# settylab/Mellon

Measured on AMD Instinct MI355X. Metric: cells/sec fit_predict, higher is better.
Workload: dtype f64

## Files before the change

### include/mellon_hip.h

```cpp
#ifndef MELLON_HIP_H
#define MELLON_HIP_H

#include <stdint.h>

#ifdef __cplusplus
extern "C" {
#endif

typedef struct mln_ctx mln_ctx;
typedef struct mln_fit mln_fit;

typedef enum {
  MLN_OK = 0,
  MLN_ERR_NOT_PD = 1,
  MLN_ERR_SHAPE = 2,
  MLN_ERR_HIP = 3,
  MLN_ERR_RCCL = 4,
  MLN_ERR_ARG = 5,
  MLN_ERR_UNSUPPORTED = 6,
  MLN_ERR_NOCONV = 7
} mln_status;

typedef enum {
  MLN_K_MATERN32 = 1,
// ... 35 lines not shown
int mln_ctx_create(int device, mln_ctx** out);
void mln_ctx_destroy(mln_ctx* ctx);
const char* mln_last_error(mln_ctx* ctx);
int mln_device_info(mln_ctx* ctx, char* name, int name_cap, int* n_cu, int64_t* mem_bytes);
int mln_device_count(int* count_out);
int mln_synchronize(mln_ctx* ctx);

int mln_malloc(mln_ctx* ctx, int64_t bytes, void** dev_ptr);
int mln_free(mln_ctx* ctx, void* dev_ptr);
int mln_memcpy(mln_ctx* ctx, void* dst, const void* src, int64_t bytes);
int mln_host_register(mln_ctx* ctx, const void* host_ptr, int64_t bytes);
int mln_host_unregister(mln_ctx* ctx, const void* host_ptr);
int mln_release_cached_memory(void);
int mln_diag_alloc_stats(int64_t* out);

#define MLN_UNIQUE_ID_BYTES 128
int mln_comm_unique_id(void* id_out );
int mln_comm_init(mln_ctx* ctx, const void* id, int n_ranks, int rank);
int mln_comm_allreduce_sum(mln_ctx* ctx, double* buf, int64_t count);
typedef struct mln_loopback mln_loopback;
int mln_loopback_create(int n_ranks , mln_loopback** out);
void mln_loopback_destroy(mln_loopback* group);
int mln_comm_init_loopback(mln_ctx* ctx, mln_loopback* group, int rank);
typedef int (*mln_host_collective_fn)(void* user, int op, double* buf, double* buf2, int64_t count);
int mln_comm_init_host(mln_ctx* ctx, int n_ranks, int rank, mln_host_collective_fn fn, void* user);
void mln_loopback_abort(mln_loopback* group);
int mln_comm_info(mln_ctx* ctx, int32_t* info, double* stats, int32_t flags);

int mln_kernel_matrix(mln_ctx* ctx, const mln_kernel_desc* cov, const double* x, int64_t n,
                      const double* y, int64_t m, int32_t d, double* out);

int mln_kernel_gram(mln_ctx* ctx, const mln_kernel_desc* cov, const double* x, int64_t n_local, int32_t d,
                    const double* xu, int64_t m, double* out );
int mln_nn_distances(mln_ctx* ctx, const double* x, int64_t n, const double* y, int64_t m, int32_t d,
                     int64_t self_offset, double* out );
int mln_knn(mln_ctx* ctx, const double* x, int64_t n, const double* y, int64_t m, int32_t d, int32_t k,
            int32_t exclude, int64_t self_offset, double* dist , int64_t* idx );
int mln_local_dimensionality(mln_ctx* ctx, const double* x, int64_t n, int32_t d, const int64_t* nbr, int64_t q,
                             int32_t k, double* out );

int mln_kmeans(mln_ctx* ctx, const double* x, int64_t n, int32_t d, int64_t m, int64_t seed,
               int32_t max_iter, double tol, double* centers, int32_t* n_iter_out, double* inertia_out);
int mln_kmeans_sklearn(mln_ctx* ctx, const double* x, int64_t n, int32_t d, int64_t m, int64_t first_id,
                       const double* uniforms, int32_t n_local_trials, int32_t max_iter, double tol, double* centers,
                       int64_t* indices_out, int32_t* n_iter_out, double* inertia_out);

int mln_chol_lower(mln_ctx* ctx, double* A, int64_t m, double add_diag);

int mln_trsm_lower(mln_ctx* ctx, const double* Lf, int64_t m, int32_t trans, double* B, int64_t p);

#define MLN_FIT_IMPLICIT 1
int mln_fit_prepare(mln_ctx* ctx, const mln_kernel_desc* cov, const double* x, int64_t n_local,
                    int32_t d, const double* xu, int64_t m, double jitter, const double* Lp_in,
                    int32_t flags, mln_fit** out);
int mln_fit_from_L(mln_ctx* ctx, const double* L, int64_t n_local, int64_t m, const double* Lp,
                   mln_fit** out);
#define MLN_FIT_FULL 2
#define MLN_FIT_DEFER_LP 4
int mln_fit_prepare_from_K(mln_ctx* ctx, const double* Kuu, int64_t n_local, int64_t m, double jitter,
                           const double* Lp_in, int32_t flags, mln_fit** out);
int mln_fit_set_K_rows(mln_fit* fit, int64_t row0, int64_t n_rows, const double* K_rows);
int mln_fit_finish_K(mln_fit* fit);
int mln_gemm(mln_ctx* ctx, int32_t ta, int32_t tb, int64_t M, int64_t N, int64_t K, double alpha, const double* A,
             int64_t lda, const double* B, int64_t ldb, double beta, double* C, int64_t ldc);
int mln_ewise(mln_ctx* ctx, int32_t op, const double* a, const double* b, double scalar, double* out, int64_t count);

void mln_fit_destroy(mln_fit* fit);
int mln_fit_get_Lp(mln_fit* fit, double* out );
int mln_fit_get_L(mln_fit* fit, int64_t row0, int64_t n_rows, double* out );
int mln_fit_rank(mln_fit* fit, int64_t* m_out);

int mln_kernel_grad(mln_ctx* ctx, const mln_kernel_desc* cov, const double* x, int64_t n, const double* y,
                    int64_t m, int32_t d, double* out );
int mln_predict_gradient(mln_ctx* ctx, const mln_kernel_desc* cov, const double* xnew, int64_t n_new,
                         int32_t d, const double* centers, int64_t m, const double* W ,
                         double* out );
int mln_predict_hessian(mln_ctx* ctx, const mln_kernel_desc* cov, const double* xnew, int64_t n_new, int32_t d,
                        const double* centers, int64_t m, const double* W , double* out);


int mln_eigh(mln_ctx* ctx, const double* A, int64_t m, double* w, double* V, int32_t* n_sweeps);
int mln_fit_gram_eigh(mln_fit* fit, double* w , int32_t* n_sweeps);
int mln_fit_gram_rank(mln_fit* fit, double tol, int64_t* rank_out, double* sigma_max_out);
int mln_fit_project(mln_fit* fit, int64_t p, mln_fit** out);

int mln_ridge_init(mln_fit* fit, const double* target, double* z0 );

int mln_precond_build(mln_fit* fit, int64_t row_stride );
int mln_fit_set_row_offset(mln_fit* fit, int64_t global_row0);
int mln_precond_apply(mln_fit* fit, int32_t mode, const double* in, double* out);
int mln_objective_precond(mln_fit* fit, const double* u, double* loss, double* grad_u ,
                          double* z_out );

int mln_fit_set_likelihood(mln_fit* fit, const double* V, const double* Vdr, double mu);

int mln_objective(mln_fit* fit, const double* z, double* loss, double* grad ,
                  double* hess_diag );

int mln_objective_batch(mln_fit* fit, const double* Z, int32_t S, double* loss , double* grad );

typedef struct {
  int32_t maxiter;
  int32_t maxcor;
  int32_t maxls;
  double ftol;
  double gtol;
} mln_solver_opts;
int mln_map_solve(mln_fit* fit, const double* z0, const mln_solver_opts* opts ,
                  double* z_out , double* loss_out, int32_t* n_eval_out, int32_t* n_iter_out,
                  int32_t* status_out);

int mln_fit_set_dim_likelihood(mln_fit* fit, const double* ell, int32_t k, double mu_dim, double mu_dens);
int mln_dim_objective(mln_fit* fit, const double* z, double* loss, double* grad ,
                      double* hess_diag );

int mln_dim_objective_batch(mln_fit* fit, const double* Z, int32_t S, double* loss , double* grad );

int mln_transform(mln_fit* fit, const double* z, double mu, double* f_out );

int mln_weights_cholesky(mln_fit* fit, const double* z, double* w );
int mln_weights_full(mln_fit* fit, const double* y, int64_t p, double mu, double* w );

int mln_sparse_solve(mln_ctx* ctx, const mln_kernel_desc* cov, const double* x, int64_t n_local,
                     int32_t d, const double* xu, int64_t m, const double* y, int64_t p, double mu,
                     double sigma, double jitter, double* W );
int mln_sparse_solve_factors(mln_ctx* ctx, const mln_kernel_desc* cov, const double* x, int64_t n_local,
                             int32_t d, const double* xu, int64_t m, const double* y, int64_t p, double mu,
                             double sigma, double jitter, double* W, double* Lp_out, double* Cs_out);

enum { MLN_SIGMA_SCALAR = 0, MLN_SIGMA_PER_OUTPUT = 1, MLN_SIGMA_PER_CELL = 2 };
int mln_sparse_solve_noise(mln_ctx* ctx, const mln_kernel_desc* cov, const double* x, int64_t n_local,
                           int32_t d, const double* xu, int64_t m, const double* y, int64_t p, double mu,
                           const double* sigma, int32_t sigma_kind, double jitter, double* W );

int mln_full_conditional_noise(mln_ctx* ctx, const mln_kernel_desc* cov, const double* x, int64_t n, int32_t d,
                               const double* y, int64_t p, double mu, const double* sigma , double jitter,
                               double* W, double* leverage, double* corrected_r2, double* variance_W);

int mln_landmark_leverage(mln_ctx* ctx, const mln_kernel_desc* cov, const double* x, int64_t n_local, int32_t d,
                          const double* xu, int64_t m, const double* Lk, const double* sigma, int64_t p,
                          double jitter, double* out );

int mln_predict_mean(mln_ctx* ctx, const mln_kernel_desc* cov, const double* xnew, int64_t n_new,
                     int32_t d, const double* centers, int64_t m, const double* W, int64_t p,
                     double mu, double* out);

int mln_diag_peak(mln_ctx* ctx, int32_t what, int64_t bytes, double* result);
int mln_diag_dgemm(mln_ctx* ctx, int32_t ta, int32_t tb, int64_t M, int64_t N, int64_t K,
                   int32_t lower_only, int32_t split_k, int32_t reps, double* ms_out);
int mln_diag_dgemm_compare(mln_ctx* ctx, int32_t ta, int32_t tb, int64_t M, int64_t N, int64_t K, int32_t lower_only,
                           int32_t kmode, double beta, int32_t any_size, double* out);
int mln_diag_gram_i8(mln_ctx* ctx, const double* A, int64_t rows, int64_t m, double* out, int32_t reps, double* ms_out);
int mln_diag_overlap(mln_ctx* ctx, int64_t n, int64_t m, int32_t d, int64_t gram_rows, double* out );

int mln_predict_covariance(mln_ctx* ctx, const mln_kernel_desc* cov, const double* xnew, int64_t n_new,
                           int32_t d, const double* centers, int64_t m, const double* Lf, int32_t diag,
                           double* out);
int mln_predict_mean_covariance(mln_ctx* ctx, const mln_kernel_desc* cov, const double* xnew, int64_t n_new,
                                int32_t d, const double* centers, int64_t m, const double* W, int64_t q,
                                int32_t diag, double* out);

#define MLN_N_STAGE_TIMES 22
int mln_stage_times(mln_fit* fit, double* out );

#ifdef __cplusplus
}
#endif
#endif
```

### mellon_amd/_lib.py

```python
import ctypes as C
import os
import threading

import numpy as np

_HERE = os.path.dirname(os.path.abspath(__file__))
LIB_PATH = os.path.join(_HERE, "libmellon_hip.so")

MLN_OK, MLN_ERR_NOT_PD, MLN_ERR_SHAPE, MLN_ERR_HIP, MLN_ERR_RCCL, MLN_ERR_ARG, MLN_ERR_UNSUPPORTED = range(7)
MLN_UNIQUE_ID_BYTES = 128
MLN_N_STAGE_TIMES = 22

K_MATERN32, K_MATERN52, K_EXPQUAD, K_EXPONENTIAL, K_RATQUAD, K_LINEAR, K_DISTANCE = 1, 2, 3, 4, 5, 6, 7
OP_LEAF, OP_CONST, OP_ADD, OP_MUL, OP_POW = 0, 1, 2, 3, 4


HOST_COLLECTIVE_FN = C.CFUNCTYPE(C.c_int, C.c_void_p, C.c_int, C.c_void_p, C.c_void_p, C.c_int64)


class MellonHipError(RuntimeError):
    """HIP / RCCL / argument failure inside libmellon_hip.so."""


class Leaf(C.Structure):
    _fields_ = [("kind", C.c_int32), ("ndims", C.c_int32), ("ls", C.c_double), ("alpha", C.c_double),
                ("dims", C.POINTER(C.c_int32))]


class Tok(C.Structure):
    _fields_ = [("op", C.c_int32), ("leaf", C.c_int32), ("value", C.c_double)]


class SolverOpts(C.Structure):
    _fields_ = [("maxiter", C.c_int32), ("maxcor", C.c_int32), ("maxls", C.c_int32), ("ftol", C.c_double),
                ("gtol", C.c_double)]


class KernelDesc(C.Structure):
    _fields_ = [("n_leaves", C.c_int32), ("n_toks", C.c_int32), ("leaves", C.POINTER(Leaf)),
                ("toks", C.POINTER(Tok))]


_vp, _i64, _i32, _dbl, _dp = C.c_void_p, C.c_int64, C.c_int32, C.c_double, C.c_void_p
_KD = C.POINTER(KernelDesc)
SYMBOLS = [
    ("mln_ctx_create", C.c_int, [C.c_int, C.POINTER(_vp)]),
    ("mln_ctx_destroy", None, [_vp]),
    ("mln_last_error", C.c_char_p, [_vp]),
    ("mln_device_info", C.c_int, [_vp, C.c_char_p, C.c_int, C.POINTER(C.c_int), C.POINTER(_i64)]),
    ("mln_device_count", C.c_int, [C.POINTER(C.c_int)]),
    ("mln_synchronize", C.c_int, [_vp]),
    ("mln_malloc", C.c_int, [_vp, _i64, C.POINTER(_vp)]),
    ("mln_free", C.c_int, [_vp, _vp]),
    ("mln_memcpy", C.c_int, [_vp, _vp, _vp, _i64]),
    ("mln_host_register", C.c_int, [_vp, _vp, _i64]),
    ("mln_host_unregister", C.c_int, [_vp, _vp]),
    ("mln_release_cached_memory", C.c_int, []),
    ("mln_diag_alloc_stats", C.c_int, [_vp]),
    ("mln_comm_unique_id", C.c_int, [_vp]),
    ("mln_comm_init", C.c_int, [_vp, _vp, C.c_int, C.c_int]),
    ("mln_comm_allreduce_sum", C.c_int, [_vp, _dp, _i64]),
    ("mln_loopback_create", C.c_int, [C.c_int, C.POINTER(_vp)]),
    ("mln_loopback_destroy", None, [_vp]),
    ("mln_comm_init_loopback", C.c_int, [_vp, _vp, C.c_int]),
    ("mln_comm_init_host", C.c_int, [_vp, C.c_int, C.c_int, _vp, _vp]),
    ("mln_loopback_abort", None, [_vp]),
    ("mln_comm_info", C.c_int, [_vp, C.POINTER(_i32), _dp, _i32]),
    ("mln_kernel_matrix", C.c_int, [_vp, _KD, _dp, _i64, _dp, _i64, _i32, _dp]),
    ("mln_kernel_grad", C.c_int, [_vp, _KD, _dp, _i64, _dp, _i64, _i32, _dp]),
    ("mln_predict_gradient", C.c_int, [_vp, _KD, _dp, _i64, _i32, _dp, _i64, _dp, _dp]),
    ("mln_predict_hessian", C.c_int, [_vp, _KD, _dp, _i64, _i32, _dp, _i64, _dp, _dp]),
    ("mln_kernel_gram", C.c_int, [_vp, _KD, _dp, _i64, _i32, _dp, _i64, _dp]),
    ("mln_nn_distances", C.c_int, [_vp, _dp, _i64, _dp, _i64, _i32, _i64, _dp]),
    ("mln_knn", C.c_int, [_vp, _dp, _i64, _dp, _i64, _i32, _i32, _i32, _i64, _dp, _vp]),
    ("mln_local_dimensionality", C.c_int, [_vp, _dp, _i64, _i32, _vp, _i64, _i32, _dp]),
    ("mln_kmeans", C.c_int, [_vp, _dp, _i64, _i32, _i64, _i64, _i32, _dbl, _dp, C.POINTER(_i32), C.POINTER(_dbl)]),
    ("mln_kmeans_sklearn", C.c_int, [_vp, _dp, _i64, _i32, _i64, _i64, _dp, _i32, _i32, _dbl, _dp, _vp, C.POINTER(_i32),
                                     C.POINTER(_dbl)]),
    ("mln_chol_lower", C.c_int, [_vp, _dp, _i64, _dbl]),
    ("mln_trsm_lower", C.c_int, [_vp, _dp, _i64, _i32, _dp, _i64]),
    ("mln_fit_prepare", C.c_int, [_vp, _KD, _dp, _i64, _i32, _dp, _i64, _dbl, _dp, _i32, C.POINTER(_vp)]),
    ("mln_fit_from_L", C.c_int, [_vp, _dp, _i64, _i64, _dp, C.POINTER(_vp)]),
    ("mln_fit_prepare_from_K", C.c_int, [_vp, _dp, _i64, _i64, _dbl, _dp, _i32, C.POINTER(_vp)]),
    ("mln_fit_set_K_rows", C.c_int, [_vp, _i64, _i64, _dp]),
    ("mln_fit_finish_K", C.c_int, [_vp]),
    ("mln_gemm", C.c_int, [_vp, _i32, _i32, _i64, _i64, _i64, _dbl, _dp, _i64, _dp, _i64, _dbl, _dp, _i64]),
    ("mln_ewise", C.c_int, [_vp, _i32, _dp, _dp, _dbl, _dp, _i64]),
    ("mln_fit_destroy", None, [_vp]),
    ("mln_fit_get_Lp", C.c_int, [_vp, _dp]),
    ("mln_fit_get_L", C.c_int, [_vp, _i64, _i64, _dp]),
    ("mln_fit_rank", C.c_int, [_vp, C.POINTER(_i64)]),
    ("mln_eigh", C.c_int, [_vp, _dp, _i64, _dp, _dp, C.POINTER(_i32)]),
    ("mln_fit_gram_eigh", C.c_int, [_vp, _dp, C.POINTER(_i32)]),
    ("mln_fit_gram_rank", C.c_int, [_vp, _dbl, C.POINTER(_i64), C.POINTER(_dbl)]),
    ("mln_fit_project", C.c_int, [_vp, _i64, C.POINTER(_vp)]),
    ("mln_ridge_init", C.c_int, [_vp, _dp, _dp]),
    ("mln_precond_build", C.c_int, [_vp, _i64]),
    ("mln_fit_set_row_offset", C.c_int, [_vp, _i64]),
    ("mln_precond_apply", C.c_int, [_vp, _i32, _dp, _dp]),
    ("mln_objective_precond", C.c_int, [_vp, _dp, C.POINTER(_dbl), _dp, _dp]),
    ("mln_map_solve", C.c_int, [_vp, _dp, C.POINTER(SolverOpts), _dp, C.POINTER(_dbl), C.POINTER(_i32),
                                C.POINTER(_i32), C.POINTER(_i32)]),
    ("mln_fit_set_likelihood", C.c_int, [_vp, _dp, _dp, _dbl]),
    ("mln_objective", C.c_int, [_vp, _dp, C.POINTER(_dbl), _dp, _dp]),
    ("mln_objective_batch", C.c_int, [_vp, _dp, _i32, _dp, _dp]),
    ("mln_fit_set_dim_likelihood", C.c_int, [_vp, _dp, _i32, _dbl, _dbl]),
    ("mln_dim_objective", C.c_int, [_vp, _dp, C.POINTER(_dbl), _dp, _dp]),
    ("mln_dim_objective_batch", C.c_int, [_vp, _dp, _i32, _dp, _dp]),
    ("mln_transform", C.c_int, [_vp, _dp, _dbl, _dp]),
    ("mln_weights_cholesky", C.c_int, [_vp, _dp, _dp]),
    ("mln_weights_full", C.c_int, [_vp, _dp, _i64, _dbl, _dp]),
    ("mln_sparse_solve", C.c_int, [_vp, _KD, _dp, _i64, _i32, _dp, _i64, _dp, _i64, _dbl, _dbl, _dbl, _dp]),
    ("mln_sparse_solve_factors", C.c_int, [_vp, _KD, _dp, _i64, _i32, _dp, _i64, _dp, _i64, _dbl, _dbl, _dbl, _dp,
                                           _dp, _dp]),
    ("mln_sparse_solve_noise", C.c_int, [_vp, _KD, _dp, _i64, _i32, _dp, _i64, _dp, _i64, _dbl, _dp, _i32, _dbl, _dp]),
    ("mln_full_conditional_noise", C.c_int, [_vp, _KD, _dp, _i64, _i32, _dp, _i64, _dbl, _dp, _dbl, _dp, _dp, _dp, _dp]),
    ("mln_landmark_leverage", C.c_int, [_vp, _KD, _dp, _i64, _i32, _dp, _i64, _dp, _dp, _i64, _dbl, _dp]),
    ("mln_predict_mean", C.c_int, [_vp, _KD, _dp, _i64, _i32, _dp, _i64, _dp, _i64, _dbl, _dp]),
    ("mln_predict_covariance", C.c_int, [_vp, _KD, _dp, _i64, _i32, _dp, _i64, _dp, _i32, _dp]),
    ("mln_predict_mean_covariance", C.c_int, [_vp, _KD, _dp, _i64, _i32, _dp, _i64, _dp, _i64, _i32, _dp]),
    ("mln_stage_times", C.c_int, [_vp, _dp]),
    ("mln_diag_peak", C.c_int, [_vp, _i32, _i64, C.POINTER(_dbl)]),
    ("mln_diag_overlap", C.c_int, [_vp, _i64, _i64, _i32, _i64, _dp]),
    ("mln_diag_gram_i8", C.c_int, [_vp, _vp, _i64, _i64, _vp, _i32, C.POINTER(_dbl)]),
    ("mln_diag_dgemm", C.c_int, [_vp, _i32, _i32, _i64, _i64, _i64, _i32, _i32, _i32, C.POINTER(_dbl)]),
    ("mln_diag_dgemm_compare", C.c_int, [_vp, _i32, _i32, _i64, _i64, _i64, _i32, _i32, _dbl, _i32, C.POINTER(_dbl)]),
]

_lib = None
_lib_lock = threading.Lock()


def load_library():
    global _lib
    with _lib_lock:
        if _lib is not None:
            return _lib
        if not os.path.exists(LIB_PATH):
            raise MellonHipError(
                f"{LIB_PATH} is missing: build it with `python -c \"import __graft_entry__ as g; g.build()\"` "
                "(hipcc --offload-arch=gfx950).  mellon_amd has no CPU fallback.")
        lib = C.CDLL(LIB_PATH, mode=C.RTLD_GLOBAL)
        for name, res, args in SYMBOLS:
            fn = getattr(lib, name)
            fn.restype = res
            fn.argtypes = args
        _lib = lib
        return lib


def device_count():
    n = C.c_int(0)
    load_library().mln_device_count(C.byref(n))
    return int(n.value)


class BlockEvaluatedCov:
    rows_per_block = 8192

    def block(self, x, y):
        raise NotImplementedError


def _needs_program(desc, what):
    if isinstance(desc, BlockEvaluatedCov):
        raise NotImplementedError(
            f"{what} needs a covariance that lowers to one device program (built-in kernels combined with + * ** within "
            "the program limits); user-defined Python kernels and larger trees support k(), fit and the predictive mean.")


class DeviceArray:

    def __init__(self, ctx, shape):
        self.ctx = ctx
        self.shape = tuple(int(s) for s in shape)
        self.size = int(np.prod(self.shape)) if self.shape else 1
        ptr = C.c_void_p()
        ctx._check(ctx.lib.mln_malloc(ctx.handle, self.size * 8, C.byref(ptr)))
        self.ptr = ptr.value

    @property
    def nbytes(self):
        return self.size * 8

    @property
    def ndim(self):
        return len(self.shape)

    def to_host(self):
        out = np.empty(self.shape, dtype=np.float64)
        self.ctx._check(self.ctx.lib.mln_memcpy(self.ctx.handle, out.ctypes.data, self.ptr, self.nbytes))
        return out

    def free(self):
        if self.ptr is not None and self.ctx.handle is not None:
            self.ctx.lib.mln_free(self.ctx.handle, self.ptr)
        self.ptr = None

    def __del__(self):
        try:
            self.free()
        except Exception:
            pass


def _f64(a):
    return np.ascontiguousarray(a, dtype=np.float64)


def _ptr(a):
    if a is None:
        return None
    if isinstance(a, DeviceArray):
        return a.ptr
    return a.ctypes.data


class Context:

    def __init__(self, device=None):
        self.lib = load_library()
        if device is None:
            device = int(os.environ.get("LOCAL_RANK", "0")) if "MELLON_AMD_DEVICE" not in os.environ \
                else int(os.environ["MELLON_AMD_DEVICE"])
        h = C.c_void_p()
        rc = self.lib.mln_ctx_create(int(device), C.byref(h))
        self.handle = None
        if rc != MLN_OK:
            msg = self.lib.mln_last_error(None).decode()
            raise MellonHipError(f"mln_ctx_create(device={device}) failed: {msg}")
        self.handle = h.value
        self.device = int(device)
        self.n_ranks, self.rank = 1, 0

    def close(self):
        if self.handle is not None:
            self.lib.mln_ctx_destroy(self.handle)
            self.handle = None

    def __del__(self):
        try:
            self.close()
        except Exception:
            pass

    def _check(self, rc, jitter=None):
        if rc == MLN_OK:
            return
        msg = self.lib.mln_last_error(self.handle).decode()
        if rc == MLN_ERR_NOT_PD:
            raise ValueError(
                f"Covariance not positively definite with jitter={jitter}. "
                "Consider increasing the jitter for numerical stabilization.")
        if rc == MLN_ERR_SHAPE:
            raise ValueError(f"libmellon_hip: {msg}")
        if rc == MLN_ERR_UNSUPPORTED:
            raise NotImplementedError(f"libmellon_hip: {msg}")
        cause = None
        staged = getattr(self, "_host_collective", None)
        if staged is not None and getattr(staged[1], "failure", None) is not None:
            cause, staged[1].failure = staged[1].failure, None
        raise MellonHipError(f"libmellon_hip error {rc}: {msg}" + (f" ({type(cause).__name__}: {cause})" if cause else "")) from cause

    def device_info(self):
        name = C.create_string_buffer(64)
        cu, mem = C.c_int(), C.c_int64()
        self._check(self.lib.mln_device_info(self.handle, name, 64, C.byref(cu), C.byref(mem)))
        return {"arch": name.value.decode(), "n_cu": cu.value, "mem_bytes": mem.value}

    def synchronize(self):
        self._check(self.lib.mln_synchronize(self.handle))

    def to_device(self, a):
        a = _f64(a)
        d = DeviceArray(self, a.shape)
        self._check(self.lib.mln_memcpy(self.handle, d.ptr, a.ctypes.data, a.nbytes))
# ... 622 lines not shown

    def gram_rank(self, tol):
        r, smax = _i64(0), C.c_double()
        self._check(self.lib.mln_fit_gram_rank(self.handle, float(tol), C.byref(r), C.byref(smax)))
        return int(r.value), smax.value

    def project(self, p):
        new = Fit.__new__(Fit)
        new.ctx, new.lib, new.handle = self.ctx, self.lib, None
        h = C.c_void_p()
        self._check(self.lib.mln_fit_project(self.handle, int(p), C.byref(h)))
        new.handle = h.value
        new.n, new.d, new.m, new.jitter = self.n, None, int(p), None
        new.implicit = False
        new._has_lp = False
        return new

    def __init__(self, ctx, desc, x, landmarks, jitter, Lp=None, implicit=False):
        self.ctx, self.lib, self.handle = ctx, ctx.lib, None
        self.implicit = bool(implicit) and landmarks is not None
        x = x if isinstance(x, DeviceArray) else _as2d(x)
        n, d = x.shape
        xu = None if landmarks is None else (landmarks if isinstance(landmarks, DeviceArray) else _as2d(landmarks))
        m = n if xu is None else xu.shape[0]
        Lp_ = None if Lp is None else _f64(Lp)
        if Lp_ is not None and Lp_.shape != (m, m):
            raise ValueError(f"Lp has shape {Lp_.shape}, expected {(m, m)}")
        h = C.c_void_p()
        flags = (1 | (4 if Lp_ is None else 0)) if self.implicit else 0
        ctx._check(self.lib.mln_fit_prepare(ctx.handle, desc.ref, _ptr(x), n, d, _ptr(xu), m, float(jitter),
                                            _ptr(Lp_), flags, C.byref(h)), jitter=jitter)
        self.handle = h.value
        self.n, self.d, self.m, self.jitter = n, d, m, jitter
        self._has_lp = True

    def _check(self, rc, jitter=None):
        if rc == MLN_ERR_NOT_PD and self.lib.mln_last_error(self.ctx.handle).startswith(b"cov(xu, xu)"):
            jitter = self.jitter
        self.ctx._check(rc, jitter=jitter)

    def close(self):
        if self.handle is not None and self.ctx.handle is not None:
            self.lib.mln_fit_destroy(self.handle)
        self.handle = None

    def __del__(self):
        try:
            self.close()
        except Exception:
            pass

    def Lp(self):
        out = np.empty((self.m, self.m), dtype=np.float64)
        self._check(self.lib.mln_fit_get_Lp(self.handle, out.ctypes.data))
        return out

    def L(self, row0=0, n_rows=None):
        n_rows = self.n - row0 if n_rows is None else n_rows
        out = np.empty((n_rows, self.m), dtype=np.float64)
        self._check(self.lib.mln_fit_get_L(self.handle, row0, n_rows, out.ctypes.data))
        return out

    def ridge_init(self, target):
        target = target if isinstance(target, DeviceArray) else _f64(target)
        z0 = np.empty(self.m, dtype=np.float64)
        self._check(self.lib.mln_ridge_init(self.handle, _ptr(target), z0.ctypes.data), jitter="ridge")
        return z0

    def set_likelihood(self, V, Vdr, mu):
        V = V if isinstance(V, DeviceArray) else _f64(V)
        Vdr = Vdr if isinstance(Vdr, DeviceArray) else _f64(Vdr)
        self._check(self.lib.mln_fit_set_likelihood(self.handle, _ptr(V), _ptr(Vdr), float(mu)))

    def objective(self, z, with_hess=False):
        z = _f64(z)
        loss = C.c_double()
        grad = np.empty(self.m, dtype=np.float64)
        hess = np.empty(self.m, dtype=np.float64) if with_hess else None
        self._check(self.lib.mln_objective(self.handle, z.ctypes.data, C.byref(loss), grad.ctypes.data,
                                               _ptr(hess)))
        return (loss.value, grad, hess) if with_hess else (loss.value, grad)

    def objective_batch(self, Z):
        Z = _f64(Z)
        if Z.ndim != 2 or Z.shape[1] != self.m or Z.shape[0] < 1:
            raise ValueError(f"Z has shape {Z.shape}, expected (S >= 1, {self.m})")
        loss = np.empty(Z.shape[0], dtype=np.float64)
        grad = np.empty(Z.shape, dtype=np.float64)
        self._check(self.lib.mln_objective_batch(self.handle, Z.ctypes.data, int(Z.shape[0]), loss.ctypes.data,
                                                 grad.ctypes.data))
        return loss, grad

    def set_dim_likelihood(self, ell, mu_dim, mu_dens):
        ell = _f64(ell)
        if ell.ndim != 2 or ell.shape[0] != self.n:
            raise ValueError(f"ell has shape {ell.shape}, expected ({self.n}, k)")
        self._check(self.lib.mln_fit_set_dim_likelihood(self.handle, ell.ctypes.data, int(ell.shape[1]), float(mu_dim),
                                                        float(mu_dens)))

    def dim_objective(self, z, with_hess=False):
        z = _f64(z)
        if z.shape != (2, self.m):
            raise ValueError(f"z has shape {z.shape}, expected {(2, self.m)}")
        loss = C.c_double()
        grad = np.empty((2, self.m), dtype=np.float64)
        hess = np.empty((2, self.m), dtype=np.float64) if with_hess else None
        self._check(self.lib.mln_dim_objective(self.handle, z.ctypes.data, C.byref(loss), grad.ctypes.data, _ptr(hess)))
        return (loss.value, grad, hess) if with_hess else (loss.value, grad)

    def dim_objective_batch(self, Z):
        Z = _f64(Z)
        if Z.ndim not in (2, 3) or Z.shape[0] < 1 or Z.shape[1:] not in ((2, self.m), (2 * self.m,)):
            raise ValueError(f"Z has shape {Z.shape}, expected (S >= 1, 2, {self.m}) or (S >= 1, {2 * self.m})")
        loss = np.empty(Z.shape[0], dtype=np.float64)
        grad = np.empty(Z.shape, dtype=np.float64)
        self._check(self.lib.mln_dim_objective_batch(self.handle, Z.ctypes.data, int(Z.shape[0]), loss.ctypes.data,
                                                     grad.ctypes.data))
        return loss, grad

    def precond_build(self, row_stride=1, row_offset=0, force=False):
        built = getattr(self, "_precond_stride", None)
        if built is not None and (not force or built == int(row_stride)):
            return
        self._check(self.lib.mln_fit_set_row_offset(self.handle, int(row_offset)))
        self._check(self.lib.mln_precond_build(self.handle, int(row_stride)), jitter="ridge")
        self._precond_stride = max(1, int(row_stride))

    def precond_apply(self, mode, v):
        v = _f64(v)
        out = np.empty(self.m, dtype=np.float64)
        self._check(self.lib.mln_precond_apply(self.handle, int(mode), v.ctypes.data, out.ctypes.data),
                        jitter="ridge")
        return out

    def objective_precond(self, u):
        u = _f64(u)
        loss = C.c_double()
        grad = np.empty(self.m, dtype=np.float64)
        z = np.empty(self.m, dtype=np.float64)
        self._check(self.lib.mln_objective_precond(self.handle, u.ctypes.data, C.byref(loss), grad.ctypes.data,
                                                       z.ctypes.data), jitter="ridge")
        return loss.value, grad, z

    def map_solve(self, z0, maxiter=5000, maxcor=10, maxls=30, ftol=1e-13, gtol=1e-7):
        z0 = _f64(z0)
        opts = SolverOpts(int(maxiter), int(maxcor), int(maxls), float(ftol), float(gtol))
        z = np.empty(self.m, dtype=np.float64)
        loss, nev, nit, st = C.c_double(), C.c_int32(), C.c_int32(), C.c_int32()
        self._check(self.lib.mln_map_solve(self.handle, z0.ctypes.data, C.byref(opts), z.ctypes.data,
                                               C.byref(loss), C.byref(nev), C.byref(nit), C.byref(st)),
                        jitter="ridge")
        return z, loss.value, nev.value, nit.value, st.value

    def transform(self, z, mu, out=None):
        z = _f64(z)
        ret = np.empty(self.n, dtype=np.float64) if out is None else out
        self._check(self.lib.mln_transform(self.handle, z.ctypes.data, float(mu), _ptr(ret)))
        return ret

    def weights_cholesky(self, z):
        z = _f64(z)
        w = np.empty(self.m, dtype=np.float64)
        self._check(self.lib.mln_weights_cholesky(self.handle, z.ctypes.data, w.ctypes.data))
        return w

    def weights_full(self, y, mu):
        y2 = _f64(y)
        p = 1 if y2.ndim == 1 else y2.shape[1]
        w = np.empty_like(y2)
        self._check(self.lib.mln_weights_full(self.handle, y2.ctypes.data, p, float(mu), w.ctypes.data))
        return w

    def stage_times(self):
        out = np.zeros(MLN_N_STAGE_TIMES, dtype=np.float64)
        self._check(self.lib.mln_stage_times(self.handle, out.ctypes.data))
        keys = ["kernel_matrix_s", "cholesky_s", "trsm_s", "ridge_gram_s", "ridge_solve_s",
                "objective_kernel_s", "objective_launches", "objective_bytes_per_launch",
                "objective32_kernel_s", "objective32_launches", "copy32_format", "emulation_excluded_s",
                "objective_sub_kernel_s", "objective_sub_launches", "objective_sub_stride", "precond_rebuild_s",
                "precond_rebuilds", "objective_pass_equivalents", "precond_rebuilds_declined", "precond_reverts",
                "start_halvings", "rank_path"]
        return dict(zip(keys, out.tolist()))


def release_cached_memory():
    load_library().mln_release_cached_memory()


def alloc_stats():
    out = (C.c_int64 * 5)()
    rc = load_library().mln_diag_alloc_stats(out)
    if rc != 0:
        raise MellonHipError(f"mln_diag_alloc_stats failed ({rc})")
    keys = ["live_blocks", "live_bytes", "live_pinned_blocks", "cached_bytes", "driver_allocs"]
    return dict(zip(keys, [int(v) for v in out]))


_default_ctx = None


def default_context():
    global _default_ctx
    from . import distributed
    comm = distributed.thread_state()
    if comm is not None and comm.ctx is not None:
        return comm.ctx
    if _default_ctx is None or _default_ctx.handle is None:
        _default_ctx = Context()
    return _default_ctx
```

### mellon_amd/csrc/api_internal.h

```cpp
#pragma once
#include <chrono>
#include <cmath>
#include <cstdio>
#include <cstdlib>
#include <algorithm>
#include <atomic>
#include <cstring>
#include <memory>
#include <mutex>
#include <string>
#include <thread>
#include <vector>

#include "linalg.h"
#include "mln_internal.h"
#include "objective.h"
#include "precond_rebuild.h"
#include "solver.h"

void fit_events_borrow(mln_ctx* ctx, std::vector<hipEvent_t>* evs);
void fit_events_return(mln_ctx* ctx, std::vector<hipEvent_t>* evs);

bool is_device_ptr(const void* p);
double now_s();

struct DevIn {
  mln_ctx* ctx;
  const double* dev = nullptr;
  DevBuf<double> owned;
  int init(mln_ctx* c, const double* p, size_t count) {
    ctx = c;
    if (count == 0 || !p) { dev = p; return MLN_OK; }
    if (is_device_ptr(p)) { dev = p; return MLN_OK; }
    MLN_TRY(owned.alloc(ctx, count, "device copy of an input"));
    MLN_HIP(ctx, hipMemcpyAsync(owned, p, count * sizeof(double), hipMemcpyHostToDevice, ctx->stream));
    dev = owned;
    return MLN_OK;
  }
  ~DevIn() {
    if (owned) (void)hipStreamSynchronize(ctx->stream);
  }
};

struct DevOut {
  mln_ctx* ctx;
  double* dev = nullptr;
  DevBuf<double> owned;
  double* host = nullptr;
  size_t count = 0;
  int init(mln_ctx* c, double* p, size_t n, bool copy_in = false) {
    ctx = c; count = n;
    if (n == 0) { dev = p; return MLN_OK; }
    if (is_device_ptr(p)) { dev = p; return MLN_OK; }
    host = p;
    MLN_TRY(owned.alloc(ctx, n, "device copy of an output"));
    if (copy_in) MLN_HIP(ctx, hipMemcpyAsync(owned, p, n * sizeof(double), hipMemcpyHostToDevice, ctx->stream));
    dev = owned;
    return MLN_OK;
  }
  int commit() {
    if (owned && count) {
      MLN_HIP(ctx, hipMemcpyAsync(host, owned, count * sizeof(double), hipMemcpyDeviceToHost, ctx->stream));
    }
    MLN_HIP(ctx, hipStreamSynchronize(ctx->stream));
    return MLN_OK;
  }
  ~DevOut() {
    if (owned) (void)hipStreamSynchronize(ctx->stream);
  }
};

struct Precond { DevBuf<double> C, Cinv, P, Q1, Q2; };

struct mln_fit {
  mln_ctx* ctx = nullptr;
  DevCov cov;
  int d = 0;
  int64_t n = 0, m = 0, ldl = 0, ldp = 0;
  bool full = false;
  DevBuf<double> L_own;
  double* L = nullptr;
  DevBuf<double> Lp;
  TriInv tri;
  DevBuf<double> V, Vdr;
  double mu = 0.0;
  int n_wg = 0;
  DevBuf<double> part_grad, part_hess, part_loss;
  DevBuf<double> d_z, d_out;
  PinnedBuf<double> h_z, h_out;
  hipEvent_t ev0 = nullptr, ev1 = nullptr;
  double times[MLN_N_STAGE_TIMES] = {0};
  Precond pc, pc_saved;
  DevBuf<double> d_u, d_gu, d_tmp;
  int n_wg_cap = 0;
  bool kspace = false;
  DevBuf<double> Kj;
  bool lp_pending = false, lp_failed = false, tri_pending = false;
  double jitter = 0.0;
  DevBuf<double> d_w;
  std::vector<double> z_cached;
  DevBuf<double> d_w_cached;
  DevBuf<double> d_zw, d_zr;
  DevBuf<double> eigU;
  DevBuf<float> L32;
  double emu_excluded = 0.0;
  bool cov_bounded01 = false;
  int l32_fixed = 0;
  int evals32 = 0;
  double times32 = 0.0;
  int64_t ld2 = 0;
  DevBuf<int> d_over;
  int64_t row0 = 0;
  SolverBuffers sv{};
  DevBuf<double> sv_block;
  PinnedBuf<SolverState> h_state;
  int sv_maxcor = 0;
  std::vector<hipEvent_t> evs;
  DevBuf<double> f_keep[2];
  int f_final = -1;
  int64_t precond_stride = 0;
  bool from_K = false, k_finished = false;
  int64_t k_rows_done = 0;
  int n_revert = 0, n_rebuild_skipped = 0, n_start_halvings = 0, rank_path = 0;
  double build_seconds = 0.0;
  double times_sub = 0.0, times_rebuild = 0.0, sub_pass_equiv = 0.0;
  int evals_sub = 0, n_rebuild = 0;
  DevBuf<double> dim_ell;
  int dim_k = 0;
  double mu_dim = 0.0, mu_dens = 0.0;
  DevBuf<double> dim_part, dim_z, dim_out;
  ~mln_fit();
};

int dev_allreduce(mln_ctx* ctx, double* dev, int64_t count);
int dev_bcast0(mln_ctx* ctx, double* dev, int64_t count);
int reject_distance_leaf(mln_ctx* ctx, const DevCov& dc);
int64_t pad16(int64_t m);
void fit_sample_rows(const mln_fit* f, int64_t s, int64_t* first, int64_t* rows);
int fit_alloc_workspace(mln_fit* f);
int fit_prepare_impl(mln_ctx* ctx, const mln_kernel_desc* cov, const double* x, int64_t n, int32_t d,
                            const double* xu, int64_t m, double jitter, const double* Lp_in, int32_t flags,
                            mln_fit* f);
ObjArgs obj_args(mln_fit* f);
void obj_account(mln_fit* f, bool f32 = false);
int fit_w_from_z(mln_fit* f, const double* z_dev, double* w_dev, const double* z_host = nullptr);
int fit_cache_pair_from_u(mln_fit* f, const double* u_dev);
int fit_enqueue_eval(mln_fit* f, const double* u_dev, double* gn_dev, bool use32, const int* gate,
                            hipEvent_t* ev, const std::vector<int64_t>* sub_strides = nullptr);
int fit_objective_u(mln_fit* f, const double* u, double* loss, double* grad_u, double* z_out,
                           bool use32 = false);
int fit_solver_alloc(mln_fit* f, int maxcor);
int gram_of(mln_ctx* ctx, const double* A, int64_t lda, int64_t rows, int64_t m, double alpha, double* G,
                   int64_t ldg, bool quantised = false);
int emulated_ranks(const mln_ctx* ctx);
int fit_ensure_kj(mln_fit* f);
int fit_ensure_lp(mln_fit* f, bool need_tri = true);
int fit_lp_finish(mln_fit* f, int rc_chol, double t0);
int fit_gram(mln_fit* f, double* G, int64_t ldg, int64_t row_stride, bool whiten = true);
int fit_gemvT(mln_fit* f, const double* t_dev, double* rhs_dev);
int fit_factor_precond(mln_fit* f);
int fit_build_precond(mln_fit* f, int64_t row_stride);
int fit_rebuild_precond(mln_fit* f, const double* f_dev, double rows_per_m, int* outcome, double cap = 1e300);
int fit_precond_revert(mln_fit* f);
int fit_small_gemv(mln_fit* f, const double* M, int trans, const double* w, double* y);
int launch_scale_rows_cols(mln_ctx* ctx, double* A, int64_t ld, int64_t rows, int64_t cols, const double* row,
                                  const double* col);
int sparse_solve_impl(mln_ctx* ctx, const mln_kernel_desc* cov, const double* x, int64_t n_local,
                             int32_t d, const double* xu, int64_t m, const double* y, int64_t p, double mu,
                             const double* sigmas, int32_t kind, double jitter, double* W, double* Lp_out,
                             double* Cs_out);
unsigned grid_1d(int64_t count);
```

### mellon_amd/csrc/api_solve.hip

```cpp
#include "api_internal.h"
#include "mln_options.h"


void obj_account(mln_fit* f, bool f32) {
  float ms = 0.f;
  const bool ok = hipEventElapsedTime(&ms, f->ev0, f->ev1) == hipSuccess;
  if (f32) {
    if (ok) f->times32 += 1e-3 * ms;
    f->evals32 += 1;
    return;
  }
  if (ok) f->times[5] += 1e-3 * ms;
  f->times[6] += 1.0;
  f->times[7] = (double)f->n * (double)f->ldl * 8.0;
}

int fit_w_from_z(mln_fit* f, const double* z_dev, double* w_dev, const double* z_host) {
  mln_ctx* ctx = f->ctx;
  if (z_host && f->z_cached.size() == (size_t)f->m &&
      std::memcmp(z_host, f->z_cached.data(), sizeof(double) * f->m) == 0) {
    MLN_HIP(ctx, hipMemcpyAsync(w_dev, f->d_w_cached, sizeof(double) * f->m, hipMemcpyDeviceToDevice, ctx->stream));
    return MLN_OK;
  }
  MLN_TRY(fit_ensure_lp(f));
  MLN_HIP(ctx, hipMemcpyAsync(w_dev, z_dev, sizeof(double) * f->m, hipMemcpyDeviceToDevice, ctx->stream));
  return triinv_solve_left_T(ctx, f->tri, w_dev, 1, 1);
}

int fit_cache_pair_from_u(mln_fit* f, const double* u_dev) {
  mln_ctx* ctx = f->ctx;
  f->z_cached.assign((size_t)f->m, 0.0);
  MLN_HIP(ctx, hipMemcpyAsync(f->z_cached.data(), f->d_z, sizeof(double) * f->m, hipMemcpyDeviceToHost, ctx->stream));
  if (f->kspace) MLN_TRY(fit_small_gemv(f, f->pc.P, 0, u_dev, f->d_w_cached));
  MLN_HIP(ctx, hipStreamSynchronize(ctx->stream));
  return MLN_OK;
}

extern "C" int mln_objective(mln_fit* f, const double* z, double* loss, double* grad, double* hess_diag) {
  if (!f || !z || !loss || !grad) return MLN_ERR_ARG;
  mln_ctx* ctx = f->ctx;
  if (!f->V) { mln_set_error(ctx, "mln_fit_set_likelihood has not been called"); return MLN_ERR_ARG; }
  if (hess_diag && f->kspace) {
    mln_set_error(ctx, "the Hessian diagonal needs the explicit factor L: prepare the fit without MLN_FIT_IMPLICIT");
    return MLN_ERR_UNSUPPORTED;
  }
  MLN_HIP(ctx, hipSetDevice(ctx->device));
  MLN_TRY(fit_ensure_lp(f));
  const int64_t m = f->m;
  MLN_HIP(ctx, hipMemcpyAsync(f->d_z, z, sizeof(double) * m, hipMemcpyDefault, ctx->stream));
  MLN_HIP(ctx, hipMemcpyAsync(f->h_z, f->d_z, sizeof(double) * m, hipMemcpyDeviceToHost, ctx->stream));
  ObjArgs a = obj_args(f);
  if (f->kspace) {
    MLN_TRY(fit_w_from_z(f, f->d_z, f->d_w));
    a.z = f->d_w;
  }
  if (hess_diag) a.part_hess = f->part_hess;
  const int64_t nout = 1 + m + (hess_diag ? m : 0);
  MLN_HIP(ctx, hipEventRecord(f->ev0, ctx->stream));
  MLN_TRY(launch_objective(ctx, a));
  MLN_HIP(ctx, hipEventRecord(f->ev1, ctx->stream));
  MLN_TRY(launch_reduce_obj(ctx, a, f->d_out));
  MLN_TRY(dev_allreduce(ctx, f->d_out, nout));
  if (f->kspace) MLN_TRY(triinv_solve_left(ctx, f->tri, f->d_out + 1, 1, 1));
  MLN_HIP(ctx, hipMemcpyAsync(f->h_out, f->d_out, sizeof(double) * nout, hipMemcpyDeviceToHost, ctx->stream));
  MLN_HIP(ctx, hipStreamSynchronize(ctx->stream));
  obj_account(f);
  double zz = 0.0;
  for (int64_t j = 0; j < m; ++j) zz += f->h_z[j] * f->h_z[j];
  *loss = f->h_out[0] + 0.5 * zz + 0.5 * (double)m * std::log(2.0 * M_PI);
  std::vector<double> tmp;
  double* gh = grad;
  if (is_device_ptr(grad)) { tmp.resize(m); gh = tmp.data(); }
  for (int64_t j = 0; j < m; ++j) gh[j] = f->h_out[1 + j] + f->h_z[j];
  if (gh != grad) MLN_HIP(ctx, hipMemcpy(grad, gh, sizeof(double) * m, hipMemcpyHostToDevice));
  if (hess_diag) {
    std::vector<double> th;
    double* hh = hess_diag;
    if (is_device_ptr(hess_diag)) { th.resize(m); hh = th.data(); }
    for (int64_t j = 0; j < m; ++j) hh[j] = f->h_out[1 + m + j] + 1.0;
    if (hh != hess_diag) MLN_HIP(ctx, hipMemcpy(hess_diag, hh, sizeof(double) * m, hipMemcpyHostToDevice));
  }
  return MLN_OK;
}

extern "C" int mln_transform(mln_fit* f, const double* z, double mu, double* f_out) {
  if (!f || !z || (f->n > 0 && !f_out)) return MLN_ERR_ARG;
  mln_ctx* ctx = f->ctx;
  MLN_HIP(ctx, hipSetDevice(ctx->device));
  if (f->n == 0) return MLN_OK;
  MLN_HIP(ctx, hipMemcpyAsync(f->d_z, z, sizeof(double) * f->m, hipMemcpyDefault, ctx->stream));
  if (f->f_final >= 0 && mu == f->mu && !is_device_ptr(z) && f->z_cached.size() == (size_t)f->m &&
      std::memcmp(z, f->z_cached.data(), sizeof(double) * f->m) == 0) {
    MLN_HIP(ctx, hipMemcpyAsync(f_out, f->f_keep[f->f_final], sizeof(double) * (size_t)f->n, hipMemcpyDefault, ctx->stream));
    MLN_HIP(ctx, hipStreamSynchronize(ctx->stream));
    return MLN_OK;
  }
  DevOut o;
  MLN_TRY(o.init(ctx, f_out, (size_t)f->n));
  ObjArgs a = obj_args(f);
  if (f->kspace) {
    MLN_TRY(fit_w_from_z(f, f->d_z, f->d_w, is_device_ptr(z) ? nullptr : z));
    a.z = f->d_w;
  }
  a.f_out = o.dev;
  a.mu = mu;
  MLN_TRY(launch_objective(ctx, a));
  return o.commit();
}

int fit_enqueue_eval(mln_fit* f, const double* u_dev, double* gn_dev, bool use32, const int* gate,
                            hipEvent_t* ev, const std::vector<int64_t>* sub_strides) {
  mln_ctx* ctx = f->ctx;
  const int64_t m = f->m, ld = f->ldl, ld2 = f->ld2;
  if (f->kspace) {
    GemvTri g1{f->pc.P, ld, m, u_dev, f->d_w, nullptr, 1, m, m, 0, 0, gate};
    MLN_TRY(launch_gemv_tri(ctx, g1));
    GemvTri gk{f->Kj, f->ldp, m, f->d_w, f->d_zr, nullptr, 2, m, m, 0, 0, gate};
    MLN_TRY(launch_gemv_tri(ctx, gk));
  } else {
    GemvTri g1{f->pc.Q1, ld, m, u_dev, f->d_zr, nullptr, 1, m, m, 0, 0, gate};
    MLN_TRY(launch_gemv_tri(ctx, g1));
  }
  ObjArgs a = obj_args(f);
  a.z = f->kspace ? f->d_w : f->d_zr;
  a.gate = gate;
  if (gate && f->f_keep[0] && objective_can_keep_f(f->n, f->n_wg)) { a.f_keep[0] = f->f_keep[0]; a.f_keep[1] = f->f_keep[1]; a.f_slot = &f->sv.st->f_slot; }
  if (gate) { a.cap = &f->sv.st->cap; a.over_flag = f->d_over; }
  if (ev) MLN_HIP(ctx, hipEventRecord(ev[0], ctx->stream));
  if (f->L32 && (gate || use32)) {
    ObjArgs a32 = a;
    a32.L32 = f->L32;
    a32.l32_fixed = f->l32_fixed;
    a32.gate_want = MLN_GATE_F32;
    if (gate) a32.cap = &f->sv.st->cap;
    MLN_TRY(launch_objective(ctx, a32));
  }
  if (ev) MLN_HIP(ctx, hipEventRecord(ev[1], ctx->stream));
  if (gate || !use32 || !f->L32) {
    a.gate_want = MLN_GATE_F64;
    MLN_TRY(launch_objective(ctx, a));
  }
  if (gate && sub_strides) {
    for (size_t lv = 0; lv < sub_strides->size(); ++lv) {
      const int64_t sub_stride = (*sub_strides)[lv];
      ObjArgs as = a;
      int64_t first = 0, rows = 0;
      fit_sample_rows(f, sub_stride, &first, &rows);
      as.n = rows; as.row_first = first; as.row_stride = sub_stride; as.out_scale = (double)sub_stride;
      as.f_keep[0] = as.f_keep[1] = nullptr; as.f_slot = nullptr;
      as.gate_want = MLN_GATE_SUB;
      as.gate2 = &f->sv.st->sub_level; as.gate2_want = (int)lv;
      MLN_TRY(launch_objective(ctx, as));
    }
  }
  if (ev) MLN_HIP(ctx, hipEventRecord(ev[2], ctx->stream));
  MLN_TRY(launch_reduce_obj2(ctx, a, f->d_zr + ld2 + m, f->d_zr + ld2));
  MLN_TRY(dev_allreduce(ctx, f->d_zr + ld2, m + 2));
  if (f->kspace) {
    GemvTri g2{f->pc.Cinv, ld, m, f->d_zr, gn_dev, nullptr, 0, m, m, 0, 0, gate};
    g2.xadd = f->d_zr + ld2;
    MLN_TRY(launch_gemv_tri(ctx, g2));
  } else {
    GemvTri g2{f->pc.Q2, 2 * ld, m, f->d_zr, gn_dev, nullptr, 0, m, m, ld, ld2, gate};
    MLN_TRY(launch_gemv_tri(ctx, g2));
  }
  return MLN_OK;
}

int fit_objective_u(mln_fit* f, const double* u, double* loss, double* grad_u, double* z_out,
                           bool use32) {
  mln_ctx* ctx = f->ctx;
  const int64_t m = f->m;
  MLN_HIP(ctx, hipMemcpyAsync(f->d_u, u, sizeof(double) * m, hipMemcpyDefault, ctx->stream));
  hipEvent_t ev[3] = {f->ev0, use32 ? f->ev1 : f->ev0, f->ev1};
  MLN_TRY(fit_enqueue_eval(f, f->d_u, f->d_gu, use32, nullptr, ev));
  MLN_HIP(ctx, hipMemcpyAsync(f->h_out, f->d_zr + f->ld2 + m, sizeof(double), hipMemcpyDeviceToHost, ctx->stream));
  MLN_HIP(ctx, hipMemcpyAsync(f->h_out + 1, f->d_gu, sizeof(double) * m, hipMemcpyDeviceToHost, ctx->stream));
  MLN_HIP(ctx, hipMemcpyAsync(f->h_z, f->kspace ? f->d_w : f->d_zr, sizeof(double) * m, hipMemcpyDeviceToHost, ctx->stream));
  if (f->kspace) MLN_HIP(ctx, hipMemcpyAsync(f->h_out + 1 + m, f->d_zr, sizeof(double) * m, hipMemcpyDeviceToHost, ctx->stream));
  MLN_HIP(ctx, hipStreamSynchronize(ctx->stream));
  obj_account(f, use32);
  double zz = 0.0;
  for (int64_t j = 0; j < m; ++j) zz += f->h_z[j] * (f->kspace ? f->h_out[1 + m + j] : f->h_z[j]);
  *loss = f->h_out[0] + 0.5 * zz + 0.5 * (double)m * std::log(2.0 * M_PI);
  std::memcpy(grad_u, f->h_out + 1, sizeof(double) * m);
  if (z_out && f->kspace) {
    MLN_TRY(fit_ensure_lp(f, false));
    MLN_TRY(fit_small_gemv(f, f->Lp, 1, f->d_w, f->d_z));
    MLN_HIP(ctx, hipMemcpyAsync(z_out, f->d_z, sizeof(double) * m, hipMemcpyDeviceToHost, ctx->stream));
    MLN_HIP(ctx, hipStreamSynchronize(ctx->stream));
  } else if (z_out) {
    std::memcpy(z_out, f->h_z, sizeof(double) * m);
  }
  return MLN_OK;
}

extern "C" int mln_objective_precond(mln_fit* f, const double* u, double* loss, double* grad_u, double* z_out) {
  if (!f || !u || !loss || !grad_u) return MLN_ERR_ARG;
  mln_ctx* ctx = f->ctx;
  if (!f->V) { mln_set_error(ctx, "mln_fit_set_likelihood has not been called"); return MLN_ERR_ARG; }
  MLN_HIP(ctx, hipSetDevice(ctx->device));
  MLN_TRY(fit_build_precond(f, 1));
  return fit_objective_u(f, u, loss, grad_u, z_out);
}

int fit_solver_alloc(mln_fit* f, int maxcor) {
  mln_ctx* ctx = f->ctx;
  if (f->sv_block && f->sv_maxcor >= maxcor) return MLN_OK;
  if (f->sv_block) { MLN_HIP(ctx, hipStreamSynchronize(ctx->stream)); f->sv_block.reset(); }
  const size_t ld = (size_t)f->ldl;
  const size_t n_dbl = 6 * ld + 2 * (size_t)maxcor * ld + 2 * 64 + 4 * 512 + (sizeof(SolverState) + 63) / 64 * 8;
  MLN_TRY(f->sv_block.alloc_zeroed(ctx, n_dbl, "sv_block"));
  double* p = f->sv_block;
  SolverBuffers& b = f->sv;
  b.u = p; p += ld; b.g = p; p += ld; b.un = p; p += ld; b.gn = p; p += ld; b.d = p; p += ld;
  b.S = p; p += (size_t)maxcor * ld; b.Y = p; p += (size_t)maxcor * ld;
  b.rho = p; p += 64; b.yy = p; p += 64;
  b.c = p; p += ld;
  b.trace = p; p += 4 * 512;
  b.st = (SolverState*)p;
  b.ld = (int64_t)ld;
  b.z = f->kspace ? f->d_w : f->d_zr;
  b.z2 = f->kspace ? f->d_zr : nullptr;
  b.lik = f->d_zr + f->ld2 + f->m;
  b.over = f->d_zr + f->ld2 + f->m + 1;
  f->sv_maxcor = maxcor;
  if (!f->h_state) MLN_TRY(f->h_state.alloc(ctx, 1, "h_state"));
  return MLN_OK;
}

extern "C" int mln_map_solve(mln_fit* f, const double* z0, const mln_solver_opts* opts_in, double* z_out,
                             double* loss_out, int32_t* n_eval_out, int32_t* n_iter_out, int32_t* status_out) {
  if (!f || !z0 || !z_out) return MLN_ERR_ARG;
  mln_ctx* ctx = f->ctx;
  if (!f->V) { mln_set_error(ctx, "mln_fit_set_likelihood has not been called"); return MLN_ERR_ARG; }
  MLN_HIP(ctx, hipSetDevice(ctx->device));
  if (f->m > 8192) {
    mln_set_error(ctx, "mln_map_solve: the device-resident solver holds at most 8192 landmarks; drive mln_objective_precond "
                       "from the host instead (the Python binding does: inference.minimize_lbfgsb)");
    return MLN_ERR_UNSUPPORTED;
  }
  MLN_TRY(fit_build_precond(f, 1));
  fit_events_borrow(ctx, &f->evs);
  mln_solver_opts o = {5000, 10, 30, 1e-13, 1e-7};
  if (opts_in) o = *opts_in;
  if (o.maxcor < 1) o.maxcor = 1;
  if (o.maxcor > 64) o.maxcor = 64;
  if (o.maxls < 1) o.maxls = 1;
  const int64_t m = f->m;
  MLN_TRY(fit_solver_alloc(f, o.maxcor));
  for (int b = 0; b < 2; ++b)
    if (!f->f_keep[b]) MLN_TRY(f->f_keep[b].alloc(ctx, (size_t)(f->n > 0 ? f->n : 1), "f_keep"));
  f->f_final = -1;
  MLN_HIP(ctx, hipMemcpyAsync(f->d_u, z0, sizeof(double) * m, hipMemcpyDefault, ctx->stream));
  if (f->kspace) {
    MLN_TRY(fit_w_from_z(f, f->d_u, f->d_w, is_device_ptr(z0) ? nullptr : z0));
    MLN_TRY(fit_small_gemv(f, f->pc.C, 1, f->d_w, f->d_gu));
  } else {
    MLN_TRY(fit_small_gemv(f, f->pc.C, 1, f->d_u, f->d_gu));
  }
  MLN_TRY(dev_bcast0(ctx, f->d_gu, m));
  const int trace_lvl = std::getenv("MELLON_AMD_TRACE") ? std::atoi(std::getenv("MELLON_AMD_TRACE")) : 0;
  const bool phase32 = f->kspace && f->L32 != nullptr;
  SolverState init{};
  init.gate = phase32 ? MLN_GATE_F32 : MLN_GATE_F64;
  init.mode = MLN_SOLVE_FIRST;
  init.status = 1;
  init.maxiter = o.maxiter; init.maxcor = o.maxcor; init.maxls = o.maxls;
  init.m = (int)m;
  init.ftol = o.ftol; init.gtol = o.gtol;
  init.ftol32 = f->l32_fixed ? 1e-9 : 3e-6;
  init.use_corr = (phase32 && f->l32_fixed) ? 1 : 0;
  if (const char* ev = mln_experiment("MELLON_AMD_CORRECTED")) init.use_corr = init.use_corr && std::atoi(ev) != 0;
  init.prior_const = 0.5 * (double)m * std::log(2.0 * M_PI);
  init.t0 = 1.0;
  init.boost = 0.15;
  if (const char* ev = mln_experiment("MELLON_AMD_LS_BOOST")) init.boost = std::atof(ev);
  init.cap = 9.0;
  init.cap_step = 4.0;
  if (const char* ev = mln_experiment("MELLON_AMD_EXP_CAP"))
    init.cap = (std::strcmp(ev, "off") == 0 || std::atof(ev) <= 0.0) ? __builtin_inf() : std::atof(ev);
  if (phase32 && !mln_experiment("MELLON_AMD_EXP_CAP")) init.cap = __builtin_inf();
  init.cap0 = init.cap;
  init.boost_fall = 0.15;
  std::vector<int64_t> sub_strides;
  if (f->precond_stride >= 11) sub_strides.push_back(std::max<int64_t>(2, 3 * f->precond_stride / 16));
  if (const char* ev = mln_experiment("MELLON_AMD_SUBSAMPLE")) { if (std::atoi(ev) == 0) sub_strides.clear(); }
  const std::vector<int64_t>* subs = sub_strides.empty() ? nullptr : &sub_strides;
  init.gate_full = init.gate;
  init.sub_tol = 1e-3;
  init.sub_max_evals = 1 << 30;
  init.n_sub_levels = (int)sub_strides.size();
  init.sub_level = 0;
  if (subs) init.gate = MLN_GATE_SUB;
  const double pass_s = (double)f->n * (double)f->ldl * 8.0 / 6.5e12 + 1.4e-4;
  const double md = (double)f->m;
  const double gram_rows = (double)f->n / (double)(f->precond_stride > 0 ? f->precond_stride : 1);
  const double build_model_s = 2.2e-4 * std::ceil(md / 128.0) + gram_rows * md * md * 2.0 / 1.0e15;
  double want_rebuild = (f->build_seconds > 0.0 && 13.0 * pass_s > build_model_s) ? 1.0 : 0.0;
  if (const char* ev = mln_experiment("MELLON_AMD_REBUILD")) want_rebuild = std::atoi(ev) != 0 ? 1.0 : 0.0;
  if (phase32 && !(f->l32_fixed)) want_rebuild = 0.0;
  const bool keeps_f = f->f_keep[0] && f->f_keep[1] && objective_can_keep_f(f->n, f->n_wg);
  {
    double vote[2] = {ctx->rank == 0 ? want_rebuild : 0.0, keeps_f ? 0.0 : 1.0};
    MLN_HIP(ctx, hipMemcpyAsync(f->d_tmp, vote, sizeof(vote), hipMemcpyHostToDevice, ctx->stream));
    MLN_TRY(dev_allreduce(ctx, f->d_tmp, 2));
    MLN_HIP(ctx, hipMemcpyAsync(vote, f->d_tmp, sizeof(vote), hipMemcpyDeviceToHost, ctx->stream));
    MLN_HIP(ctx, hipStreamSynchronize(ctx->stream));
    want_rebuild = (vote[0] != 0.0 && vote[1] == 0.0) ? 1.0 : 0.0;
  }
  int max_rebuilds = 1000;
  if (const char* ev = mln_experiment("MELLON_AMD_MAX_REBUILDS")) max_rebuilds = std::max(1, std::atoi(ev));
  init.rebuild_armed = want_rebuild != 0.0 ? (phase32 ? 1 : max_rebuilds) : 0;
  init.it_resume = -1;
  init.over_many = std::max(8.0, 1e-4 * (double)f->n * (double)(ctx->n_ranks > 1 ? ctx->n_ranks : 1));
  init.over_cnt_acc = 0.0;
  init.switch_t0 = 0.35;
  init.gap_tol = 0.2 * o.ftol;
  init.dec_prev = 0.0; init.dec_prev2 = 0.0;
  init.rebuild_tol = 1e-3;
  init.start_cap = 1e30;
  init.n_shrink = 0;
  init.revert_after = 0; init.it_at_resume = -1; init.pause_reason = 0;
  int revert_after = 60;
  if (const char* ev = mln_experiment("MELLON_AMD_REVERT_AFTER")) revert_after = std::atoi(ev);
  double rebuild_rows_per_m = 6.0;
  MLN_TRY(launch_solver_init(ctx, f->sv, init, f->d_gu));
  const int* gate = &f->sv.st->gate;
  static const bool timing = !(std::getenv("MELLON_AMD_TIMING") && std::atoi(std::getenv("MELLON_AMD_TIMING")) == 0);
  int n_enq = 0, rebuilds_this_solve = 0, failed_rebuilds = 0;
  auto events_for = [&](int i) -> hipEvent_t* {
    if (!timing || i >= 512) return nullptr;
    while ((int)f->evs.size() < 3 * (i + 1)) {
      hipEvent_t e;
      if (hipEventCreate(&e) != hipSuccess) return nullptr;
      f->evs.push_back(e);
    }
    return &f->evs[3 * i];
  };
  MLN_TRY(fit_enqueue_eval(f, f->sv.un, f->sv.gn, false, gate, events_for(n_enq), subs));
  ++n_enq;
  std::vector<std::pair<int, int>> slot_shift;
  const std::vector<int64_t>* subs_live = subs;
  int batch = 8;
  const int64_t hard_cap = (int64_t)o.maxiter * o.maxls + 16;
  for (;;) {
    for (int b = 0; b < batch; ++b) {
      MLN_TRY(launch_solver_step(ctx, f->sv, (int)m));
      MLN_TRY(fit_enqueue_eval(f, f->sv.un, f->sv.gn, false, gate, events_for(n_enq), subs_live));
      ++n_enq;
    }
    MLN_TRY(dev_bcast0(ctx, (double*)f->sv.st, (int64_t)(sizeof(SolverState) / sizeof(double))));
    MLN_HIP(ctx, hipMemcpyAsync(f->h_state, f->sv.st, sizeof(SolverState), hipMemcpyDeviceToHost, ctx->stream));
    MLN_HIP(ctx, hipStreamSynchronize(ctx->stream));
    if (f->h_state->gate == MLN_GATE_DONE) break;
    if (subs_live && f->h_state->n_eval_sub > 0 && f->h_state->gate != MLN_GATE_SUB) subs_live = nullptr;
    if (f->h_state->gate == MLN_GATE_PAUSE) {
      const double tr0 = now_s(), ex_r0 = f->emu_excluded;
      const SolverState ps = *f->h_state;
      const bool revert = ps.pause_reason == 2 && f->pc_saved.C;
      if (!revert && (ps.pause_reason == 2 || !ps.f_valid)) {
        MLN_TRY(launch_solver_resume(ctx, f->sv, ps.gate_after_pause, 0));
      } else {
        DevBuf<double> zt;
        MLN_TRY(zt.alloc_zeroed(ctx, 3 * (size_t)f->ldl, "zt"));
        double *gz = zt + f->ldl, *cz = gz + f->ldl;
        int rc = f->kspace ? fit_small_gemv(f, f->pc.P, 0, f->sv.u, zt) : fit_small_gemv(f, f->pc.Cinv, 1, f->sv.u, zt);
        if (rc == MLN_OK) rc = fit_small_gemv(f, f->pc.C, 0, f->sv.g, gz);
        if (rc == MLN_OK && ps.corr) rc = fit_small_gemv(f, f->pc.C, 0, f->sv.c, cz);
        int outcome = 0;
        if (rc == MLN_OK) rc = revert ? fit_precond_revert(f) : fit_rebuild_precond(f, f->f_keep[ps.f_slot], rebuild_rows_per_m * (rebuilds_this_solve > 0 ? 2.0 : 1.0), &outcome, ps.cap);
        if (rc == MLN_OK && outcome == 0) {
          rc = fit_small_gemv(f, f->pc.C, 1, zt, f->sv.u);
          if (rc == MLN_OK) rc = f->kspace ? fit_small_gemv(f, f->pc.P, 1, gz, f->sv.g) : fit_small_gemv(f, f->pc.Cinv, 0, gz, f->sv.g);
          if (rc == MLN_OK && ps.corr) rc = f->kspace ? fit_small_gemv(f, f->pc.P, 1, cz, f->sv.c) : fit_small_gemv(f, f->pc.Cinv, 0, cz, f->sv.c);
        }
        (void)hipStreamSynchronize(ctx->stream);
        zt.reset();
        MLN_TRY(rc);
        if (outcome == 0) {
          if (revert && ps.corr && (ps.gate_after_pause & 3) == MLN_GATE_F32)
            MLN_TRY(launch_solver_resume_plain32(ctx, f->sv, MLN_GATE_F32, (int)m, 1));
          else
            MLN_TRY(launch_solver_resume(ctx, f->sv, ps.gate_after_pause, 1, (revert || ps.rebuild_armed > 0) ? 0 : revert_after));
          if (revert) f->n_revert += 1; else { f->n_rebuild += 1; rebuilds_this_solve += 1; }
        } else {
          failed_rebuilds += 1;
          if (ps.corr && (ps.gate_after_pause & 3) == MLN_GATE_F32) MLN_TRY(launch_solver_resume_plain32(ctx, f->sv, MLN_GATE_F32, (int)m));
          else MLN_TRY(launch_solver_resume(ctx, f->sv, ps.gate_after_pause, 0, 0, failed_rebuilds >= 2 ? 0 : -1));
          f->n_rebuild_skipped += 1;
        }
        if (trace_lvl) fprintf(stderr, "[trace] map_solve pause at evaluation %d: %s\n", ps.n_eval,
                               revert ? "second preconditioner failed its trial: first one restored"
                                      : (outcome == 0 ? "preconditioner rebuilt" : (outcome == 1 ? "rebuild declined (weight range)" : "rebuild lost positive definiteness: kept the first")));
      }
      MLN_HIP(ctx, hipStreamSynchronize(ctx->stream));
      f->times_rebuild += now_s() - tr0 - (f->emu_excluded - ex_r0);
      slot_shift.push_back({ps.n_eval, n_enq - ps.n_eval});
      continue;
    }
    if (n_enq > hard_cap) { mln_set_error(ctx, "map_solve: the device solver did not terminate"); return MLN_ERR_NOCONV; }
    if (batch < 16 && f->h_state->gate == MLN_GATE_F64) batch = std::min(batch, 6);
  }
  const SolverState st = *f->h_state;
  if (f->pc_saved.C) (void)hipStreamSynchronize(ctx->stream);
  f->pc_saved = Precond();
  f->n_start_halvings = st.n_shrink;
  std::vector<double> tr;
  const int n_done = st.n_eval < 512 ? st.n_eval : 512;
  if (n_done > 0) {
    tr.resize((size_t)4 * n_done);
    MLN_HIP(ctx, hipMemcpy(tr.data(), f->sv.trace, sizeof(double) * 4 * n_done, hipMemcpyDeviceToHost));
    for (int i = 0; i < n_done && timing; ++i) {
      const int gcode = (int)tr[4 * i + 3] & 15, lvl = (int)tr[4 * i + 3] >> 4;
      const bool was32 = (gcode & 3) == MLN_GATE_F32, was_sub = gcode == MLN_GATE_SUB;
      int slot = i;
      for (const auto& sh : slot_shift) if (i >= sh.first) slot = i + sh.second;
      if (3 * (slot + 1) > (int)f->evs.size()) continue;
      float ms = 0.f;
      if (hipEventElapsedTime(&ms, f->evs[3 * slot + (was32 ? 0 : 1)], f->evs[3 * slot + (was32 ? 1 : 2)]) != hipSuccess) continue;
      if (was_sub) {
        f->times_sub += 1e-3 * ms; f->evals_sub += 1;
        f->sub_pass_equiv += 1.0 / (double)((lvl >= 0 && lvl < (int)sub_strides.size()) ? sub_strides[lvl] : 1);
      }
      else if (was32) { f->times32 += 1e-3 * ms; f->evals32 += 1; }
      else { f->times[5] += 1e-3 * ms; f->times[6] += 1.0; f->times[7] = (double)f->n * (double)f->ldl * 8.0; }
    }
    if (trace_lvl >= 2)
      for (int i = 0; i < n_done; ++i)
        fprintf(stderr, "[eval %d] %s mode=%d t=%.3g f=%.15g\n", i, ((int)tr[4 * i + 3] & 15) == MLN_GATE_F32 ? "f32" : (((int)tr[4 * i + 3] & 15) == MLN_GATE_F32C ? "f32c" : (((int)tr[4 * i + 3] & 15) == MLN_GATE_SUB ? (((int)tr[4 * i + 3] >> 4) ? "sub1" : "sub0") : "f64")),
                (int)tr[4 * i + 2], tr[4 * i + 1], tr[4 * i]);
  }
  {
    if (f->kspace) {
      GemvTri g1{f->pc.P, f->ldl, m, f->sv.u, f->d_w_cached, nullptr, 1, m, m, 0, 0, nullptr};
      MLN_TRY(launch_gemv_tri(ctx, g1));
      MLN_TRY(fit_ensure_lp(f, false));
      MLN_TRY(fit_small_gemv(f, f->Lp, 1, f->d_w_cached, f->d_z));
    } else {
      GemvTri g1{f->pc.Q1, f->ldl, m, f->sv.u, f->d_z, nullptr, 1, m, m, 0, 0, nullptr};
      MLN_TRY(launch_gemv_tri(ctx, g1));
    }
    f->z_cached.assign((size_t)m, 0.0);
    MLN_HIP(ctx, hipMemcpyAsync(f->z_cached.data(), f->d_z, sizeof(double) * m, hipMemcpyDeviceToHost, ctx->stream));
    MLN_HIP(ctx, hipMemcpyAsync(z_out, f->d_z, sizeof(double) * m, hipMemcpyDefault, ctx->stream));
    MLN_HIP(ctx, hipStreamSynchronize(ctx->stream));
  }
  if (st.f_valid && objective_can_keep_f(f->n, f->n_wg)) f->f_final = st.f_slot;
  if (trace_lvl)
    fprintf(stderr, "[trace] map_solve: %d evaluations (%d on the 32-bit copy, %d on the row subsample of stride %lld), %d iterations, "
            "%d rebuild(s), %d enqueued, status %d\n", st.n_eval, st.n_eval32, st.n_eval_sub, (long long)(subs ? sub_strides[0] : 0), st.it,
            f->n_rebuild, n_enq, st.status);
  if (loss_out) *loss_out = st.fx;
  if (n_eval_out) *n_eval_out = st.n_eval;
  if (n_iter_out) *n_iter_out = st.it;
  if (status_out) *status_out = st.status | ((st.status != 0 && st.over_acc && st.cap < 1e300) ? 4 : 0);
  return MLN_OK;
}

extern "C" int mln_weights_cholesky(mln_fit* f, const double* z, double* w) {
  if (!f || !z || !w) return MLN_ERR_ARG;
  mln_ctx* ctx = f->ctx;
  MLN_HIP(ctx, hipSetDevice(ctx->device));
  if (!f->Lp) { mln_set_error(ctx, "this fit handle holds no Lp"); return MLN_ERR_ARG; }
  DevOut o;
  MLN_TRY(o.init(ctx, w, (size_t)f->m));
  if (f->kspace && !is_device_ptr(z) && f->z_cached.size() == (size_t)f->m &&
      std::memcmp(z, f->z_cached.data(), sizeof(double) * f->m) == 0) {
    MLN_HIP(ctx, hipMemcpyAsync(o.dev, f->d_w_cached, sizeof(double) * f->m, hipMemcpyDeviceToDevice, ctx->stream));
    return o.commit();
  }
  MLN_TRY(fit_ensure_lp(f));
  MLN_HIP(ctx, hipMemcpyAsync(o.dev, z, sizeof(double) * f->m, hipMemcpyDefault, ctx->stream));
  MLN_TRY(triinv_solve_left_T(ctx, f->tri, o.dev, 1, 1));
  return o.commit();
}

extern "C" int mln_weights_full(mln_fit* f, const double* y, int64_t p, double mu, double* w) {
  if (!f || !y || !w || p < 1) return MLN_ERR_ARG;
  mln_ctx* ctx = f->ctx;
  MLN_HIP(ctx, hipSetDevice(ctx->device));
  if (!f->Lp) { mln_set_error(ctx, "this fit handle holds no Lp"); return MLN_ERR_ARG; }
  MLN_TRY(fit_ensure_lp(f));
  const int64_t cnt = f->m * p;
  DevOut o;
  MLN_TRY(o.init(ctx, w, (size_t)cnt));
  MLN_HIP(ctx, hipMemcpyAsync(o.dev, y, sizeof(double) * cnt, hipMemcpyDefault, ctx->stream));
  if (mu != 0.0) {
    DevBuf<double> ones;
    MLN_TRY(ones.alloc(ctx, cnt, "ones"));
    std::vector<double> h((size_t)cnt, 1.0);
    MLN_HIP(ctx, hipMemcpyAsync(ones, h.data(), sizeof(double) * cnt, hipMemcpyHostToDevice, ctx->stream));
    int rc = launch_axpby(ctx, cnt, -mu, ones, 1.0, o.dev);
    (void)hipStreamSynchronize(ctx->stream);
    ones.reset();
    if (rc != MLN_OK) return rc;
  }
  MLN_TRY(triinv_solve_left(ctx, f->tri, o.dev, p, p));
  MLN_TRY(triinv_solve_left_T(ctx, f->tri, o.dev, p, p));
  return o.commit();
}

extern "C" int mln_stage_times(mln_fit* f, double* out) {
  if (!f || !out) return MLN_ERR_ARG;
  for (int i = 0; i < 8; ++i) out[i] = f->times[i];
  out[8] = f->times32;
  out[9] = (double)f->evals32;
  out[10] = f->L32 ? (f->l32_fixed ? 2.0 : 1.0) : 0.0;
  out[11] = f->emu_excluded;
  out[12] = f->times_sub;
  out[13] = (double)f->evals_sub;
  out[14] = (double)(f->precond_stride > 0 ? f->precond_stride : 1);
  out[15] = f->times_rebuild;
  out[16] = (double)f->n_rebuild;
  out[17] = f->times[6] + 0.5 * (double)f->evals32 + f->sub_pass_equiv;
  out[18] = (double)f->n_rebuild_skipped;
  out[19] = (double)f->n_revert;
  out[20] = (double)f->n_start_halvings;
  out[21] = (double)f->rank_path;
  return MLN_OK;
}
```

### mellon_amd/csrc/objective.h

```cpp
#pragma once
#include "mln_core.h"

struct ObjArgs {
  const double* L; int64_t ldl; int64_t n; int64_t m;
  const double* z; const double* V; const double* Vdr; double mu;
  double* part_grad;
  double* part_hess;
  double* part_loss;
  const double* weights;
  double* f_out;
  int n_wg; int64_t m_pad;
  const float* L32;
  int l32_fixed;
  double* f_keep[2];
  const int* f_slot;
  const double* cap;
  int* over_flag;
  const int* gate;
  int gate_want;
  int64_t row_stride;
  int64_t row_first;
  double out_scale;
  const int* gate2;
  int gate2_want;
  int64_t seg_cols;
  int64_t seg_left;
  int f_accum;
};
enum { MLN_GATE_F64 = 0, MLN_GATE_F32 = 1, MLN_GATE_DONE = 2, MLN_GATE_SUB = 3, MLN_GATE_F32C = 5, MLN_GATE_PAUSE = 6 };
int objective_max_m();
int objective_max_m_one_pass();
bool objective_can_keep_f(int64_t n, int n_wg);
int launch_to_f32(mln_ctx* ctx, const double* src, float* dst, int64_t count);
int launch_objective(mln_ctx* ctx, const ObjArgs& a);
int launch_reduce_obj(mln_ctx* ctx, const ObjArgs& a, double* out_loss_grad );
int launch_reduce_obj2(mln_ctx* ctx, const ObjArgs& a, double* out_loss, double* out_grad);
int launch_gemv_rows(mln_ctx* ctx, const double* M, int64_t ld, int64_t rows, int64_t cols, const double* x,
                     double* y);
int launch_gemv_rows_tri(mln_ctx* ctx, const double* M, int64_t ld, int64_t rows, const double* x, double* y,
                         int upper, int64_t blk, int64_t ncol, int64_t seg);
struct GemvTri {
  const double* M; int64_t ld; int64_t rows;
  const double* x; double* y; double* y2;
  int upper;
  int64_t blk, ncol, mseg, xseg;
  const int* gate;
  const double* xadd;
};
int launch_gemv_tri(mln_ctx* ctx, const GemvTri& g);
```

### mellon_amd/csrc/objective.hip

```cpp
#include <cstdlib>

#include "mln_internal.h"
#include "objective.h"
#include "mln_options.h"

namespace {

constexpr int WG = 512;
constexpr int MLN_FSTAGE = 6144;
enum { MODE_OBJ = 0, MODE_OBJ_HESS = 1, MODE_GEMVT = 2, MODE_FONLY = 3 };

typedef double d2 __attribute__((ext_vector_type(2)));

__device__ __forceinline__ void lds_store_f64(double* base, int idx, double v) {
  const unsigned addr = (unsigned)(uintptr_t)(__attribute__((address_space(3))) double*)base + 8u * (unsigned)idx;
  asm volatile("ds_write_b64 %0, %1" : : "v"(addr), "v"(v));
}

struct RowMap { int64_t r0, rs; __device__ __forceinline__ int64_t operator()(int64_t i) const { return r0 + i * rs; } };
__device__ __forceinline__ RowMap row_map(const ObjArgs& a) { return RowMap{a.row_first, a.row_stride > 0 ? a.row_stride : 1}; }

template <int CPT, int R>
__device__ __forceinline__ void load_rows(const d2* __restrict__ L2, int64_t ld2, int64_t row, int64_t row_end,
                                          unsigned tid, d2 (&v)[R][CPT], const RowMap rm, unsigned lim) {
#pragma unroll
  for (int r = 0; r < R; ++r) {
    const bool rok = (row + r) < row_end;
    const d2* rowp = L2 + rm(rok ? (row + r) : row) * ld2;
#pragma unroll
    for (int c = 0; c < CPT; ++c) {
      unsigned off = (unsigned)c * WG + tid;
      off = (off < lim) ? off : lim - 1u;
      v[r][c] = __builtin_nontemporal_load(rowp + off);
    }
  }
}


template <int R>
__device__ __forceinline__ void load_lik(const ObjArgs& a, int64_t row, double (&pv)[2][R]) {
  const RowMap rm = row_map(a);
#pragma unroll
  for (int r = 0; r < R; ++r) {
    const int64_t i = rm((row + r < a.n) ? (row + r) : (a.n - 1));
    pv[0][r] = a.V[i];
    pv[1][r] = a.Vdr[i];
  }
}

template <int R>
__device__ __forceinline__ void load_lik_vec(const ObjArgs& a, int64_t row, int tid, double (&pv)[2][R]) {
  const RowMap rm = row_map(a);
  const int lane = tid & 63;
  const int64_t want = row + (lane < R ? lane : R - 1);
  const int64_t i = rm((want < a.n) ? want : (a.n - 1));
  pv[0][0] = a.V[i];
  pv[1][0] = a.Vdr[i];
}

__device__ __forceinline__ double read_lane_f64(double v, int lane) {
  const int lo = __builtin_amdgcn_readlane(__double2loint(v), lane);
  const int hi = __builtin_amdgcn_readlane(__double2hiint(v), lane);
  return __hiloint2double(hi, lo);
}

template <int R>
__device__ __forceinline__ double transposed_wave_sum(double (&v)[R], int lane) {
  constexpr int K = (R == 16) ? 4 : (R == 8) ? 3 : (R == 4) ? 2 : (R == 2) ? 1 : 0;
  static_assert((1 << K) == R, "R must be a power of two <= 16");
#pragma unroll
  for (int st = 0; st < K; ++st) {
    const int half = R >> (st + 1), mask = 32 >> st;
    const bool upper = (lane & mask) != 0;
#pragma unroll
    for (int i = 0; i < half; ++i) {
      const double send = upper ? v[i] : v[i + half];
      const double keep = upper ? v[i + half] : v[i];
      v[i] = keep + __shfl_xor(send, mask, 64);
    }
  }
  double s = v[0];
#pragma unroll
  for (int mask = 32 >> K; mask > 0; mask >>= 1) s += __shfl_xor(s, mask, 64);
  return s;
}

template <int CPT, int R, int MODE, bool KEEP, bool VEC = false>
__device__ __forceinline__ void process_rows(const ObjArgs& a, int64_t row, int64_t row_end, int tid, int par,
                                             const d2 (&v)[R][CPT], const d2 (&z)[CPT], d2 (&g)[CPT],
                                             d2 (&h)[CPT], double& loss, double (*red)[8][R], double* fstage,
                                             int64_t fbase, const double (&pv)[2][R], const double capv, int& any_over) {
  double coef[R], aexp[R];
  const RowMap rm = row_map(a);
  if constexpr (MODE == MODE_GEMVT) {
#pragma unroll
    for (int r = 0; r < R; ++r) coef[r] = (row + r < row_end) ? a.weights[rm(row + r)] : 0.0;
  } else if constexpr (VEC && (MODE == MODE_OBJ || MODE == MODE_OBJ_HESS)) {
    double dot[R];
#pragma unroll
    for (int r = 0; r < R; ++r) {
      double s = 0.0;
#pragma unroll
      for (int c = 0; c < CPT; ++c) {
        s = fma(v[r][c].x, z[c].x, s);
        s = fma(v[r][c].y, z[c].y, s);
      }
      dot[r] = s;
    }
    const int wave = tid >> 6, lane = tid & 63;
    constexpr int GRP = 64 / R;
    const double tot = transposed_wave_sum<R>(dot, lane);
    if ((lane & (GRP - 1)) == 0) red[par][wave][lane / GRP] = tot;
    __syncthreads();
    const int rl = lane < R ? lane : R - 1;
    double sr = 0.0;
#pragma unroll
    for (int w = 0; w < 8; ++w) sr += red[par][w][rl];
    const bool rok = lane < R && (row + rl) < row_end;
    const double f = sr + a.mu;
    const double Vi = pv[0][0];
    const double tt = f + Vi;
    const bool over = tt > capv;
    const double ex = rok ? exp(over ? capv : tt) : 0.0;
    const double dc = over ? (tt - capv) : 0.0;
    const double e = ex * fma(dc, fma(0.5, dc, 1.0), 1.0);
    const double cf = rok ? (over ? fma(ex, dc, ex - 1.0) : ex - 1.0) : 0.0;
    if (wave == 0 && rok) loss -= (f + pv[1][0]) - e;
    any_over += (wave == 0 && rok && over) ? 1 : 0;
    if (KEEP) lds_store_f64(fstage, (wave == 0 && rok) ? (int)(row + rl - fbase) : (MLN_FSTAGE + tid), f);
#pragma unroll
    for (int r = 0; r < R; ++r) {
      coef[r] = read_lane_f64(cf, r);
      aexp[r] = (MODE == MODE_OBJ_HESS) ? read_lane_f64(ex, r) : 0.0;
    }
  } else {
    double dot[R];
#pragma unroll
    for (int r = 0; r < R; ++r) {
      double s = 0.0;
#pragma unroll
      for (int c = 0; c < CPT; ++c) {
        s = fma(v[r][c].x, z[c].x, s);
        s = fma(v[r][c].y, z[c].y, s);
      }
#pragma unroll
      for (int off = 32; off > 0; off >>= 1) s += __shfl_xor(s, off, 64);
      dot[r] = s;
    }
    const int wave = tid >> 6;
    if ((tid & 63) == 0) {
#pragma unroll
      for (int r = 0; r < R; ++r) red[par][wave][r] = dot[r];
    }
    __syncthreads();
#pragma unroll
    for (int r = 0; r < R; ++r) {
      double s = 0.0;
#pragma unroll
      for (int w = 0; w < 8; ++w) s += red[par][w][r];
      const bool rok = (row + r) < row_end;
      const double f = s + a.mu;
      if (MODE == MODE_FONLY) {
        if (rok && tid == 0) a.f_out[row + r] = a.f_accum ? (s + a.f_out[row + r]) : f;
        coef[r] = 0.0;
        aexp[r] = 0.0;
      } else {
        const double Vi = KEEP ? pv[0][r] : (rok ? a.V[rm(row + r)] : 0.0);
        const double tt = f + Vi;
        const bool over = tt > capv;
        const double ex = rok ? exp(over ? capv : tt) : 0.0;
        const double dc = over ? (tt - capv) : 0.0;
        const double e = ex * fma(dc, fma(0.5, dc, 1.0), 1.0);
        aexp[r] = ex;
        coef[r] = rok ? (over ? fma(ex, dc, ex - 1.0) : ex - 1.0) : 0.0;
        if (KEEP) { if (tid == 0 && rok) loss -= (f + pv[1][r]) - e; }
        else if (tid == 0 && rok) loss -= (f + a.Vdr[rm(row + r)]) - e;
        any_over += (tid == 0 && rok && over) ? 1 : 0;
        if (KEEP) lds_store_f64(fstage, (tid == 0 && rok) ? (int)(row + r - fbase) : (MLN_FSTAGE + tid), f);
      }
    }
  }
  if (MODE != MODE_FONLY) {
#pragma unroll
    for (int r = 0; r < R; ++r) {
#pragma unroll
      for (int c = 0; c < CPT; ++c) {
        g[c].x = fma(coef[r], v[r][c].x, g[c].x);
        g[c].y = fma(coef[r], v[r][c].y, g[c].y);
        if (MODE == MODE_OBJ_HESS) {
          h[c].x = fma(aexp[r] * v[r][c].x, v[r][c].x, h[c].x);
          h[c].y = fma(aexp[r] * v[r][c].y, v[r][c].y, h[c].y);
        }
      }
    }
  }
}

template <int CPT, int R, int MODE, bool KEEP = false, bool VEC = false>
__global__ __launch_bounds__(WG) void k_objective(ObjArgs a) {
  if (a.gate && (*a.gate & 3) != a.gate_want) return;
  if (a.gate2 && *a.gate2 != a.gate2_want) return;
  __shared__ double red[2][8][R];
  const int tid = threadIdx.x;
  const int64_t ld2 = a.ldl / 2;
  const d2* __restrict__ L2 = reinterpret_cast<const d2*>(a.L);
  const int64_t nsteps = (a.n + R - 1) / R;
  const int64_t per = (nsteps + a.n_wg - 1) / a.n_wg;
  const int64_t s_beg = (int64_t)blockIdx.x * per;
  int64_t s_end = s_beg + per;
  if (s_end > nsteps) s_end = nsteps;

  d2 z[CPT], g[CPT], h[CPT];
#pragma unroll
  for (int c = 0; c < CPT; ++c) {
    const int64_t col = 2 * ((int64_t)c * WG + tid);
    z[c] = (d2){0.0, 0.0};
    if (MODE != MODE_GEMVT) {
      if (col < a.m) z[c].x = a.z[col];
      if (col + 1 < a.m) z[c].y = a.z[col + 1];
    }
    g[c] = (d2){0.0, 0.0};
    h[c] = (d2){0.0, 0.0};
  }
  double loss = 0.0;
  int any_over = 0;
  const double capv = a.cap ? *a.cap : __builtin_inf();
  __shared__ double fstage[KEEP ? (MLN_FSTAGE + WG) : 1];
  const int64_t fbase = s_beg * R;
  d2 va[R][CPT], vb[R][CPT];
  const int64_t s_last = s_end - 1;
  double pa[2][R], pb[2][R];
  const RowMap rm = row_map(a);
  const unsigned lim = a.seg_cols > 0 ? (unsigned)(a.seg_left / 2) : (unsigned)ld2;
  auto lik = [&](int64_t r0, double (&pv)[2][R]) { if (VEC) load_lik_vec<R>(a, r0, tid, pv); else load_lik<R>(a, r0, pv); };
  constexpr bool PRE = KEEP || (VEC && (MODE == MODE_OBJ || MODE == MODE_OBJ_HESS));
  if (s_beg < s_end) { load_rows<CPT, R>(L2, ld2, s_beg * R, a.n, tid, va, rm, lim); if (PRE) lik(s_beg * R, pa); }
  for (int64_t s = s_beg; s < s_end; s += 2) {
    const int64_t s1 = (s + 1 < s_end) ? s + 1 : s_last, s2 = (s + 2 < s_end) ? s + 2 : s_last;
    load_rows<CPT, R>(L2, ld2, s1 * R, a.n, tid, vb, rm, lim);
    if (PRE) lik(s1 * R, pb);
    process_rows<CPT, R, MODE, KEEP, VEC>(a, s * R, a.n, tid, 0, va, z, g, h, loss, red, fstage, fbase, pa, capv, any_over);
    load_rows<CPT, R>(L2, ld2, s2 * R, a.n, tid, va, rm, lim);
    if (PRE) lik(s2 * R, pa);
    if (s + 1 < s_end) process_rows<CPT, R, MODE, KEEP, VEC>(a, (s + 1) * R, a.n, tid, 1, vb, z, g, h, loss, red, fstage, fbase, pb, capv, any_over);
  }
  if (any_over && a.over_flag) atomicAdd(a.over_flag, any_over);
  if (KEEP) {
    __syncthreads();
    double* fo = a.f_keep[1 - *a.f_slot];
    const int64_t r_beg = s_beg * R, r_end = (s_end * R < a.n) ? s_end * R : a.n;
    for (int64_t i = r_beg + tid; i < r_end; i += WG) fo[i] = fstage[i - r_beg];
  }
  if (MODE != MODE_FONLY) {
    double* pg = a.part_grad + (int64_t)blockIdx.x * a.m_pad;
    const int64_t store_lim = a.seg_cols > 0 ? ((a.seg_cols + 1) & ~(int64_t)1) : a.m_pad;
    const double osc = a.out_scale != 0.0 ? a.out_scale : 1.0;
#pragma unroll
    for (int c = 0; c < CPT; ++c) {
      const int64_t col = 2 * ((int64_t)c * WG + tid);
      if (col < store_lim) *reinterpret_cast<d2*>(pg + col) = (d2){g[c].x * osc, g[c].y * osc};
    }
    if (MODE == MODE_OBJ_HESS) {
      double* ph = a.part_hess + (int64_t)blockIdx.x * a.m_pad;
#pragma unroll
      for (int c = 0; c < CPT; ++c) {
        const int64_t col = 2 * ((int64_t)c * WG + tid);
        if (col < a.m_pad) *reinterpret_cast<d2*>(ph + col) = h[c];
      }
    }
    if (VEC) {
#pragma unroll
      for (int off = 32; off > 0; off >>= 1) loss += __shfl_xor(loss, off, 64);
    }
    if (tid == 0 && a.part_loss) a.part_loss[blockIdx.x] = loss * osc;
  }
}

typedef float f4 __attribute__((ext_vector_type(4)));

template <int CQ, int R, int NW>
__device__ __forceinline__ void load_rows32(const f4* __restrict__ L4, int64_t ld4, int64_t row, int64_t row_end,
                                            unsigned tid, f4 (&v)[R][CQ], const RowMap rm) {
#pragma unroll
  for (int r = 0; r < R; ++r) {
    const bool rok = (row + r) < row_end;
    const f4* rowp = L4 + rm(rok ? (row + r) : row) * ld4;
#pragma unroll
    for (int c = 0; c < CQ; ++c) {
      unsigned off = (unsigned)c * (64 * NW) + tid;
      off = (off < (unsigned)ld4) ? off : (unsigned)ld4 - 1u;
      v[r][c] = __builtin_nontemporal_load(rowp + off);
    }
  }
}

template <bool FIXED>
__device__ __forceinline__ double elem32(float v) {
  return FIXED ? (double)__float_as_uint(v) : (double)v;
}

template <int CQ, int R, bool GEMVT, bool KEEP, int NW, bool FIXED, bool VEC = false>
__device__ __forceinline__ void process_rows32(const ObjArgs& a, int64_t row, int64_t row_end, int tid, int par,
                                               const f4 (&v)[R][CQ], const double (&z)[CQ][4], double (&g)[CQ][4],
                                               double& loss, double (*red)[NW][R], double* fstage, int64_t fbase,
                                               const double (&pv)[2][R], double capv, double ecap, int& any_over) {
  double coef[R], dot[R];
  const RowMap rm = row_map(a);
  if (GEMVT) {
#pragma unroll
    for (int r = 0; r < R; ++r) coef[r] = (row + r < row_end) ? a.weights[rm(row + r)] : 0.0;
#pragma unroll
    for (int r = 0; r < R; ++r) {
#pragma unroll
      for (int c = 0; c < CQ; ++c) {
        g[c][0] = fma(coef[r], elem32<FIXED>(v[r][c].x), g[c][0]);
        g[c][1] = fma(coef[r], elem32<FIXED>(v[r][c].y), g[c][1]);
        g[c][2] = fma(coef[r], elem32<FIXED>(v[r][c].z), g[c][2]);
        g[c][3] = fma(coef[r], elem32<FIXED>(v[r][c].w), g[c][3]);
      }
    }
    return;
  }
  if constexpr (VEC) {
#pragma unroll
    for (int r = 0; r < R; ++r) {
      double s = 0.0;
#pragma unroll
      for (int c = 0; c < CQ; ++c) {
        s = fma(elem32<FIXED>(v[r][c].x), z[c][0], s);
        s = fma(elem32<FIXED>(v[r][c].y), z[c][1], s);
        s = fma(elem32<FIXED>(v[r][c].z), z[c][2], s);
        s = fma(elem32<FIXED>(v[r][c].w), z[c][3], s);
      }
      dot[r] = s;
    }
    const int wave = tid >> 6, lane = tid & 63;
    constexpr int GRP = 64 / R;
    const double tot = transposed_wave_sum<R>(dot, lane);
    if ((lane & (GRP - 1)) == 0) red[par][wave][lane / GRP] = tot;
    __syncthreads();
    const int rl = lane < R ? lane : R - 1;
    double sr = 0.0;
#pragma unroll
    for (int w = 0; w < NW; ++w) sr += red[par][w][rl];
    const bool rok = lane < R && (row + rl) < row_end;
    const double f = sr + a.mu;
    const double Vi = pv[0][0];
    const double tt = f + Vi;
    const bool over = tt > capv;
    const double ex = exp(over ? capv : tt);
    const double dc = over ? (tt - capv) : 0.0;
    const double e = rok ? ex * fma(dc, fma(0.5, dc, 1.0), 1.0) : 0.0;
    const double cf = rok ? (over ? fma(ex, dc, ex - 1.0) : ex - 1.0) : 0.0;
    if (wave == 0 && rok) loss -= (f + pv[1][0]) - e;
    any_over += (wave == 0 && rok && over) ? 1 : 0;
    if (KEEP) lds_store_f64(fstage, (wave == 0 && rok) ? (int)(row + rl - fbase) : (MLN_FSTAGE + tid), f);
#pragma unroll
    for (int r = 0; r < R; ++r) coef[r] = read_lane_f64(cf, r);
  } else {
#pragma unroll
  for (int r = 0; r < R; ++r) {
    double s = 0.0;
#pragma unroll
    for (int c = 0; c < CQ; ++c) {
      s = fma(elem32<FIXED>(v[r][c].x), z[c][0], s);
      s = fma(elem32<FIXED>(v[r][c].y), z[c][1], s);
      s = fma(elem32<FIXED>(v[r][c].z), z[c][2], s);
      s = fma(elem32<FIXED>(v[r][c].w), z[c][3], s);
    }
#pragma unroll
    for (int off = 32; off > 0; off >>= 1) s += __shfl_xor(s, off, 64);
    dot[r] = s;
  }
  const int wave = tid >> 6;
  if ((tid & 63) == 0) {
#pragma unroll
    for (int r = 0; r < R; ++r) red[par][wave][r] = dot[r];
  }
  __syncthreads();
#pragma unroll
  for (int r = 0; r < R; ++r) {
    double s = 0.0;
#pragma unroll
    for (int w = 0; w < NW; ++w) s += red[par][w][r];
    const bool rok = (row + r) < row_end;
    const double f = s + a.mu;
    const double Vi = KEEP ? pv[0][r] : (rok ? a.V[rm(row + r)] : 0.0);
    const double tt = f + Vi;
    const bool over = tt > capv;
    const double ex = exp(over ? capv : tt);
    const double dc = over ? (tt - capv) : 0.0;
    const double e = rok ? ex * fma(dc, fma(0.5, dc, 1.0), 1.0) : 0.0;
    coef[r] = rok ? (over ? fma(ex, dc, ex - 1.0) : ex - 1.0) : 0.0;
    if (KEEP) { if (tid == 0 && rok) loss -= (f + pv[1][r]) - e; }
    else if (tid == 0 && rok) loss -= (f + a.Vdr[rm(row + r)]) - e;
    any_over += (tid == 0 && rok && over) ? 1 : 0;
    if (KEEP) lds_store_f64(fstage, (tid == 0 && rok) ? (int)(row + r - fbase) : (MLN_FSTAGE + tid), f);
  }
  }
#pragma unroll
  for (int r = 0; r < R; ++r) {
#pragma unroll
    for (int c = 0; c < CQ; ++c) {
      g[c][0] = fma(coef[r], elem32<FIXED>(v[r][c].x), g[c][0]);
      g[c][1] = fma(coef[r], elem32<FIXED>(v[r][c].y), g[c][1]);
      g[c][2] = fma(coef[r], elem32<FIXED>(v[r][c].z), g[c][2]);
      g[c][3] = fma(coef[r], elem32<FIXED>(v[r][c].w), g[c][3]);
    }
  }
}

template <int CQ, int R, bool GEMVT = false, bool KEEP = false, int NW = 8, bool FIXED = false, bool VEC = false>
__global__ __launch_bounds__(64 * NW) void k_objective32(ObjArgs a) {
  if (a.gate && (*a.gate & 3) != a.gate_want) return;
  if (a.gate2 && *a.gate2 != a.gate2_want) return;
  constexpr int WG = 64 * NW;
  __shared__ double red[2][NW][R];
  const int tid = threadIdx.x;
  const int64_t ld4 = a.ldl / 4;
  const f4* __restrict__ L4 = reinterpret_cast<const f4*>(a.L32);
  const int64_t nsteps = (a.n + R - 1) / R;
  const int64_t per = (nsteps + a.n_wg - 1) / a.n_wg;
  const int64_t s_beg = (int64_t)blockIdx.x * per;
  int64_t s_end = s_beg + per;
  if (s_end > nsteps) s_end = nsteps;
  double z[CQ][4], g[CQ][4];
#pragma unroll
  for (int c = 0; c < CQ; ++c)
#pragma unroll
    for (int e = 0; e < 4; ++e) {
      const int64_t col = 4 * ((int64_t)c * WG + tid) + e;
      z[c][e] = (!GEMVT && col < a.m) ? a.z[col] * (FIXED ? 0x1p-32 : 1.0) : 0.0;
      g[c][e] = 0.0;
    }
  double loss = 0.0;
  int any_over = 0;
  const double capv = a.cap ? *a.cap : __builtin_inf();
  const double ecap = exp(capv);
  __shared__ double fstage[KEEP ? (MLN_FSTAGE + WG) : 1];
  const int64_t fbase = s_beg * R;
  f4 va[R][CQ], vb[R][CQ];
  const int64_t s_last = s_end - 1;
  double pa[2][R], pb[2][R];
  const RowMap rm = row_map(a);
  constexpr bool PRE = KEEP || (VEC && !GEMVT);
  auto lik = [&](int64_t r0, double (&pv)[2][R]) { if (VEC) load_lik_vec<R>(a, r0, tid, pv); else load_lik<R>(a, r0, pv); };
  if (s_beg < s_end) { load_rows32<CQ, R, NW>(L4, ld4, s_beg * R, a.n, tid, va, rm); if (PRE) lik(s_beg * R, pa); }
  for (int64_t s = s_beg; s < s_end; s += 2) {
    const int64_t s1 = (s + 1 < s_end) ? s + 1 : s_last, s2 = (s + 2 < s_end) ? s + 2 : s_last;
    load_rows32<CQ, R, NW>(L4, ld4, s1 * R, a.n, tid, vb, rm);
    if (PRE) lik(s1 * R, pb);
    process_rows32<CQ, R, GEMVT, KEEP, NW, FIXED, VEC>(a, s * R, a.n, tid, 0, va, z, g, loss, red, fstage, fbase, pa, capv, ecap, any_over);
    load_rows32<CQ, R, NW>(L4, ld4, s2 * R, a.n, tid, va, rm);
    if (PRE) lik(s2 * R, pa);
    if (s + 1 < s_end) process_rows32<CQ, R, GEMVT, KEEP, NW, FIXED, VEC>(a, (s + 1) * R, a.n, tid, 1, vb, z, g, loss, red, fstage, fbase, pb, capv, ecap, any_over);
  }
  if (any_over && a.over_flag) atomicAdd(a.over_flag, any_over);
  if (KEEP) {
    __syncthreads();
    double* fo = a.f_keep[1 - *a.f_slot];
    const int64_t r_beg = s_beg * R, r_end = (s_end * R < a.n) ? s_end * R : a.n;
    for (int64_t i = r_beg + tid; i < r_end; i += WG) fo[i] = fstage[i - r_beg];
  }
  double* pg = a.part_grad + (int64_t)blockIdx.x * a.m_pad;
#pragma unroll
  for (int c = 0; c < CQ; ++c) {
    const int64_t col = 4 * ((int64_t)c * WG + tid);
    if (col < a.m_pad) {
      const double sc = (FIXED ? 0x1p-32 : 1.0) * (a.out_scale != 0.0 ? a.out_scale : 1.0);
      *reinterpret_cast<d2*>(pg + col) = (d2){g[c][0] * sc, g[c][1] * sc};
      *reinterpret_cast<d2*>(pg + col + 2) = (d2){g[c][2] * sc, g[c][3] * sc};
    }
  }
  if (VEC) {
#pragma unroll
    for (int off = 32; off > 0; off >>= 1) loss += __shfl_xor(loss, off, 64);
  }
  if (tid == 0 && a.part_loss) a.part_loss[blockIdx.x] = loss * (a.out_scale != 0.0 ? a.out_scale : 1.0);
}

template <int CQ, int R, int NW, bool VEC = false>
int launch_f32_nw(mln_ctx* ctx, const ObjArgs& a) {
  const dim3 grid((unsigned)a.n_wg), block(64 * NW);
  if (a.l32_fixed) {
    if (a.weights) hipLaunchKernelGGL((k_objective32<CQ, R, true, false, NW, true>), grid, block, 0, ctx->stream, a);
    else hipLaunchKernelGGL((k_objective32<CQ, R, false, false, NW, true, VEC>), grid, block, 0, ctx->stream, a);
  } else {
    if (a.weights) hipLaunchKernelGGL((k_objective32<CQ, R, true, false, NW>), grid, block, 0, ctx->stream, a);
    else hipLaunchKernelGGL((k_objective32<CQ, R, false, false, NW, false, VEC>), grid, block, 0, ctx->stream, a);
  }
  MLN_HIP(ctx, hipGetLastError());
  return MLN_OK;
}

template <int CQ, int R, bool VEC = false>
int launch_f32(mln_ctx* ctx, const ObjArgs& a) {
  const int64_t ld4 = a.ldl / 4;
  int nw = (int)((ld4 + 64 * CQ - 1) / (64 * CQ));
  if (nw <= 6) return launch_f32_nw<CQ, R, 6, VEC>(ctx, a);
  if (nw == 7) return launch_f32_nw<CQ, R, 7, VEC>(ctx, a);
  return launch_f32_nw<CQ, R, 8, VEC>(ctx, a);
}

__global__ void k_to_f32(const double* __restrict__ src, float* __restrict__ dst, int64_t count) {
  const int64_t i = 2 * ((int64_t)blockIdx.x * blockDim.x + threadIdx.x);
  if (i + 1 < count) {
    const d2 v = __builtin_nontemporal_load(reinterpret_cast<const d2*>(src + i));
    dst[i] = (float)v.x;
    dst[i + 1] = (float)v.y;
  } else if (i < count) {
    dst[i] = (float)src[i];
  }
}

__global__ __launch_bounds__(256) void k_reduce_obj(ObjArgs a, double* __restrict__ out_loss,
                                                    double* __restrict__ out_grad, int with_hess) {
  if (a.gate && (*a.gate & 3) == MLN_GATE_DONE) return;
  __shared__ double red[2][16][16];
  const int c = threadIdx.x & 15, grp = threadIdx.x >> 4;
  const int64_t j = (int64_t)blockIdx.x * 16 + c;
  double s = 0.0, t = 0.0;
  if (j < a.m) {
    const int per = (a.n_wg + 15) / 16;
    const int w0 = grp * per, w1 = (w0 + per < a.n_wg) ? (w0 + per) : a.n_wg;
#pragma unroll 4
    for (int w = w0; w < w1; ++w) s += a.part_grad[(int64_t)w * a.m_pad + j];
    if (with_hess)
      for (int w = w0; w < w1; ++w) t += a.part_hess[(int64_t)w * a.m_pad + j];
  }
  red[0][grp][c] = s;
  red[1][grp][c] = t;
  __syncthreads();
  if (grp == 0 && j < a.m) {
    double gs = 0.0, hs = 0.0;
#pragma unroll
    for (int q = 0; q < 16; ++q) { gs += red[0][q][c]; hs += red[1][q][c]; }
    out_grad[j] = gs;
    if (with_hess) out_grad[a.m + j] = hs;
  }
  if (blockIdx.x == 0 && threadIdx.x < 64) {
    double l = 0.0;
    if (a.part_loss)
      for (int w = threadIdx.x; w < a.n_wg; w += 64) l += a.part_loss[w];
#pragma unroll
    for (int off = 32; off > 0; off >>= 1) l += __shfl_xor(l, off, 64);
    if (threadIdx.x == 0) {
      out_loss[0] = l;
      if (a.over_flag) { out_loss[1] = (double)*a.over_flag; *a.over_flag = 0; }
    }
  }
}

__global__ __launch_bounds__(256) void k_gemv_rows(const double* __restrict__ M, int64_t ld, int64_t rows,
                                                   int64_t cols, const double* __restrict__ x,
                                                   double* __restrict__ y) {
  const int lane = threadIdx.x & 63;
  const int64_t r = (int64_t)blockIdx.x * 4 + (threadIdx.x >> 6);
  if (r >= rows) return;
  const d2* __restrict__ row = reinterpret_cast<const d2*>(M + r * ld);
  const d2* __restrict__ xv = reinterpret_cast<const d2*>(x);
  const int64_t pairs = cols / 2;
  double s0 = 0.0, s1 = 0.0;
  for (int64_t p = lane; p < pairs; p += 64) {
    const d2 a = row[p], b = xv[p];
    s0 = fma(a.x, b.x, s0);
    s1 = fma(a.y, b.y, s1);
  }
  double s = s0 + s1;
  if ((cols & 1) && lane == 0) s = fma(M[r * ld + cols - 1], x[cols - 1], s);
#pragma unroll
  for (int off = 32; off > 0; off >>= 1) s += __shfl_xor(s, off, 64);
  if (lane == 0) y[r] = s;
}

__global__ __launch_bounds__(256) void k_gemv_rows_tri(GemvTri g) {
  if (g.gate && (*g.gate & 3) == MLN_GATE_DONE) return;
  const int lane = threadIdx.x & 63;
  const int64_t r = (int64_t)blockIdx.x * 4 + (threadIdx.x >> 6);
  if (r >= g.rows) return;
  const int64_t i = r % g.blk;
  const int64_t c_lo = (g.upper == 1) ? (i & ~(int64_t)1) : 0, c_hi = g.upper ? g.ncol : i + 1;
  const double* __restrict__ rowp = g.M + r * g.ld;
  double s0 = 0.0, s1 = 0.0;
  const int nseg = g.mseg ? 2 : 1;
  for (int sg = 0; sg < nseg; ++sg) {
    const double* __restrict__ rb = rowp + sg * g.mseg;
    const double* __restrict__ xb = g.x + sg * g.xseg;
    const d2* __restrict__ row = reinterpret_cast<const d2*>(rb);
    const d2* __restrict__ xv = reinterpret_cast<const d2*>(xb);
    const d2* __restrict__ xa = (g.xadd && sg == 0) ? reinterpret_cast<const d2*>(g.xadd) : nullptr;
    int64_t p = c_lo / 2 + lane;
    const int64_t p_end = c_hi / 2;
    double t0 = 0.0, t1 = 0.0, t2 = 0.0, t3 = 0.0, t4 = 0.0, t5 = 0.0;
    for (; p + 192 < p_end; p += 256) {
      const d2 a0 = row[p], a1 = row[p + 64], a2 = row[p + 128], a3 = row[p + 192];
      d2 b0 = xv[p], b1 = xv[p + 64], b2 = xv[p + 128], b3 = xv[p + 192];
      if (xa) {
        const d2 c0 = xa[p], c1 = xa[p + 64], c2 = xa[p + 128], c3 = xa[p + 192];
        b0.x += c0.x; b0.y += c0.y; b1.x += c1.x; b1.y += c1.y; b2.x += c2.x; b2.y += c2.y; b3.x += c3.x; b3.y += c3.y;
      }
      s0 = fma(a0.x, b0.x, s0); s1 = fma(a0.y, b0.y, s1);
      t0 = fma(a1.x, b1.x, t0); t1 = fma(a1.y, b1.y, t1);
      t2 = fma(a2.x, b2.x, t2); t3 = fma(a2.y, b2.y, t3);
      t4 = fma(a3.x, b3.x, t4); t5 = fma(a3.y, b3.y, t5);
    }
    for (; p < p_end; p += 64) {
      const d2 a = row[p];
      d2 b = xv[p];
      if (xa) { const d2 c = xa[p]; b.x += c.x; b.y += c.y; }
      s0 = fma(a.x, b.x, s0);
      s1 = fma(a.y, b.y, s1);
    }
    s0 += (t0 + t2) + t4;
    s1 += (t1 + t3) + t5;
    if ((c_hi & 1) && lane == 0) s0 = fma(rb[c_hi - 1], xb[c_hi - 1] + (xa ? g.xadd[c_hi - 1] : 0.0), s0);
  }
  double s = s0 + s1;
#pragma unroll
  for (int off = 32; off > 0; off >>= 1) s += __shfl_xor(s, off, 64);
  if (lane == 0) {
    if (g.y2 && r >= g.blk) g.y2[r - g.blk] = s;
    else g.y[r] = s;
  }
}

template <int CPT, int R, bool VEC = false>
int launch_mode(mln_ctx* ctx, const ObjArgs& a, int mode) {
  dim3 grid((unsigned)a.n_wg), block(WG);
  switch (mode) {
    case MODE_OBJ:
      if (a.f_slot) hipLaunchKernelGGL((k_objective<CPT, R, MODE_OBJ, true, VEC>), grid, block, 0, ctx->stream, a);
      else hipLaunchKernelGGL((k_objective<CPT, R, MODE_OBJ, false, VEC>), grid, block, 0, ctx->stream, a);
      break;
    case MODE_OBJ_HESS: hipLaunchKernelGGL((k_objective<CPT, R, MODE_OBJ_HESS, false, VEC>), grid, block, 0, ctx->stream, a); break;
    case MODE_GEMVT: hipLaunchKernelGGL((k_objective<CPT, R, MODE_GEMVT>), grid, block, 0, ctx->stream, a); break;
    default: hipLaunchKernelGGL((k_objective<CPT, R, MODE_FONLY>), grid, block, 0, ctx->stream, a); break;
  }
  MLN_HIP(ctx, hipGetLastError());
  return MLN_OK;
}

}

int launch_to_f32(mln_ctx* ctx, const double* src, float* dst, int64_t count) {
  if (count <= 0) return MLN_OK;
  const int64_t blocks = (count / 2 + 256) / 256;
  hipLaunchKernelGGL(k_to_f32, dim3((unsigned)blocks), dim3(256), 0, ctx->stream, src, dst, count);
  MLN_HIP(ctx, hipGetLastError());
  return MLN_OK;
}

int objective_max_m() { return 65535; }
static constexpr int64_t MLN_SEG = 8192;

namespace {

__global__ __launch_bounds__(256) void k_lik_rows(const double* __restrict__ f, const double* __restrict__ V,
                                                  const double* __restrict__ Vdr, int64_t n, double* __restrict__ coef,
                                                  double* __restrict__ part_loss, int n_part) {
  __shared__ double red[4];
  const int64_t per = (n + n_part - 1) / n_part;
  const int64_t r0 = (int64_t)blockIdx.x * per, r1 = (r0 + per < n) ? r0 + per : n;
  double l = 0.0;
  for (int64_t i = r0 + threadIdx.x; i < r1; i += 256) {
    const double e = exp(f[i] + V[i]);
    coef[i] = e - 1.0;
    l -= (f[i] + Vdr[i]) - e;
  }
#pragma unroll
  for (int off = 32; off > 0; off >>= 1) l += __shfl_xor(l, off, 64);
  if ((threadIdx.x & 63) == 0) red[threadIdx.x >> 6] = l;
  __syncthreads();
  if (threadIdx.x == 0) part_loss[blockIdx.x] = (red[0] + red[1]) + (red[2] + red[3]);
}

}

int launch_objective(mln_ctx* ctx, const ObjArgs& a);

static int launch_objective_wide(mln_ctx* ctx, const ObjArgs& a) {
  if (a.gate || a.part_hess || a.L32 || (a.row_stride > 1)) {
    mln_set_error(ctx, "objective: this mode is not available beyond 8192 landmarks");
    return MLN_ERR_UNSUPPORTED;
  }
  const bool gemvt = a.weights != nullptr, fonly = !gemvt && a.f_out != nullptr;
  DevBuf<double> ftmp;
  double* coef = nullptr;
  const int64_t n1 = a.n > 0 ? a.n : 1;
  if (!gemvt && !fonly) {
    MLN_TRY(ftmp.alloc(ctx, (size_t)n1 * 2, "ftmp"));
    coef = ftmp + n1;
  }
  int rc = MLN_OK;
  if (!gemvt) {
    for (int64_t c0 = 0; c0 < a.m && rc == MLN_OK; c0 += MLN_SEG) {
      ObjArgs s = a;
      s.L = a.L + c0; s.m = std::min<int64_t>(MLN_SEG, a.m - c0); s.z = a.z + c0;
      s.ldl = a.ldl; s.m_pad = a.m_pad;
      s.weights = nullptr; s.part_hess = nullptr; s.part_loss = nullptr;
      s.f_out = fonly ? a.f_out : ftmp;
      s.f_accum = c0 > 0 ? 1 : 0;
      s.f_slot = nullptr;
      s.seg_cols = s.m; s.seg_left = a.ldl - c0;
      rc = launch_objective(ctx, s);
    }
  }
  if (rc == MLN_OK && !gemvt && !fonly) {
    hipLaunchKernelGGL(k_lik_rows, dim3((unsigned)a.n_wg), dim3(256), 0, ctx->stream, ftmp, a.V, a.Vdr, a.n, coef,
                       a.part_loss, a.n_wg);
    if (hipGetLastError() != hipSuccess) rc = MLN_ERR_HIP;
  }
  if (rc == MLN_OK && !fonly) {
    for (int64_t c0 = 0; c0 < a.m && rc == MLN_OK; c0 += MLN_SEG) {
      ObjArgs s = a;
      s.L = a.L + c0; s.m = std::min<int64_t>(MLN_SEG, a.m - c0);
      s.weights = gemvt ? a.weights : coef;
      s.part_grad = a.part_grad + c0; s.part_hess = nullptr; s.part_loss = nullptr; s.f_out = nullptr; s.f_slot = nullptr;
      s.seg_cols = s.m; s.seg_left = a.ldl - c0;
      rc = launch_objective(ctx, s);
    }
  }
  if (ftmp) (void)hipStreamSynchronize(ctx->stream);
  return rc;
}

int objective_max_m_one_pass() { return (int)MLN_SEG; }
bool objective_can_keep_f(int64_t n, int n_wg) { return n_wg > 0 && (n + n_wg - 1) / n_wg + 16 <= MLN_FSTAGE; }

int launch_objective(mln_ctx* ctx, const ObjArgs& a) {
  if (a.ldl % 2 != 0) { mln_set_error(ctx, "objective: leading dimension of L must be even"); return MLN_ERR_ARG; }
  if (a.seg_cols == 0 && a.m > MLN_SEG) return launch_objective_wide(ctx, a);
  int mode = MODE_OBJ;
  if (a.weights) mode = MODE_GEMVT;
  else if (a.f_out) mode = MODE_FONLY;
  else if (a.part_hess) mode = MODE_OBJ_HESS;
  if (a.L32 && (mode == MODE_OBJ || mode == MODE_GEMVT) && a.ldl % 4 == 0) {
    const int cq = (int)((a.ldl / 4 + WG - 1) / WG);
    const bool vec32 = mode == MODE_OBJ;
    switch (cq) {
      case 1: return vec32 ? launch_f32<1, 8, true>(ctx, a) : launch_f32<1, 8>(ctx, a);
      case 2: return vec32 ? launch_f32<2, 4, true>(ctx, a) : launch_f32<2, 4>(ctx, a);
      case 3:
        return vec32 ? launch_f32<3, 2, true>(ctx, a) : launch_f32<3, 3>(ctx, a);
      default: return launch_f32<4, 2>(ctx, a);
    }
  }
  const int64_t pairs = a.seg_cols > 0 ? (a.seg_cols + 1) / 2 : a.ldl / 2;
  const int cpt = (int)((pairs + WG - 1) / WG);
  const bool vec = mode == MODE_OBJ || mode == MODE_OBJ_HESS;
  switch (cpt) {
    case 1: return vec ? launch_mode<1, 8, true>(ctx, a, mode) : launch_mode<1, 8>(ctx, a, mode);
    case 2: return vec ? launch_mode<2, 8, true>(ctx, a, mode) : launch_mode<2, 5>(ctx, a, mode);
    case 3: return vec ? launch_mode<3, 4, true>(ctx, a, mode) : launch_mode<3, 3>(ctx, a, mode);
    case 4: return launch_mode<4, 2>(ctx, a, mode);
    case 5: return launch_mode<5, 2>(ctx, a, mode);
    case 6: return launch_mode<6, 2>(ctx, a, mode);
    case 7:
    case 8: return launch_mode<8, 1>(ctx, a, mode);
    default:
      mln_set_error(ctx, "objective: m > 8192 landmarks is not supported by this build");
      return MLN_ERR_UNSUPPORTED;
  }
}

int launch_gemv_rows(mln_ctx* ctx, const double* M, int64_t ld, int64_t rows, int64_t cols, const double* x,
                     double* y) {
  if (rows <= 0) return MLN_OK;
  if ((ld & 1) || ((uintptr_t)M & 15) || ((uintptr_t)x & 15)) { mln_set_error(ctx, "gemv_rows: unaligned operands"); return MLN_ERR_ARG; }
  hipLaunchKernelGGL(k_gemv_rows, dim3((unsigned)((rows + 3) / 4)), dim3(256), 0, ctx->stream, M, ld, rows, cols, x, y);
  MLN_HIP(ctx, hipGetLastError());
  return MLN_OK;
}

int launch_gemv_tri(mln_ctx* ctx, const GemvTri& g) {
  if (g.rows <= 0) return MLN_OK;
  if ((g.ld & 1) || (g.mseg & 1) || (g.xseg & 1) || ((uintptr_t)g.M & 15) || ((uintptr_t)g.x & 15)) {
    mln_set_error(ctx, "gemv_rows_tri: unaligned operands");
    return MLN_ERR_ARG;
  }
  hipLaunchKernelGGL(k_gemv_rows_tri, dim3((unsigned)((g.rows + 3) / 4)), dim3(256), 0, ctx->stream, g);
  MLN_HIP(ctx, hipGetLastError());
  return MLN_OK;
}

int launch_gemv_rows_tri(mln_ctx* ctx, const double* M, int64_t ld, int64_t rows, const double* x, double* y,
                         int upper, int64_t blk, int64_t ncol, int64_t seg) {
  GemvTri g{M, ld, rows, x, y, nullptr, upper, blk, ncol, seg, seg, nullptr};
  return launch_gemv_tri(ctx, g);
}

int launch_reduce_obj2(mln_ctx* ctx, const ObjArgs& a, double* out_loss, double* out_grad) {
  hipLaunchKernelGGL(k_reduce_obj, dim3((unsigned)((a.m + 15) / 16)), dim3(256), 0, ctx->stream, a, out_loss, out_grad,
                     a.part_hess ? 1 : 0);
  MLN_HIP(ctx, hipGetLastError());
  return MLN_OK;
}

int launch_reduce_obj(mln_ctx* ctx, const ObjArgs& a, double* out) { return launch_reduce_obj2(ctx, a, out, out + 1); }
```

### mellon_amd/csrc/precond_rebuild.h

```cpp
#pragma once
#include "mln_core.h"

struct RebuildSelection {
  int64_t rows = 0;
  DevBuf<int64_t> idx;
  DevBuf<double> scale;
  double w_max = 1.0;
  double c = 0.0;
  double sum_a = 0.0;
  void reset() { idx.reset(); scale.reset(); rows = 0; }
};

int rebuild_select_rows(mln_ctx* ctx, const double* f_dev, const double* V_dev, int64_t n, int64_t row0,
                        double target_rows_global, uint64_t seed, RebuildSelection* out, double cap = 1e300);
int launch_gather_scale_rows(mln_ctx* ctx, const double* A, int64_t ld, const int64_t* idx, const double* scale,
                             int64_t rows, double* R);
```

### mellon_amd/csrc/precond_rebuild.hip

```cpp
#include <algorithm>
#include <cmath>
#include <vector>

#include "mln_internal.h"
#include "precond_rebuild.h"

namespace {

constexpr int SB = 1024;

__device__ __forceinline__ double hash_unit(uint64_t i) {
  uint64_t z = i + 0x9e3779b97f4a7c15ull;
  z = (z ^ (z >> 30)) * 0xbf58476d1ce4e5b9ull;
  z = (z ^ (z >> 27)) * 0x94d049bb133111ebull;
  z ^= z >> 31;
  return (double)(z >> 11) * 0x1p-53;
}

__device__ __forceinline__ double block_sum256(double v, double* red) {
#pragma unroll
  for (int off = 32; off > 0; off >>= 1) v += __shfl_xor(v, off, 64);
  __syncthreads();
  if ((threadIdx.x & 63) == 0) red[threadIdx.x >> 6] = v;
  __syncthreads();
  return (red[0] + red[1]) + (red[2] + red[3]);
}

__global__ __launch_bounds__(256) void k_weights(const double* __restrict__ f, const double* __restrict__ V, int64_t n,
                                                 double* __restrict__ a, double* __restrict__ part_sum,
                                                 double* __restrict__ part_max, double cap) {
  __shared__ double red[4];
  double s = 0.0, mx = 0.0;
  for (int64_t i = (int64_t)blockIdx.x * 256 + threadIdx.x; i < n; i += (int64_t)gridDim.x * 256) {
    double t = f[i] + V[i];
    t = fmin(fmax(t, -700.0), fmin(600.0, cap));
    const double v = exp(t);
    a[i] = v;
    s += v;
    mx = fmax(mx, v);
  }
  s = block_sum256(s, red);
#pragma unroll
  for (int off = 32; off > 0; off >>= 1) mx = fmax(mx, __shfl_xor(mx, off, 64));
  __shared__ double redm[4];
  if ((threadIdx.x & 63) == 0) redm[threadIdx.x >> 6] = mx;
  __syncthreads();
  if (threadIdx.x == 0) {
    part_sum[blockIdx.x] = s;
    part_max[blockIdx.x] = fmax(fmax(redm[0], redm[1]), fmax(redm[2], redm[3]));
  }
}

__global__ __launch_bounds__(256) void k_expected(const double* __restrict__ a, int64_t n, double c,
                                                  double* __restrict__ part, double* __restrict__ part_slope) {
  __shared__ double red[4];
  double s = 0.0, sl = 0.0;
  for (int64_t i = (int64_t)blockIdx.x * 256 + threadIdx.x; i < n; i += (int64_t)gridDim.x * 256) {
    const double v = a[i], ca = c * v;
    s += fmin(1.0, ca);
    sl += (ca < 1.0) ? v : 0.0;
  }
  s = block_sum256(s, red);
  sl = block_sum256(sl, red);
  if (threadIdx.x == 0) { part[blockIdx.x] = s; part_slope[blockIdx.x] = sl; }
}

__global__ void k_fold2(const double* __restrict__ p0, const double* __restrict__ p1, int n_part, double* __restrict__ out) {
  if (blockIdx.x == 0 && threadIdx.x < 2) {
    const double* p = threadIdx.x == 0 ? p0 : p1;
    double s = 0.0;
    for (int i = 0; i < n_part; ++i) s += p[i];
    out[threadIdx.x] = s;
  }
}

__global__ void k_fold(const double* __restrict__ part, int n_part, int take_max, double* __restrict__ out) {
  if (threadIdx.x == 0 && blockIdx.x == 0) {
    double s = 0.0;
    for (int i = 0; i < n_part; ++i) s = take_max ? fmax(s, part[i]) : s + part[i];
    out[0] = s;
  }
}

__device__ __forceinline__ bool picked(double a, double c, int64_t gidx, uint64_t seed) {
  const double p = fmin(1.0, c * a);
  return hash_unit((uint64_t)gidx * 0x2545f4914f6cdd1dull + seed) < p;
}

__global__ __launch_bounds__(256) void k_select_count(const double* __restrict__ a, int64_t n, double c, int64_t row0,
                                                      uint64_t seed, int* __restrict__ counts) {
  __shared__ int tot;
  if (threadIdx.x == 0) tot = 0;
  __syncthreads();
  const int64_t base = (int64_t)blockIdx.x * SB;
  int mine = 0;
  for (int j = threadIdx.x; j < SB; j += 256) {
    const int64_t i = base + j;
    if (i < n && picked(a[i], c, row0 + i, seed)) ++mine;
  }
  atomicAdd(&tot, mine);
  __syncthreads();
  if (threadIdx.x == 0) counts[blockIdx.x] = tot;
}

__global__ __launch_bounds__(64) void k_select_write(const double* __restrict__ a, int64_t n, double c, int64_t row0,
                                                     uint64_t seed, const int64_t* __restrict__ offsets, double inv_wmax,
                                                     int64_t* __restrict__ idx, double* __restrict__ scale) {
  const int64_t base = (int64_t)blockIdx.x * SB;
  int64_t out = offsets[blockIdx.x];
  for (int j0 = 0; j0 < SB; j0 += 64) {
    const int64_t i = base + j0 + threadIdx.x;
    const bool on = i < n && picked(a[i], c, row0 + i, seed);
    const uint64_t mask = __ballot(on);
    if (on) {
      const int pos = __popcll(mask & ((1ull << threadIdx.x) - 1ull));
      idx[out + pos] = i;
      const double w = fmax(a[i], 1.0 / c);
      scale[out + pos] = sqrt(w * inv_wmax);
    }
    out += __popcll(mask);
  }
}

typedef double d2 __attribute__((ext_vector_type(2)));

__global__ __launch_bounds__(256) void k_gather_scale(const double* __restrict__ A, int64_t ld, const int64_t* __restrict__ idx,
                                                      const double* __restrict__ scale, int64_t rows, double* __restrict__ R) {
  const int64_t k = blockIdx.x;
  if (k >= rows) return;
  const d2* __restrict__ src = reinterpret_cast<const d2*>(A + idx[k] * ld);
  d2* __restrict__ dst = reinterpret_cast<d2*>(R + k * ld);
  const double s = scale[k];
  for (int64_t p = threadIdx.x; p < ld / 2; p += 256) {
    const d2 v = src[p];
    dst[p] = (d2){v.x * s, v.y * s};
  }
}

}

int rebuild_select_rows(mln_ctx* ctx, const double* f_dev, const double* V_dev, int64_t n, int64_t row0,
                        double target_rows_global, uint64_t seed, RebuildSelection* out, double cap) {
  *out = RebuildSelection();
  const int nb = 256;
  DevBuf<double> a, part, part2, scal;
  const int64_t n1 = n > 0 ? n : 1;
  MLN_TRY(a.alloc(ctx, (size_t)n1, "a"));
  if (part.alloc(ctx, nb, "part") != MLN_OK || part2.alloc(ctx, nb, "part2") != MLN_OK || scal.alloc(ctx, 16, "scal") != MLN_OK) {
    mln_set_error(ctx, "preconditioner rebuild: out of device memory");
    return MLN_ERR_HIP;
  }
  hipLaunchKernelGGL(k_weights, dim3(nb), dim3(256), 0, ctx->stream, f_dev, V_dev, n, a.get(), part.get(), part2.get(), cap);
  hipLaunchKernelGGL(k_fold, dim3(1), dim3(64), 0, ctx->stream, part.get(), nb, 0, scal.get());
  hipLaunchKernelGGL(k_fold, dim3(1), dim3(64), 0, ctx->stream, part2.get(), nb, 1, scal + 1);
  int rc = comm_allreduce(ctx, scal, 1);
  if (rc != MLN_OK) return rc;
  const int nr = ctx->n_ranks > 1 ? ctx->n_ranks : 1;
  DevBuf<double> gathered;
  MLN_TRY(gathered.alloc(ctx, nr, "gathered"));
  rc = (nr > 1) ? comm_allgather(ctx, scal + 1, gathered, 1)
                : (hipMemcpyAsync(gathered, scal + 1, sizeof(double), hipMemcpyDeviceToDevice, ctx->stream) == hipSuccess ? MLN_OK : MLN_ERR_HIP);
  std::vector<double> h(nr + 1);
  if (rc == MLN_OK && (hipMemcpyAsync(h.data(), gathered, sizeof(double) * nr, hipMemcpyDeviceToHost, ctx->stream) != hipSuccess ||
                       hipMemcpyAsync(h.data() + nr, scal, sizeof(double), hipMemcpyDeviceToHost, ctx->stream) != hipSuccess ||
                       hipStreamSynchronize(ctx->stream) != hipSuccess)) rc = MLN_ERR_HIP;
  gathered.reset();
  if (rc != MLN_OK) return rc;
  double a_max = 0.0;
  for (int r = 0; r < nr; ++r) a_max = std::max(a_max, h[r]);
  const double sum_a = h[nr];
  if (!(sum_a > 0.0) || !std::isfinite(sum_a)) { mln_set_error(ctx, "preconditioner rebuild: degenerate weights"); return MLN_ERR_ARG; }
  double c = target_rows_global / sum_a;
  for (int it = 0; it < 14; ++it) {
    hipLaunchKernelGGL(k_expected, dim3(nb), dim3(256), 0, ctx->stream, a.get(), n, c, part.get(), part2.get());
    hipLaunchKernelGGL(k_fold2, dim3(1), dim3(64), 0, ctx->stream, part.get(), part2.get(), nb, scal + 2);
    rc = comm_allreduce(ctx, scal + 2, 2);
    double gs[2] = {0.0, 0.0};
    if (rc == MLN_OK && (hipMemcpyAsync(gs, scal + 2, sizeof(gs), hipMemcpyDeviceToHost, ctx->stream) != hipSuccess ||
                         hipStreamSynchronize(ctx->stream) != hipSuccess)) rc = MLN_ERR_HIP;
    if (rc != MLN_OK) return rc;
    const double cnt = gs[0], slope = gs[1];
    if (!(cnt > 0.0)) break;
    if (std::fabs(target_rows_global / cnt - 1.0) < 1e-3) break;
    if (!(slope > 0.0)) break;
    const double c_new = c + (target_rows_global - cnt) / slope;
    if (!(c_new > c) || !std::isfinite(c_new)) break;
    c = c_new;
    if (c * a_max > 1e12) break;
  }
  const double w_max = std::max(a_max, 1.0 / c);
  const int64_t n_blk = (n + SB - 1) / SB;
  DevBuf<int> counts;
  DevBuf<int64_t> offsets;
  if (n_blk > 0) {
    MLN_TRY(counts.alloc(ctx, (size_t)n_blk, "counts"));
    MLN_TRY(offsets.alloc(ctx, (size_t)n_blk, "offsets"));
    hipLaunchKernelGGL(k_select_count, dim3((unsigned)n_blk), dim3(256), 0, ctx->stream, a.get(), n, c, row0, seed, counts.get());
    std::vector<int> hc((size_t)n_blk);
    std::vector<int64_t> ho((size_t)n_blk);
    if (hipMemcpyAsync(hc.data(), counts, sizeof(int) * (size_t)n_blk, hipMemcpyDeviceToHost, ctx->stream) != hipSuccess ||
        hipStreamSynchronize(ctx->stream) != hipSuccess) rc = MLN_ERR_HIP;
    int64_t total = 0;
    for (int64_t b = 0; b < n_blk && rc == MLN_OK; ++b) { ho[(size_t)b] = total; total += hc[(size_t)b]; }
    if (rc == MLN_OK && total > 0) {
      rc = out->idx.alloc(ctx, (size_t)total, "idx");
      if (rc == MLN_OK) rc = out->scale.alloc(ctx, (size_t)total, "scale");
      if (rc == MLN_OK && hipMemcpyAsync(offsets, ho.data(), sizeof(int64_t) * (size_t)n_blk, hipMemcpyHostToDevice, ctx->stream) != hipSuccess)
        rc = MLN_ERR_HIP;
      if (rc == MLN_OK) {
        hipLaunchKernelGGL(k_select_write, dim3((unsigned)n_blk), dim3(64), 0, ctx->stream, a.get(), n, c, row0, seed, offsets.get(),
                           1.0 / w_max, out->idx.get(), out->scale.get());
        if (hipStreamSynchronize(ctx->stream) != hipSuccess) rc = MLN_ERR_HIP;
      }
    }
    counts.reset();
    offsets.reset();
    if (rc != MLN_OK) { (void)hipStreamSynchronize(ctx->stream); out->reset(); mln_set_error(ctx, "preconditioner rebuild: row selection failed"); return rc; }
    out->rows = total;
  }
  out->w_max = w_max; out->c = c; out->sum_a = sum_a;
  (void)hipStreamSynchronize(ctx->stream);
  return MLN_OK;
}

int launch_gather_scale_rows(mln_ctx* ctx, const double* A, int64_t ld, const int64_t* idx, const double* scale,
                             int64_t rows, double* R) {
  if (rows <= 0) return MLN_OK;
  if (ld & 1) { mln_set_error(ctx, "gather rows: odd leading dimension"); return MLN_ERR_ARG; }
  hipLaunchKernelGGL(k_gather_scale, dim3((unsigned)rows), dim3(256), 0, ctx->stream, A, ld, idx, scale, rows, R);
  MLN_HIP(ctx, hipGetLastError());
  return MLN_OK;
}
```

### mellon_amd/csrc/solver.h

```cpp
#pragma once
#include "mln_core.h"

enum { MLN_SOLVE_FIRST = 0, MLN_SOLVE_LS = 1, MLN_SOLVE_REEVAL = 2, MLN_SOLVE_RESUME = 3 };

struct SolverState {
  int gate;
  int mode;
  int status;
  int it, n_eval, n_eval32, ls;
  int k, head;
  int maxiter, maxcor, maxls;
  int m;
  int f_slot;
  int f_valid;
  int corr;
  int n_anchor;
  int use_corr;
  double ftol, gtol, ftol32;
  double prior_const;
  double fx, t, gd;
  double cap;
  double cap_step;
  int over_acc;
  double cap0;
  double boost_fall;
  double t0, boost;
  double corr_k;
  double sub_tol;
  int sub_max_evals;
  int gate_full;
  int n_eval_sub;
  int sub_level, n_sub_levels;
  int rebuild_armed;
  int it_resume;
  double over_many;
  double over_cnt_acc;
  int it_full;
  int resume_keep_pairs;
  int gate_after_pause;
  double rebuild_tol;
  double switch_t0;
  double gap_tol;
  double dec_prev, dec_prev2;
  double start_cap;
  int n_shrink;
  int revert_after;
  int it_at_resume;
  int pause_reason;
};

struct SolverBuffers {
  SolverState* st;
  double *u, *g, *un, *gn, *d;
  double *S, *Y;
  double *rho, *yy;
  double* c;
  const double* z;
  const double* z2;
  const double* lik;
  const double* over;
  int64_t ld;
  double* trace;
};

int launch_solver_init(mln_ctx* ctx, const SolverBuffers& b, const SolverState& init, const double* u0);
int launch_solver_step(mln_ctx* ctx, const SolverBuffers& b, int m);
int launch_solver_resume(mln_ctx* ctx, const SolverBuffers& b, int gate, int pairs_dropped, int revert_after = 0, int rearm = -1);
int launch_solver_resume_plain32(mln_ctx* ctx, const SolverBuffers& b, int gate, int m, int pairs_dropped = 0);
int launch_solver_refresh_pairs(mln_ctx* ctx, const SolverBuffers& b, int maxcor);
```

### mellon_amd/csrc/solver.hip

```cpp
#include <cmath>

#include "objective.h"
#include "solver.h"

namespace {

constexpr int ST = 512;

__device__ __forceinline__ double wave_sum(double v) {
#pragma unroll
  for (int off = 32; off > 0; off >>= 1) v += __shfl_xor(v, off, 64);
  return v;
}

__device__ __forceinline__ double block_sum(double v, double* red) {
  v = wave_sum(v);
  __syncthreads();
  if ((threadIdx.x & 63) == 0) red[threadIdx.x >> 6] = v;
  __syncthreads();
  double s = 0.0;
#pragma unroll
  for (int w = 0; w < ST / 64; ++w) s += red[w];
  return s;
}

__device__ __forceinline__ void block_sum3(double& a, double& b, double& c, double (*red3)[ST / 64]) {
  a = wave_sum(a); b = wave_sum(b); c = wave_sum(c);
  __syncthreads();
  if ((threadIdx.x & 63) == 0) { red3[0][threadIdx.x >> 6] = a; red3[1][threadIdx.x >> 6] = b; red3[2][threadIdx.x >> 6] = c; }
  __syncthreads();
  double s0 = 0.0, s1 = 0.0, s2 = 0.0;
#pragma unroll
  for (int w = 0; w < ST / 64; ++w) { s0 += red3[0][w]; s1 += red3[1][w]; s2 += red3[2][w]; }
  a = s0; b = s1; c = s2;
}

__device__ __forceinline__ double block_max(double v, double* red) {
#pragma unroll
  for (int off = 32; off > 0; off >>= 1) v = fmax(v, __shfl_xor(v, off, 64));
  __syncthreads();
  if ((threadIdx.x & 63) == 0) red[threadIdx.x >> 6] = v;
  __syncthreads();
  double s = 0.0;
#pragma unroll
  for (int w = 0; w < ST / 64; ++w) s = fmax(s, red[w]);
  return s;
}

template <int EPT>
__global__ __launch_bounds__(ST) void k_solver_step(SolverBuffers b) {
  SolverState* st = b.st;
  if ((st->gate & 3) == MLN_GATE_DONE) return;
  __shared__ double red[ST / 64];
  __shared__ double red3[3][ST / 64];
  __shared__ double alpha_s[64];
  const int tid = threadIdx.x;
  const int m = st->m;
  const int64_t ld = b.ld;
  bool on[EPT];
  int idx[EPT];
#pragma unroll
  for (int e = 0; e < EPT; ++e) { idx[e] = tid + ST * e; on[e] = idx[e] < m; }
  double u[EPT], g[EPT], un[EPT], gn[EPT], d[EPT];
  double zz = 0.0;
#pragma unroll
  for (int e = 0; e < EPT; ++e) {
    u[e] = on[e] ? b.u[idx[e]] : 0.0;
    g[e] = on[e] ? b.g[idx[e]] : 0.0;
    un[e] = on[e] ? b.un[idx[e]] : 0.0;
    gn[e] = on[e] ? b.gn[idx[e]] : 0.0;
    d[e] = on[e] ? b.d[idx[e]] : 0.0;
    const double zv = on[e] ? b.z[idx[e]] : 0.0;
    const double z2v = b.z2 ? (on[e] ? b.z2[idx[e]] : 0.0) : zv;
    zz = fma(zv, z2v, zz);
  }
  zz = block_sum(zz, red);
  double fn = b.lik[0] + 0.5 * zz + st->prior_const;
  const bool resume = st->mode == MLN_SOLVE_RESUME;
  const bool phaseA = st->gate == MLN_GATE_F32, phaseC = st->gate == MLN_GATE_F32C, phaseS = st->gate == MLN_GATE_SUB;
  const bool phase32 = phaseA || phaseC;
  const bool approx = phase32 || phaseS;
  if (phaseC) {
    double cu = 0.0;
#pragma unroll
    for (int e = 0; e < EPT; ++e) {
      const double cv = on[e] ? b.c[idx[e]] : 0.0;
      cu = fma(cv, un[e], cu);
      gn[e] += cv;
    }
    fn += block_sum(cu, red) + st->corr_k;
  }
  int mode = st->mode, it = st->it, n_eval = st->n_eval + (resume ? 0 : 1), n_eval32 = st->n_eval32 + ((phase32 && !resume) ? 1 : 0);
  int n_eval_sub = st->n_eval_sub + ((phaseS && !resume) ? 1 : 0), it_full = st->it_full, sub_level = st->sub_level;
  bool next_level = false;
  int ls = st->ls, k = st->k, head = st->head, status = st->status, gate = st->gate;
  double fx = st->fx, t = st->t, gd = st->gd, corr_k = st->corr_k, t0 = st->t0, cap = st->cap;
  double dec_prev = st->dec_prev, dec_prev2 = st->dec_prev2;
  const bool after_switch = mode == MLN_SOLVE_REEVAL && !phaseS && !phaseC && st->n_eval_sub > 0 && st->it_full == 0;
  bool recap = false;
  if (mode != MLN_SOLVE_LS && !resume) t0 = 1.0;
  int f_slot = st->f_slot, f_valid = st->f_valid, corr = st->corr, n_anchor = st->n_anchor;
  int over_acc = st->over_acc;
  double over_cnt_acc = st->over_cnt_acc;
  const double over_cnt_now = (cap < 1e300 && b.over) ? b.over[0] : 0.0;
  const int over_now = over_cnt_now > 0.0 ? 1 : 0;
  if (b.trace && tid == 0 && !resume) {
    double* tr = b.trace + 4 * ((n_eval - 1) & 511);
    tr[0] = fn; tr[1] = (mode == MLN_SOLVE_LS) ? t : 0.0; tr[2] = (double)mode; tr[3] = (double)(gate + 16 * st->sub_level);
  }
  bool to_head = false, reeval = false, done = false, verify = false, pause = false, shrink = false;
  int pause_reason = 1;
  if (resume) {
    to_head = true;
    if (!st->resume_keep_pairs) { k = 0; head = 0; }
    dec_prev = 0.0; dec_prev2 = 0.0;
  } else if (mode == MLN_SOLVE_FIRST && (!isfinite(fn) || fn > st->start_cap) && st->n_shrink < 64) {
#pragma unroll
    for (int e = 0; e < EPT; ++e) { u[e] *= 0.5; un[e] = u[e]; }
    shrink = true;
  } else if (mode != MLN_SOLVE_LS) {
    if (mode == MLN_SOLVE_REEVAL && !phase32 && st->use_corr) {
      verify = corr != 0;
      if (n_anchor < 4) {
        double dcu = 0.0;
#pragma unroll
        for (int e = 0; e < EPT; ++e) {
          const double dc = gn[e] - g[e];
          const double cv = (corr && on[e]) ? b.c[idx[e]] : 0.0;
          if (on[e]) b.c[idx[e]] = cv + dc;
          dcu = fma(dc, u[e], dcu);
        }
        dcu = block_sum(dcu, red);
        corr_k = (corr ? corr_k : 0.0) + (fn - fx) - dcu;
        corr = 1; ++n_anchor;
        gate = MLN_GATE_F32C;
      } else {
        corr = 0;
      }
    }
    fx = fn;
    over_acc = over_now; over_cnt_acc = over_cnt_now;
    f_slot ^= 1; f_valid = approx ? 0 : 1;
#pragma unroll
    for (int e = 0; e < EPT; ++e) g[e] = gn[e];
    if (mode == MLN_SOLVE_REEVAL && !approx && st->rebuild_armed && corr && n_anchor == 1 && st->use_corr) pause = true;
    else to_head = true;
  } else {
    ++ls;
    const bool ok = isfinite(fn) && fn <= fx + 1e-4 * t * gd;
    if (ok) {
      double sy = 0.0, ss = 0.0, yy = 0.0;
      double sv[EPT], yv[EPT];
#pragma unroll
      for (int e = 0; e < EPT; ++e) {
        sv[e] = un[e] - u[e];
        yv[e] = gn[e] - g[e];
        sy = fma(sv[e], yv[e], sy); ss = fma(sv[e], sv[e], ss); yy = fma(yv[e], yv[e], yy);
      }
      block_sum3(sy, ss, yy, red3);
      if (st->boost > 0.0) {
        double sl = 0.0;
#pragma unroll
        for (int e = 0; e < EPT; ++e) sl = fma(gn[e], d[e], sl);
        sl = block_sum(sl, red);
        t0 = (ls == 1 && t >= 1.0 && gd < 0.0 && sl / gd > st->boost && (fx - fn) > st->boost_fall * fabs(fx)) ? fmin(2.0 * t, 16.0) : 1.0;
      }
      const double f_old = fx;
#pragma unroll
      for (int e = 0; e < EPT; ++e) { u[e] = un[e]; g[e] = gn[e]; }
      fx = fn;
      over_acc = over_now; over_cnt_acc = over_cnt_now;
      f_slot ^= 1; f_valid = approx ? 0 : 1;
      if (!phaseS) ++it_full;
      if (sy > 1e-10 * sqrt(ss * yy)) {
        int slot;
        if (k < st->maxcor) { slot = (head + k) % st->maxcor; ++k; }
        else { slot = head; head = (head + 1) % st->maxcor; }
#pragma unroll
        for (int e = 0; e < EPT; ++e)
          if (on[e]) { b.S[slot * ld + idx[e]] = sv[e]; b.Y[slot * ld + idx[e]] = yv[e]; }
        if (tid == 0) { b.rho[slot] = 1.0 / sy; b.yy[slot] = yy; }
        __threadfence_block();
        __syncthreads();
      }
      ++it;
      const double fscale = fmax(fmax(fabs(f_old), fabs(fx)), 1.0);
      const double dec_now = f_old - fx;
      const bool slow = (f_old - fx) <= st->rebuild_tol * fscale && (f_old - fx) > st->ftol * fscale;
      if (cap < 1e300 && over_acc && it >= 3 && slow) { cap += st->cap_step; recap = true; }
      const bool revert = st->revert_after > 0 && st->it_at_resume >= 0 && !phaseS && it - st->it_at_resume > st->revert_after &&
                          (f_old - fx) > st->ftol * fscale;
      if (revert) {
        pause = true; pause_reason = 2;
      } else if (phaseS) {
        if (it >= 4 && ((f_old - fx) <= st->sub_tol * fscale || n_eval_sub >= st->sub_max_evals)) { reeval = true; next_level = true; } else to_head = true;
      } else if (st->rebuild_armed > 0 && st->it_resume < 0 && !phase32 && !recap && it_full >= 2 && (slow || (it_full >= 4 && st->over_many > 0.0 && over_cnt_acc >= st->over_many && isfinite(fx)))) {
        pause = true;
      } else if (st->rebuild_armed > 0 && st->it_resume >= 0 && !approx && !recap && it - st->it_resume >= 6 && dec_prev > 0.0 &&
                 dec_prev2 > 0.0 && dec_now > 0.5 * dec_prev && dec_prev > 0.5 * dec_prev2 && dec_now > st->ftol * fscale) {
        pause = true;
      } else if (phaseA && st->rebuild_armed && it_full >= 2 && (f_old - fx) <= st->rebuild_tol * fscale) {
        reeval = true;
      } else if (phaseA) {
        if ((f_old - fx) <= st->ftol32 * fscale) reeval = true; else to_head = true;
      } else if ((f_old - fx) <= st->ftol * fscale) {
        if (phaseC) reeval = true; else { status = 0; done = true; }
      } else {
        const double dec = f_old - fx;
        bool small_gap = false;
        if (st->gap_tol > 0.0 && !phaseS && dec_prev > 0.0 && dec_prev2 > 0.0 && dec < 0.25 * dec_prev && dec_prev < 0.25 * dec_prev2 &&
            dec_prev2 <= 1e-4 * fscale) {
          const double r = dec / dec_prev;
          small_gap = dec * r / (1.0 - r) <= st->gap_tol * fscale;
        }
        if (small_gap) { if (phaseC) reeval = true; else { status = 0; done = true; } }
        else to_head = true;
      }
      if (!phaseS) { dec_prev2 = dec_prev; dec_prev = f_old - fx; }
    } else if (isfinite(fn) && fabs(fn - fx) <= st->ftol * fmax(fmax(fabs(fx), fabs(fn)), 1.0)) {
      if (approx && !(phaseC && f_valid)) { reeval = true; next_level = phaseS; } else { status = 0; done = true; }
    } else if (ls >= st->maxls) {
      if (approx && !(phaseC && f_valid)) { reeval = true; next_level = phaseS; }
      else { status = phaseC ? 0 : 2; done = true; }
    } else {
      if (isfinite(fn)) {
        const double tq = -gd * t * t / (2.0 * (fn - fx - gd * t));
        t = fmin(fmax(tq, 0.1 * t), 0.5 * t);
      } else {
        t *= 0.1;
      }
#pragma unroll
      for (int e = 0; e < EPT; ++e) un[e] = fma(t, d[e], u[e]);
    }
  }
  if (to_head) {
    double gm = 0.0;
#pragma unroll
    for (int e = 0; e < EPT; ++e) gm = fmax(gm, fabs(g[e]));
    gm = block_max(gm, red);
    if (!(gm > st->gtol)) {
      if (approx) { reeval = true; next_level = phaseS; } else { status = 0; done = true; }
    } else if (it >= st->maxiter) {
      status = 1; done = true;
    } else {
      double q[EPT];
#pragma unroll
      for (int e = 0; e < EPT; ++e) q[e] = g[e];
      double sv[EPT], yv[EPT], sn[EPT], yn[EPT];
      auto load_pair = [&](int j, double (&s_)[EPT], double (&y_)[EPT]) {
        const int slot = (head + j) % st->maxcor;
#pragma unroll
        for (int e = 0; e < EPT; ++e) {
          s_[e] = on[e] ? b.S[slot * ld + idx[e]] : 0.0;
          y_[e] = on[e] ? b.Y[slot * ld + idx[e]] : 0.0;
        }
      };
      if (k > 0) load_pair(k - 1, sv, yv);
      for (int j = k - 1; j >= 0; --j) {
        const int slot = (head + j) % st->maxcor;
        if (j > 0) load_pair(j - 1, sn, yn); else load_pair(0, sn, yn);
        double acc = 0.0;
#pragma unroll
        for (int e = 0; e < EPT; ++e) acc = fma(sv[e], q[e], acc);
        const double a = b.rho[slot] * block_sum(acc, red);
        if (tid == 0) alpha_s[j] = a;
#pragma unroll
        for (int e = 0; e < EPT; ++e) { q[e] = fma(-a, yv[e], q[e]); sv[e] = sn[e]; yv[e] = yn[e]; }
      }
      if (k > 0) {
        const int last = (head + k - 1) % st->maxcor;
        const double gamma = 1.0 / (b.rho[last] * b.yy[last]);
#pragma unroll
        for (int e = 0; e < EPT; ++e) q[e] *= gamma;
      }
      __syncthreads();
      for (int j = 0; j < k; ++j) {
        const int slot = (head + j) % st->maxcor;
        if (j + 1 < k) load_pair(j + 1, sn, yn);
        double acc = 0.0;
#pragma unroll
        for (int e = 0; e < EPT; ++e) acc = fma(yv[e], q[e], acc);
        const double beta = b.rho[slot] * block_sum(acc, red);
        const double c = alpha_s[j] - beta;
#pragma unroll
        for (int e = 0; e < EPT; ++e) { q[e] = fma(sv[e], c, q[e]); sv[e] = sn[e]; yv[e] = yn[e]; }
      }
      double acc = 0.0;
#pragma unroll
      for (int e = 0; e < EPT; ++e) { d[e] = -q[e]; acc = fma(g[e], d[e], acc); }
      gd = block_sum(acc, red);
      if (!(gd < 0.0)) {
        k = 0; head = 0;
        acc = 0.0;
#pragma unroll
        for (int e = 0; e < EPT; ++e) { d[e] = -g[e]; acc = fma(g[e], g[e], acc); }
        gd = -block_sum(acc, red);
      }
      if (verify && -0.5 * gd <= st->ftol * fmax(fabs(fx), 1.0)) { status = 0; done = true; }
      t = t0;
      if (after_switch && st->switch_t0 > 0.0) t = st->switch_t0;
      if (k == 0 && !resume) {
        double g1 = 0.0;
#pragma unroll
        for (int e = 0; e < EPT; ++e) g1 += fabs(g[e]);
        g1 = block_sum(g1, red);
        t = fmin(1.0, 1.0 / g1);
      }
      ls = 0;
      mode = MLN_SOLVE_LS;
#pragma unroll
      for (int e = 0; e < EPT; ++e) un[e] = fma(t, d[e], u[e]);
    }
  }
  if (reeval) {
    cap = phaseS ? st->cap0 : (phase32 ? __builtin_inf() : cap);
    if (phaseS && next_level && sub_level + 1 < st->n_sub_levels) { ++sub_level; gate = MLN_GATE_SUB; }
    else gate = phaseS ? st->gate_full : MLN_GATE_F64;
    mode = MLN_SOLVE_REEVAL;
#pragma unroll
    for (int e = 0; e < EPT; ++e) un[e] = u[e];
  }
  if (done && status == 0 && cap < 1e300 && over_acc && !approx) { done = false; cap += st->cap_step; recap = true; }
  if (recap && !reeval && !done) {
    mode = MLN_SOLVE_REEVAL;
#pragma unroll
    for (int e = 0; e < EPT; ++e) un[e] = u[e];
  }
  if (pause) { if (tid == 0) st->gate_after_pause = gate; gate = MLN_GATE_PAUSE; }
  if (done) gate = MLN_GATE_DONE;
#pragma unroll
  for (int e = 0; e < EPT; ++e)
    if (on[e]) { b.u[idx[e]] = u[e]; b.g[idx[e]] = g[e]; b.un[idx[e]] = un[e]; b.d[idx[e]] = d[e]; }
  if (tid == 0) {
    st->gate = gate; st->mode = mode; st->status = status; st->it = it; st->n_eval = n_eval; st->n_eval32 = n_eval32;
    st->ls = ls; st->k = k; st->head = head; st->fx = fx; st->t = t; st->gd = gd;
    st->f_slot = f_slot; st->f_valid = f_valid;
    st->corr = corr; st->n_anchor = n_anchor; st->corr_k = corr_k; st->t0 = t0; st->cap = cap;
    st->n_eval_sub = n_eval_sub; st->it_full = it_full; st->sub_level = sub_level;
    st->dec_prev = dec_prev; st->dec_prev2 = dec_prev2;
    st->over_acc = over_acc; st->over_cnt_acc = over_cnt_acc;
    if (shrink) st->n_shrink += 1;
    if (pause) { st->rebuild_armed = (pause_reason == 1 && st->rebuild_armed > 0) ? st->rebuild_armed - 1 : 0; st->pause_reason = pause_reason; st->it_at_resume = -1; }
  }
}

__global__ void k_solver_init(SolverBuffers b, SolverState init, const double* __restrict__ u0) {
  const int i = blockIdx.x * blockDim.x + threadIdx.x;
  if (i < init.m) {
    const double v = u0[i];
    b.u[i] = v; b.un[i] = v; b.g[i] = 0.0; b.gn[i] = 0.0; b.d[i] = 0.0;
  }
  if (i == 0) *b.st = init;
}

__global__ __launch_bounds__(512) void k_solver_refresh_pairs(SolverBuffers b) {
  __shared__ double red[ST / 64];
  const SolverState* st = b.st;
  const int slot = blockIdx.x;
  if (slot >= st->maxcor) return;
  double acc = 0.0;
  for (int i = threadIdx.x; i < st->m; i += ST) { const double v = b.Y[slot * b.ld + i]; acc = fma(v, v, acc); }
  acc = block_sum(acc, red);
  if (threadIdx.x == 0) b.yy[slot] = acc;
}

__global__ void k_solver_resume(SolverBuffers b, int gate, int pairs_dropped, int revert_after, int rearm) {
  if (threadIdx.x == 0 && blockIdx.x == 0) {
    SolverState* st = b.st;
    st->gate = gate;
    st->mode = MLN_SOLVE_RESUME;
    if (pairs_dropped) { st->k = 0; st->head = 0; }
    st->resume_keep_pairs = pairs_dropped ? 0 : 1;
    st->revert_after = revert_after;
    st->it_at_resume = revert_after > 0 ? st->it : -1;
    st->it_resume = st->it;
    if (rearm >= 0) st->rebuild_armed = rearm;
    st->pause_reason = 0;
  }
}

__global__ void k_solver_resume_plain32(SolverBuffers b, int gate, int m, int pairs_dropped) {
  const int i = blockIdx.x * blockDim.x + threadIdx.x;
  if (i < m) b.un[i] = b.u[i];
  if (i == 0) {
    SolverState* st = b.st;
    st->gate = gate;
    st->mode = MLN_SOLVE_REEVAL;
    if (pairs_dropped) { st->k = 0; st->head = 0; }
    st->corr = 0; st->n_anchor = 0; st->corr_k = 0.0;
    st->revert_after = 0; st->it_at_resume = -1; st->pause_reason = 0;
    st->rebuild_armed = 0; st->it_resume = st->it;
  }
}

}

int launch_solver_resume_plain32(mln_ctx* ctx, const SolverBuffers& b, int gate, int m, int pairs_dropped) {
  hipLaunchKernelGGL(k_solver_resume_plain32, dim3((unsigned)((m + 255) / 256)), dim3(256), 0, ctx->stream, b, gate, m, pairs_dropped);
  MLN_HIP(ctx, hipGetLastError());
  return MLN_OK;
}

int launch_solver_refresh_pairs(mln_ctx* ctx, const SolverBuffers& b, int maxcor) {
  hipLaunchKernelGGL(k_solver_refresh_pairs, dim3((unsigned)maxcor), dim3(ST), 0, ctx->stream, b);
  MLN_HIP(ctx, hipGetLastError());
  return MLN_OK;
}

int launch_solver_resume(mln_ctx* ctx, const SolverBuffers& b, int gate, int pairs_dropped, int revert_after, int rearm) {
  hipLaunchKernelGGL(k_solver_resume, dim3(1), dim3(64), 0, ctx->stream, b, gate, pairs_dropped, revert_after, rearm);
  MLN_HIP(ctx, hipGetLastError());
  return MLN_OK;
}

int launch_solver_init(mln_ctx* ctx, const SolverBuffers& b, const SolverState& init, const double* u0) {
  hipLaunchKernelGGL(k_solver_init, dim3((unsigned)((init.m + 255) / 256)), dim3(256), 0, ctx->stream, b, init, u0);
  MLN_HIP(ctx, hipGetLastError());
  return MLN_OK;
}

int launch_solver_step(mln_ctx* ctx, const SolverBuffers& b, int m) {
  const int ept = (m + ST - 1) / ST;
  const dim3 grid(1), block(ST);
#define MLN_STEP(E) case E: hipLaunchKernelGGL(k_solver_step<E>, grid, block, 0, ctx->stream, b); break;
  switch (ept) {
    MLN_STEP(1) MLN_STEP(2) MLN_STEP(3) MLN_STEP(4) MLN_STEP(5) MLN_STEP(6) MLN_STEP(7) MLN_STEP(8)
    MLN_STEP(9) MLN_STEP(10) MLN_STEP(11) MLN_STEP(12) MLN_STEP(13) MLN_STEP(14) MLN_STEP(15) MLN_STEP(16)
    default: mln_set_error(ctx, "solver: m > 8192 is not supported by this build"); return MLN_ERR_UNSUPPORTED;
  }
#undef MLN_STEP
  MLN_HIP(ctx, hipGetLastError());
  return MLN_OK;
}
```

Before: 7.479 million.

## Add importance-sampled tail phase to the MAP solver using a subset of rows

Adds a new solver phase in which, after a preconditioner rebuild, the objective is evaluated on an importance-sampled subset of rows with per-row weights. A correction term anchors the subset objective to the full objective, and full f64 re-evaluations verify progress. If verification fails, a guard reverts to the saved anchor point. The aim is to cut the cost of the many full-data objective passes late in the L-BFGS solve, in exchange for extra solver-state complexity and a risk of more iterations or fallbacks. It also adds a diagnostic row-subset objective entry point and new stage-time counters.

```diff
diff --git a/include/mellon_hip.h b/include/mellon_hip.h
--- a/include/mellon_hip.h
+++ b/include/mellon_hip.h
@@ -211,6 +211,9 @@
                            int32_t kmode, double beta, int32_t any_size, double* out);
 int mln_diag_gram_i8(mln_ctx* ctx, const double* A, int64_t rows, int64_t m, double* out, int32_t reps, double* ms_out);
 int mln_diag_overlap(mln_ctx* ctx, int64_t n, int64_t m, int32_t d, int64_t gram_rows, double* out );
+int mln_diag_objective_rows(mln_fit* fit, const double* z, int64_t count, int64_t first, int64_t stride,
+                            const int64_t* rows, const double* row_w, double out_scale, double* loss, double* grad,
+                            double* f_rows);
 
 int mln_predict_covariance(mln_ctx* ctx, const mln_kernel_desc* cov, const double* xnew, int64_t n_new,
                            int32_t d, const double* centers, int64_t m, const double* Lf, int32_t diag,
@@ -219,7 +222,7 @@
                                 int32_t d, const double* centers, int64_t m, const double* W, int64_t q,
                                 int32_t diag, double* out);
 
-#define MLN_N_STAGE_TIMES 22
+#define MLN_N_STAGE_TIMES 26
 int mln_stage_times(mln_fit* fit, double* out );
 
 #ifdef __cplusplus
diff --git a/mellon_amd/_lib.py b/mellon_amd/_lib.py
--- a/mellon_amd/_lib.py
+++ b/mellon_amd/_lib.py
@@ -9,7 +9,7 @@
 
 MLN_OK, MLN_ERR_NOT_PD, MLN_ERR_SHAPE, MLN_ERR_HIP, MLN_ERR_RCCL, MLN_ERR_ARG, MLN_ERR_UNSUPPORTED = range(7)
 MLN_UNIQUE_ID_BYTES = 128
-MLN_N_STAGE_TIMES = 22
+MLN_N_STAGE_TIMES = 26
 
 K_MATERN32, K_MATERN52, K_EXPQUAD, K_EXPONENTIAL, K_RATQUAD, K_LINEAR, K_DISTANCE = 1, 2, 3, 4, 5, 6, 7
 OP_LEAF, OP_CONST, OP_ADD, OP_MUL, OP_POW = 0, 1, 2, 3, 4
@@ -122,6 +122,7 @@
     ("mln_stage_times", C.c_int, [_vp, _dp]),
     ("mln_diag_peak", C.c_int, [_vp, _i32, _i64, C.POINTER(_dbl)]),
     ("mln_diag_overlap", C.c_int, [_vp, _i64, _i64, _i32, _i64, _dp]),
+    ("mln_diag_objective_rows", C.c_int, [_vp, _dp, _i64, _i64, _i64, _vp, _dp, _dbl, C.POINTER(_dbl), _dp, _dp]),
     ("mln_diag_gram_i8", C.c_int, [_vp, _vp, _i64, _i64, _vp, _i32, C.POINTER(_dbl)]),
     ("mln_diag_dgemm", C.c_int, [_vp, _i32, _i32, _i64, _i64, _i64, _i32, _i32, _i32, C.POINTER(_dbl)]),
     ("mln_diag_dgemm_compare", C.c_int, [_vp, _i32, _i32, _i64, _i64, _i64, _i32, _i32, _dbl, _i32, C.POINTER(_dbl)]),
@@ -1050,6 +1051,23 @@
                         jitter="ridge")
         return z, loss.value, nev.value, nit.value, st.value
 
+    def objective_rows(self, z, count=None, first=0, stride=1, rows=None, weights=None, out_scale=0.0):
+        z = _f64(z)
+        if rows is not None:
+            rows = np.ascontiguousarray(rows, dtype=np.int64)
+            count = rows.shape[0]
+        if weights is not None:
+            weights = _f64(weights)
+            assert rows is not None and weights.shape[0] == count
+        loss = C.c_double()
+        grad = np.empty(self.m, dtype=np.float64)
+        f = np.empty(int(count), dtype=np.float64)
+        self._check(self.lib.mln_diag_objective_rows(self.handle, z.ctypes.data, int(count), int(first), int(stride),
+                                                     None if rows is None else rows.ctypes.data,
+                                                     None if weights is None else weights.ctypes.data, float(out_scale),
+                                                     C.byref(loss), grad.ctypes.data, f.ctypes.data))
+        return loss.value, grad, f
+
     def transform(self, z, mu, out=None):
         z = _f64(z)
         ret = np.empty(self.n, dtype=np.float64) if out is None else out
@@ -1077,7 +1095,8 @@
                 "objective32_kernel_s", "objective32_launches", "copy32_format", "emulation_excluded_s",
                 "objective_sub_kernel_s", "objective_sub_launches", "objective_sub_stride", "precond_rebuild_s",
                 "precond_rebuilds", "objective_pass_equivalents", "precond_rebuilds_declined", "precond_reverts",
-                "start_halvings", "rank_path"]
+                "start_halvings", "rank_path", "objective_tail_launches", "objective_tail_rows",
+                "objective_tail_kernel_s", "objective_tail_guard"]
         return dict(zip(keys, out.tolist()))
 
 
diff --git a/mellon_amd/csrc/api_internal.h b/mellon_amd/csrc/api_internal.h
--- a/mellon_amd/csrc/api_internal.h
+++ b/mellon_amd/csrc/api_internal.h
@@ -125,6 +125,10 @@
   double build_seconds = 0.0;
   double times_sub = 0.0, times_rebuild = 0.0, sub_pass_equiv = 0.0;
   int evals_sub = 0, n_rebuild = 0;
+  RebuildSelection tail_sel;
+  double times_tail = 0.0;
+  int evals_tail = 0, n_tail_guard = 0;
+  int64_t tail_rows = 0;
   DevBuf<double> dim_ell;
   int dim_k = 0;
   double mu_dim = 0.0, mu_dens = 0.0;
@@ -146,7 +150,8 @@
 int fit_w_from_z(mln_fit* f, const double* z_dev, double* w_dev, const double* z_host = nullptr);
 int fit_cache_pair_from_u(mln_fit* f, const double* u_dev);
 int fit_enqueue_eval(mln_fit* f, const double* u_dev, double* gn_dev, bool use32, const int* gate,
-                            hipEvent_t* ev, const std::vector<int64_t>* sub_strides = nullptr);
+                            hipEvent_t* ev, const std::vector<int64_t>* sub_strides = nullptr,
+                            const RebuildSelection* tail = nullptr);
 int fit_objective_u(mln_fit* f, const double* u, double* loss, double* grad_u, double* z_out,
                            bool use32 = false);
 int fit_solver_alloc(mln_fit* f, int maxcor);
diff --git a/mellon_amd/csrc/api_solve.hip b/mellon_amd/csrc/api_solve.hip
--- a/mellon_amd/csrc/api_solve.hip
+++ b/mellon_amd/csrc/api_solve.hip
@@ -83,6 +83,54 @@
   return MLN_OK;
 }
 
+extern "C" int mln_diag_objective_rows(mln_fit* f, const double* z, int64_t count, int64_t first, int64_t stride,
+                                       const int64_t* rows, const double* row_w, double out_scale, double* loss,
+                                       double* grad, double* f_rows) {
+  if (!f || !z || !loss || !grad || !f_rows || count < 1) return MLN_ERR_ARG;
+  mln_ctx* ctx = f->ctx;
+  if (!f->V) { mln_set_error(ctx, "mln_fit_set_likelihood has not been called"); return MLN_ERR_ARG; }
+  if (f->m > objective_max_m_one_pass() || !objective_can_keep_f(count, f->n_wg)) {
+    mln_set_error(ctx, "mln_diag_objective_rows: shape beyond the one-pass kernel / its f staging");
+    return MLN_ERR_UNSUPPORTED;
+  }
+  bool ok = true;
+  if (rows) { for (int64_t i = 0; i < count; ++i) ok = ok && rows[i] >= 0 && rows[i] < f->n; }
+  else ok = stride >= 1 && first >= 0 && first + (count - 1) * stride < f->n;
+  if (!ok) { mln_set_error(ctx, "mln_diag_objective_rows: rows outside the buffer"); return MLN_ERR_ARG; }
+  MLN_HIP(ctx, hipSetDevice(ctx->device));
+  DevBuf<double> fk, wd;
+  DevBuf<int64_t> rd;
+  DevBuf<int> slot;
+  MLN_TRY(fk.alloc_zeroed(ctx, 2 * (size_t)count, "diag f"));
+  MLN_TRY(slot.alloc_zeroed(ctx, 1, "diag slot"));
+  MLN_HIP(ctx, hipMemcpyAsync(f->d_z, z, sizeof(double) * f->m, hipMemcpyHostToDevice, ctx->stream));
+  ObjArgs a = obj_args(f);
+  a.n = count; a.out_scale = out_scale;
+  a.f_keep[0] = fk; a.f_keep[1] = fk + count; a.f_slot = slot;
+  if (rows) {
+    MLN_TRY(rd.alloc(ctx, (size_t)count, "diag rows"));
+    MLN_HIP(ctx, hipMemcpyAsync(rd, rows, sizeof(int64_t) * (size_t)count, hipMemcpyHostToDevice, ctx->stream));
+    a.rows = rd;
+    if (row_w) {
+      MLN_TRY(wd.alloc(ctx, (size_t)count, "diag weights"));
+      MLN_HIP(ctx, hipMemcpyAsync(wd, row_w, sizeof(double) * (size_t)count, hipMemcpyHostToDevice, ctx->stream));
+      a.row_w = wd;
+    }
+  } else {
+    a.row_first = first; a.row_stride = stride;
+  }
+  int rc = launch_objective(ctx, a);
+  if (rc == MLN_OK) rc = launch_reduce_obj(ctx, a, f->d_out);
+  if (rc == MLN_OK && (hipMemcpyAsync(f->h_out, f->d_out, sizeof(double) * (1 + f->m), hipMemcpyDeviceToHost, ctx->stream) != hipSuccess ||
+                       hipMemcpyAsync(f_rows, fk + count, sizeof(double) * (size_t)count, hipMemcpyDeviceToHost, ctx->stream) != hipSuccess))
+    rc = MLN_ERR_HIP;
+  if (hipStreamSynchronize(ctx->stream) != hipSuccess && rc == MLN_OK) rc = MLN_ERR_HIP;
+  if (rc != MLN_OK) return rc;
+  *loss = f->h_out[0];
+  std::memcpy(grad, f->h_out + 1, sizeof(double) * f->m);
+  return MLN_OK;
+}
+
 extern "C" int mln_transform(mln_fit* f, const double* z, double mu, double* f_out) {
   if (!f || !z || (f->n > 0 && !f_out)) return MLN_ERR_ARG;
   mln_ctx* ctx = f->ctx;
@@ -109,7 +157,7 @@
 }
 
 int fit_enqueue_eval(mln_fit* f, const double* u_dev, double* gn_dev, bool use32, const int* gate,
-                            hipEvent_t* ev, const std::vector<int64_t>* sub_strides) {
+                            hipEvent_t* ev, const std::vector<int64_t>* sub_strides, const RebuildSelection* tail) {
   mln_ctx* ctx = f->ctx;
   const int64_t m = f->m, ld = f->ldl, ld2 = f->ld2;
   if (f->kspace) {
@@ -152,6 +200,17 @@
       as.gate2 = &f->sv.st->sub_level; as.gate2_want = (int)lv;
       MLN_TRY(launch_objective(ctx, as));
     }
+  }
+  if (gate && tail) {
+    ObjArgs at = a;
+    at.n = tail->rows > 0 ? tail->rows : 0;
+    at.rows = tail->rows > 0 ? tail->idx.get() : nullptr;
+    at.row_w = tail->rows > 0 ? tail->scale.get() : nullptr;
+    at.row_stride = 0; at.row_first = 0; at.out_scale = 0.0;
+    at.f_keep[0] = at.f_keep[1] = nullptr; at.f_slot = nullptr;
+    at.gate_want = MLN_GATE_SUB;
+    at.gate2 = &f->sv.st->sub_level; at.gate2_want = MLN_TAIL_LEVEL;
+    MLN_TRY(launch_objective(ctx, at));
   }
   if (ev) MLN_HIP(ctx, hipEventRecord(ev[2], ctx->stream));
   MLN_TRY(launch_reduce_obj2(ctx, a, f->d_zr + ld2 + m, f->d_zr + ld2));
@@ -209,7 +268,7 @@
   if (f->sv_block && f->sv_maxcor >= maxcor) return MLN_OK;
   if (f->sv_block) { MLN_HIP(ctx, hipStreamSynchronize(ctx->stream)); f->sv_block.reset(); }
   const size_t ld = (size_t)f->ldl;
-  const size_t n_dbl = 6 * ld + 2 * (size_t)maxcor * ld + 2 * 64 + 4 * 512 + (sizeof(SolverState) + 63) / 64 * 8;
+  const size_t n_dbl = 8 * ld + 2 * (size_t)maxcor * ld + 2 * 64 + 4 * 512 + (sizeof(SolverState) + 63) / 64 * 8;
   MLN_TRY(f->sv_block.alloc_zeroed(ctx, n_dbl, "sv_block"));
   double* p = f->sv_block;
   SolverBuffers& b = f->sv;
@@ -217,6 +276,7 @@
   b.S = p; p += (size_t)maxcor * ld; b.Y = p; p += (size_t)maxcor * ld;
   b.rho = p; p += 64; b.yy = p; p += 64;
   b.c = p; p += ld;
+  b.ua = p; p += ld; b.ga = p; p += ld;
   b.trace = p; p += 4 * 512;
   b.st = (SolverState*)p;
   b.ld = (int64_t)ld;
@@ -301,14 +361,27 @@
   if (const char* ev = mln_experiment("MELLON_AMD_REBUILD")) want_rebuild = std::atoi(ev) != 0 ? 1.0 : 0.0;
   if (phase32 && !(f->l32_fixed)) want_rebuild = 0.0;
   const bool keeps_f = f->f_keep[0] && f->f_keep[1] && objective_can_keep_f(f->n, f->n_wg);
+  double tail_frac = 8.0;
+  if (const char* ev = mln_experiment("MELLON_AMD_TAIL_FRAC")) tail_frac = std::max(1.0, std::atof(ev));
+  double want_tail = (2.0 * pass_s > 12.0 * ((pass_s - 1.4e-4) / tail_frac + 1.6e-4) + 5e-4) ? 1.0 : 0.0;
+  if (const char* ev = mln_experiment("MELLON_AMD_IMPORTANCE_TAIL")) want_tail = std::atoi(ev) != 0 ? 1.0 : 0.0;
+  double n_total = (double)f->n;
   {
-    double vote[2] = {ctx->rank == 0 ? want_rebuild : 0.0, keeps_f ? 0.0 : 1.0};
-    MLN_HIP(ctx, hipMemcpyAsync(f->d_tmp, vote, sizeof(vote), hipMemcpyHostToDevice, ctx->stream));
-    MLN_TRY(dev_allreduce(ctx, f->d_tmp, 2));
-    MLN_HIP(ctx, hipMemcpyAsync(vote, f->d_tmp, sizeof(vote), hipMemcpyDeviceToHost, ctx->stream));
+    double vote[3] = {ctx->rank == 0 ? want_rebuild + 2.0 * want_tail : 0.0, keeps_f ? 0.0 : 1.0, (double)f->n};
+    MLN_HIP(ctx, hipMemcpyAsync(f->d_out, vote, sizeof(vote), hipMemcpyHostToDevice, ctx->stream));
+    MLN_TRY(dev_allreduce(ctx, f->d_out, 3));
+    MLN_HIP(ctx, hipMemcpyAsync(vote, f->d_out, sizeof(vote), hipMemcpyDeviceToHost, ctx->stream));
     MLN_HIP(ctx, hipStreamSynchronize(ctx->stream));
-    want_rebuild = (vote[0] != 0.0 && vote[1] == 0.0) ? 1.0 : 0.0;
-  }
+    want_tail = ((int)vote[0] & 2) ? 1.0 : 0.0;
+    want_rebuild = (((int)vote[0] & 1) && vote[1] == 0.0) ? 1.0 : 0.0;
+    n_total = vote[2];
+  }
+  const bool tail_enabled = !phase32 && want_rebuild != 0.0 && want_tail != 0.0;
+  init.tail_max_evals = 24;
+  init.tail_ftol = 100.0 * o.ftol;
+  if (const char* ev = mln_experiment("MELLON_AMD_TAIL_FTOL")) init.tail_ftol = std::atof(ev);
+  if (f->tail_sel.idx || f->tail_sel.scale) { MLN_HIP(ctx, hipStreamSynchronize(ctx->stream)); f->tail_sel.reset(); }
+  const RebuildSelection* tail_live = nullptr;
   int max_rebuilds = 1000;
   if (const char* ev = mln_experiment("MELLON_AMD_MAX_REBUILDS")) max_rebuilds = std::max(1, std::atoi(ev));
   init.rebuild_armed = want_rebuild != 0.0 ? (phase32 ? 1 : max_rebuilds) : 0;
@@ -347,7 +420,7 @@
   for (;;) {
     for (int b = 0; b < batch; ++b) {
       MLN_TRY(launch_solver_step(ctx, f->sv, (int)m));
-      MLN_TRY(fit_enqueue_eval(f, f->sv.un, f->sv.gn, false, gate, events_for(n_enq), subs_live));
+      MLN_TRY(fit_enqueue_eval(f, f->sv.un, f->sv.gn, false, gate, events_for(n_enq), subs_live, tail_live));
       ++n_enq;
     }
     MLN_TRY(dev_bcast0(ctx, (double*)f->sv.st, (int64_t)(sizeof(SolverState) / sizeof(double))));
@@ -381,8 +454,21 @@
         if (outcome == 0) {
           if (revert && ps.corr && (ps.gate_after_pause & 3) == MLN_GATE_F32)
             MLN_TRY(launch_solver_resume_plain32(ctx, f->sv, MLN_GATE_F32, (int)m, 1));
-          else
-            MLN_TRY(launch_solver_resume(ctx, f->sv, ps.gate_after_pause, 1, (revert || ps.rebuild_armed > 0) ? 0 : revert_after));
+          else {
+            int resume_gate = ps.gate_after_pause;
+            const double tail_target = std::max(n_total / tail_frac, 24.0 * (double)m);
+            if (tail_enabled && !revert && rebuilds_this_solve == 0 && !tail_live && ps.gate_after_pause == MLN_GATE_F64 && !ps.corr &&
+                tail_target <= 0.5 * n_total) {
+              const char* poor = mln_experiment("MELLON_AMD_TAIL_POOR_LIST");
+              MLN_TRY(rebuild_select_rows(ctx, f->f_keep[ps.f_slot], f->V, f->n, f->row0, tail_target, 0x6d656c6c6f6eull, &f->tail_sel, ps.cap,
+                                          !(poor && std::atoi(poor) != 0)));
+              tail_live = &f->tail_sel;
+              resume_gate = MLN_GATE_TAIL;
+              if (trace_lvl) fprintf(stderr, "[trace] importance tail: %lld of %lld local rows (target %.0f of %.0f), c = %.4g\n",
+                                     (long long)f->tail_sel.rows, (long long)f->n, tail_target, n_total, f->tail_sel.c);
+            }
+            MLN_TRY(launch_solver_resume(ctx, f->sv, resume_gate, 1, (revert || ps.rebuild_armed > 0) ? 0 : revert_after));
+          }
           if (revert) f->n_revert += 1; else { f->n_rebuild += 1; rebuilds_this_solve += 1; }
         } else {
           failed_rebuilds += 1;
@@ -403,6 +489,9 @@
     if (batch < 16 && f->h_state->gate == MLN_GATE_F64) batch = std::min(batch, 6);
   }
   const SolverState st = *f->h_state;
+  const int64_t tail_rows = f->tail_sel.rows;
+  if (tail_live) { (void)hipStreamSynchronize(ctx->stream); f->tail_sel.reset(); f->tail_rows = tail_rows; }
+  f->n_tail_guard += st.n_tail_guard;
   if (f->pc_saved.C) (void)hipStreamSynchronize(ctx->stream);
   f->pc_saved = Precond();
   f->n_start_halvings = st.n_shrink;
@@ -413,7 +502,7 @@
     MLN_HIP(ctx, hipMemcpy(tr.data(), f->sv.trace, sizeof(double) * 4 * n_done, hipMemcpyDeviceToHost));
     for (int i = 0; i < n_done && timing; ++i) {
       const int gcode = (int)tr[4 * i + 3] & 15, lvl = (int)tr[4 * i + 3] >> 4;
-      const bool was32 = (gcode & 3) == MLN_GATE_F32, was_sub = gcode == MLN_GATE_SUB;
+      const bool was32 = (gcode & 3) == MLN_GATE_F32, was_sub = gcode == MLN_GATE_SUB, was_tail = gcode == MLN_GATE_TAIL;
       int slot = i;
       for (const auto& sh : slot_shift) if (i >= sh.first) slot = i + sh.second;
       if (3 * (slot + 1) > (int)f->evs.size()) continue;
@@ -423,12 +512,16 @@
         f->times_sub += 1e-3 * ms; f->evals_sub += 1;
         f->sub_pass_equiv += 1.0 / (double)((lvl >= 0 && lvl < (int)sub_strides.size()) ? sub_strides[lvl] : 1);
       }
+      else if (was_tail) {
+        f->times_tail += 1e-3 * ms; f->evals_tail += 1;
+        f->sub_pass_equiv += f->n > 0 ? (double)tail_rows / (double)f->n : 0.0;
+      }
       else if (was32) { f->times32 += 1e-3 * ms; f->evals32 += 1; }
       else { f->times[5] += 1e-3 * ms; f->times[6] += 1.0; f->times[7] = (double)f->n * (double)f->ldl * 8.0; }
     }
     if (trace_lvl >= 2)
       for (int i = 0; i < n_done; ++i)
-        fprintf(stderr, "[eval %d] %s mode=%d t=%.3g f=%.15g\n", i, ((int)tr[4 * i + 3] & 15) == MLN_GATE_F32 ? "f32" : (((int)tr[4 * i + 3] & 15) == MLN_GATE_F32C ? "f32c" : (((int)tr[4 * i + 3] & 15) == MLN_GATE_SUB ? (((int)tr[4 * i + 3] >> 4) ? "sub1" : "sub0") : "f64")),
+        fprintf(stderr, "[eval %d] %s mode=%d t=%.3g f=%.15g\n", i, ((int)tr[4 * i + 3] & 15) == MLN_GATE_F32 ? "f32" : (((int)tr[4 * i + 3] & 15) == MLN_GATE_F32C ? "f32c" : (((int)tr[4 * i + 3] & 15) == MLN_GATE_SUB ? (((int)tr[4 * i + 3] >> 4) ? "sub1" : "sub0") : (((int)tr[4 * i + 3] & 15) == MLN_GATE_TAIL ? "tail" : "f64"))),
                 (int)tr[4 * i + 2], tr[4 * i + 1], tr[4 * i]);
   }
   {
@@ -518,5 +611,9 @@
   out[19] = (double)f->n_revert;
   out[20] = (double)f->n_start_halvings;
   out[21] = (double)f->rank_path;
-  return MLN_OK;
-}
+  out[22] = (double)f->evals_tail;
+  out[23] = (double)f->tail_rows;
+  out[24] = f->times_tail;
+  out[25] = (double)f->n_tail_guard;
+  return MLN_OK;
+}
diff --git a/mellon_amd/csrc/objective.h b/mellon_amd/csrc/objective.h
--- a/mellon_amd/csrc/objective.h
+++ b/mellon_amd/csrc/objective.h
@@ -26,8 +26,11 @@
   int64_t seg_cols;
   int64_t seg_left;
   int f_accum;
+  const int64_t* rows;
+  const double* row_w;
 };
-enum { MLN_GATE_F64 = 0, MLN_GATE_F32 = 1, MLN_GATE_DONE = 2, MLN_GATE_SUB = 3, MLN_GATE_F32C = 5, MLN_GATE_PAUSE = 6 };
+enum { MLN_GATE_F64 = 0, MLN_GATE_F32 = 1, MLN_GATE_DONE = 2, MLN_GATE_SUB = 3, MLN_GATE_F32C = 5, MLN_GATE_PAUSE = 6, MLN_GATE_TAIL = 7 };
+enum { MLN_TAIL_LEVEL = 64 };
 int objective_max_m();
 int objective_max_m_one_pass();
 bool objective_can_keep_f(int64_t n, int n_wg);
diff --git a/mellon_amd/csrc/objective.hip b/mellon_amd/csrc/objective.hip
--- a/mellon_amd/csrc/objective.hip
+++ b/mellon_amd/csrc/objective.hip
@@ -36,9 +36,51 @@
   }
 }
 
-
 template <int R>
-__device__ __forceinline__ void load_lik(const ObjArgs& a, int64_t row, double (&pv)[2][R]) {
+__device__ __forceinline__ void load_idx(const ObjArgs& a, int64_t row, int64_t (&idx)[R]) {
+#pragma unroll
+  for (int r = 0; r < R; ++r) idx[r] = a.rows[(row + r < a.n) ? (row + r) : (a.n - 1)];
+}
+
+template <int CPT, int R>
+__device__ __forceinline__ void load_rows_idx(const d2* __restrict__ L2, int64_t ld2, const int64_t (&idx)[R], unsigned tid,
+                                              d2 (&v)[R][CPT], unsigned lim) {
+#pragma unroll
+  for (int r = 0; r < R; ++r) {
+    const d2* rowp = L2 + idx[r] * ld2;
+#pragma unroll
+    for (int c = 0; c < CPT; ++c) {
+      unsigned off = (unsigned)c * WG + tid;
+      off = (off < lim) ? off : lim - 1u;
+      v[r][c] = __builtin_nontemporal_load(rowp + off);
+    }
+  }
+}
+
+template <int R, bool VEC>
+__device__ __forceinline__ void load_lik_idx(const ObjArgs& a, int64_t row, const int64_t (&idx)[R], int tid, double (&pv)[3][R]) {
+  if constexpr (VEC) {
+    const int lane = tid & 63;
+    int64_t i = idx[R - 1];
+#pragma unroll
+    for (int r = 0; r < R - 1; ++r) i = (lane == r) ? idx[r] : i;
+    const int64_t want = row + (lane < R ? lane : R - 1);
+    pv[0][0] = a.V[i];
+    pv[1][0] = a.Vdr[i];
+    pv[2][0] = a.row_w ? a.row_w[(want < a.n) ? want : (a.n - 1)] : 1.0;
+  } else {
+#pragma unroll
+    for (int r = 0; r < R; ++r) {
+      pv[0][r] = a.V[idx[r]];
+      pv[1][r] = a.Vdr[idx[r]];
+      pv[2][r] = a.row_w ? a.row_w[(row + r < a.n) ? (row + r) : (a.n - 1)] : 1.0;
+    }
+  }
+}
+
+
+template <int R>
+__device__ __forceinline__ void load_lik(const ObjArgs& a, int64_t row, double (&pv)[3][R]) {
   const RowMap rm = row_map(a);
 #pragma unroll
   for (int r = 0; r < R; ++r) {
@@ -49,7 +91,7 @@
 }
 
 template <int R>
-__device__ __forceinline__ void load_lik_vec(const ObjArgs& a, int64_t row, int tid, double (&pv)[2][R]) {
+__device__ __forceinline__ void load_lik_vec(const ObjArgs& a, int64_t row, int tid, double (&pv)[3][R]) {
   const RowMap rm = row_map(a);
   const int lane = tid & 63;
   const int64_t want = row + (lane < R ? lane : R - 1);
@@ -85,11 +127,11 @@
   return s;
 }
 
-template <int CPT, int R, int MODE, bool KEEP, bool VEC = false>
+template <int CPT, int R, int MODE, bool KEEP, bool VEC = false, bool LIST = false>
 __device__ __forceinline__ void process_rows(const ObjArgs& a, int64_t row, int64_t row_end, int tid, int par,
                                              const d2 (&v)[R][CPT], const d2 (&z)[CPT], d2 (&g)[CPT],
                                              d2 (&h)[CPT], double& loss, double (*red)[8][R], double* fstage,
-                                             int64_t fbase, const double (&pv)[2][R], const double capv, int& any_over) {
+                                             int64_t fbase, const double (&pv)[3][R], const double capv, int& any_over) {
   double coef[R], aexp[R];
   const RowMap rm = row_map(a);
   if constexpr (MODE == MODE_GEMVT) {
@@ -121,7 +163,8 @@
     const double Vi = pv[0][0];
     const double tt = f + Vi;
     const bool over = tt > capv;
-    const double ex = rok ? exp(over ? capv : tt) : 0.0;
+    double ex = rok ? exp(over ? capv : tt) : 0.0;
+    if constexpr (LIST) ex *= pv[2][0];
     const double dc = over ? (tt - capv) : 0.0;
     const double e = ex * fma(dc, fma(0.5, dc, 1.0), 1.0);
     const double cf = rok ? (over ? fma(ex, dc, ex - 1.0) : ex - 1.0) : 0.0;
@@ -165,15 +208,16 @@
         coef[r] = 0.0;
         aexp[r] = 0.0;
       } else {
-        const double Vi = KEEP ? pv[0][r] : (rok ? a.V[rm(row + r)] : 0.0);
+        const double Vi = (KEEP || LIST) ? pv[0][r] : (rok ? a.V[rm(row + r)] : 0.0);
         const double tt = f + Vi;
         const bool over = tt > capv;
-        const double ex = rok ? exp(over ? capv : tt) : 0.0;
+        double ex = rok ? exp(over ? capv : tt) : 0.0;
+        if constexpr (LIST) ex *= pv[2][r];
         const double dc = over ? (tt - capv) : 0.0;
         const double e = ex * fma(dc, fma(0.5, dc, 1.0), 1.0);
         aexp[r] = ex;
         coef[r] = rok ? (over ? fma(ex, dc, ex - 1.0) : ex - 1.0) : 0.0;
-        if (KEEP) { if (tid == 0 && rok) loss -= (f + pv[1][r]) - e; }
+        if (KEEP || LIST) { if (tid == 0 && rok) loss -= (f + pv[1][r]) - e; }
         else if (tid == 0 && rok) loss -= (f + a.Vdr[rm(row + r)]) - e;
         any_over += (tid == 0 && rok && over) ? 1 : 0;
         if (KEEP) lds_store_f64(fstage, (tid == 0 && rok) ? (int)(row + r - fbase) : (MLN_FSTAGE + tid), f);
@@ -196,7 +240,7 @@
   }
 }
 
-template <int CPT, int R, int MODE, bool KEEP = false, bool VEC = false>
+template <int CPT, int R, int MODE, bool KEEP = false, bool VEC = false, bool LIST = false>
 __global__ __launch_bounds__(WG) void k_objective(ObjArgs a) {
   if (a.gate && (*a.gate & 3) != a.gate_want) return;
   if (a.gate2 && *a.gate2 != a.gate2_want) return;
@@ -229,11 +273,31 @@
   const int64_t fbase = s_beg * R;
   d2 va[R][CPT], vb[R][CPT];
   const int64_t s_last = s_end - 1;
-  double pa[2][R], pb[2][R];
+  double pa[3][R], pb[3][R];
   const RowMap rm = row_map(a);
   const unsigned lim = a.seg_cols > 0 ? (unsigned)(a.seg_left / 2) : (unsigned)ld2;
-  auto lik = [&](int64_t r0, double (&pv)[2][R]) { if (VEC) load_lik_vec<R>(a, r0, tid, pv); else load_lik<R>(a, r0, pv); };
+  auto lik = [&](int64_t r0, double (&pv)[3][R]) { if (VEC) load_lik_vec<R>(a, r0, tid, pv); else load_lik<R>(a, r0, pv); };
   constexpr bool PRE = KEEP || (VEC && (MODE == MODE_OBJ || MODE == MODE_OBJ_HESS));
+  if constexpr (LIST) {
+    int64_t ia[R], ib[R];
+    if (s_beg < s_end) {
+      load_idx<R>(a, s_beg * R, ia);
+      load_idx<R>(a, ((s_beg + 1 < s_end) ? s_beg + 1 : s_last) * R, ib);
+      load_rows_idx<CPT, R>(L2, ld2, ia, tid, va, lim);
+      load_lik_idx<R, VEC>(a, s_beg * R, ia, tid, pa);
+    }
+    for (int64_t s = s_beg; s < s_end; s += 2) {
+      const int64_t s1 = (s + 1 < s_end) ? s + 1 : s_last, s2 = (s + 2 < s_end) ? s + 2 : s_last, s3 = (s + 3 < s_end) ? s + 3 : s_last;
+      load_rows_idx<CPT, R>(L2, ld2, ib, tid, vb, lim);
+      load_lik_idx<R, VEC>(a, s1 * R, ib, tid, pb);
+      load_idx<R>(a, s2 * R, ia);
+      process_rows<CPT, R, MODE, KEEP, VEC, true>(a, s * R, a.n, tid, 0, va, z, g, h, loss, red, fstage, fbase, pa, capv, any_over);
+      load_rows_idx<CPT, R>(L2, ld2, ia, tid, va, lim);
+      load_lik_idx<R, VEC>(a, s2 * R, ia, tid, pa);
+      load_idx<R>(a, s3 * R, ib);
+      if (s + 1 < s_end) process_rows<CPT, R, MODE, KEEP, VEC, true>(a, (s + 1) * R, a.n, tid, 1, vb, z, g, h, loss, red, fstage, fbase, pb, capv, any_over);
+    }
+  } else {
   if (s_beg < s_end) { load_rows<CPT, R>(L2, ld2, s_beg * R, a.n, tid, va, rm, lim); if (PRE) lik(s_beg * R, pa); }
   for (int64_t s = s_beg; s < s_end; s += 2) {
     const int64_t s1 = (s + 1 < s_end) ? s + 1 : s_last, s2 = (s + 2 < s_end) ? s + 2 : s_last;
@@ -244,6 +308,7 @@
     if (PRE) lik(s2 * R, pa);
     if (s + 1 < s_end) process_rows<CPT, R, MODE, KEEP, VEC>(a, (s + 1) * R, a.n, tid, 1, vb, z, g, h, loss, red, fstage, fbase, pb, capv, any_over);
   }
+  }
   if (any_over && a.over_flag) atomicAdd(a.over_flag, any_over);
   if (KEEP) {
     __syncthreads();
@@ -303,7 +368,7 @@
 __device__ __forceinline__ void process_rows32(const ObjArgs& a, int64_t row, int64_t row_end, int tid, int par,
                                                const f4 (&v)[R][CQ], const double (&z)[CQ][4], double (&g)[CQ][4],
                                                double& loss, double (*red)[NW][R], double* fstage, int64_t fbase,
-                                               const double (&pv)[2][R], double capv, double ecap, int& any_over) {
+                                               const double (&pv)[3][R], double capv, double ecap, int& any_over) {
   double coef[R], dot[R];
   const RowMap rm = row_map(a);
   if (GEMVT) {
@@ -441,10 +506,10 @@
   const int64_t fbase = s_beg * R;
   f4 va[R][CQ], vb[R][CQ];
   const int64_t s_last = s_end - 1;
-  double pa[2][R], pb[2][R];
+  double pa[3][R], pb[3][R];
   const RowMap rm = row_map(a);
   constexpr bool PRE = KEEP || (VEC && !GEMVT);
-  auto lik = [&](int64_t r0, double (&pv)[2][R]) { if (VEC) load_lik_vec<R>(a, r0, tid, pv); else load_lik<R>(a, r0, pv); };
+  auto lik = [&](int64_t r0, double (&pv)[3][R]) { if (VEC) load_lik_vec<R>(a, r0, tid, pv); else load_lik<R>(a, r0, pv); };
   if (s_beg < s_end) { load_rows32<CQ, R, NW>(L4, ld4, s_beg * R, a.n, tid, va, rm); if (PRE) lik(s_beg * R, pa); }
   for (int64_t s = s_beg; s < s_end; s += 2) {
     const int64_t s1 = (s + 1 < s_end) ? s + 1 : s_last, s2 = (s + 2 < s_end) ? s + 2 : s_last;
@@ -629,7 +694,9 @@
   dim3 grid((unsigned)a.n_wg), block(WG);
   switch (mode) {
     case MODE_OBJ:
-      if (a.f_slot) hipLaunchKernelGGL((k_objective<CPT, R, MODE_OBJ, true, VEC>), grid, block, 0, ctx->stream, a);
+      if (a.rows && a.f_slot) hipLaunchKernelGGL((k_objective<CPT, R, MODE_OBJ, true, VEC, true>), grid, block, 0, ctx->stream, a);
+      else if (a.rows) hipLaunchKernelGGL((k_objective<CPT, R, MODE_OBJ, false, VEC, true>), grid, block, 0, ctx->stream, a);
+      else if (a.f_slot) hipLaunchKernelGGL((k_objective<CPT, R, MODE_OBJ, true, VEC>), grid, block, 0, ctx->stream, a);
       else hipLaunchKernelGGL((k_objective<CPT, R, MODE_OBJ, false, VEC>), grid, block, 0, ctx->stream, a);
       break;
     case MODE_OBJ_HESS: hipLaunchKernelGGL((k_objective<CPT, R, MODE_OBJ_HESS, false, VEC>), grid, block, 0, ctx->stream, a); break;
@@ -679,7 +746,7 @@
 int launch_objective(mln_ctx* ctx, const ObjArgs& a);
 
 static int launch_objective_wide(mln_ctx* ctx, const ObjArgs& a) {
-  if (a.gate || a.part_hess || a.L32 || (a.row_stride > 1)) {
+  if (a.gate || a.part_hess || a.L32 || (a.row_stride > 1) || a.rows) {
     mln_set_error(ctx, "objective: this mode is not available beyond 8192 landmarks");
     return MLN_ERR_UNSUPPORTED;
   }
@@ -734,6 +801,10 @@
   if (a.weights) mode = MODE_GEMVT;
   else if (a.f_out) mode = MODE_FONLY;
   else if (a.part_hess) mode = MODE_OBJ_HESS;
+  if (a.rows && (mode != MODE_OBJ || a.L32 || a.seg_cols > 0)) {
+    mln_set_error(ctx, "objective: a row list goes with the plain fp64 objective only");
+    return MLN_ERR_UNSUPPORTED;
+  }
   if (a.L32 && (mode == MODE_OBJ || mode == MODE_GEMVT) && a.ldl % 4 == 0) {
     const int cq = (int)((a.ldl / 4 + WG - 1) / WG);
     const bool vec32 = mode == MODE_OBJ;
diff --git a/mellon_amd/csrc/precond_rebuild.h b/mellon_amd/csrc/precond_rebuild.h
--- a/mellon_amd/csrc/precond_rebuild.h
+++ b/mellon_amd/csrc/precond_rebuild.h
@@ -12,6 +12,7 @@
 };
 
 int rebuild_select_rows(mln_ctx* ctx, const double* f_dev, const double* V_dev, int64_t n, int64_t row0,
-                        double target_rows_global, uint64_t seed, RebuildSelection* out, double cap = 1e300);
+                        double target_rows_global, uint64_t seed, RebuildSelection* out, double cap = 1e300,
+                        bool inverse_prob = false);
 int launch_gather_scale_rows(mln_ctx* ctx, const double* A, int64_t ld, const int64_t* idx, const double* scale,
                              int64_t rows, double* R);
diff --git a/mellon_amd/csrc/precond_rebuild.hip b/mellon_amd/csrc/precond_rebuild.hip
--- a/mellon_amd/csrc/precond_rebuild.hip
+++ b/mellon_amd/csrc/precond_rebuild.hip
@@ -105,7 +105,7 @@
 
 __global__ __launch_bounds__(64) void k_select_write(const double* __restrict__ a, int64_t n, double c, int64_t row0,
                                                      uint64_t seed, const int64_t* __restrict__ offsets, double inv_wmax,
-                                                     int64_t* __restrict__ idx, double* __restrict__ scale) {
+                                                     int64_t* __restrict__ idx, double* __restrict__ scale, int inverse_prob) {
   const int64_t base = (int64_t)blockIdx.x * SB;
   int64_t out = offsets[blockIdx.x];
   for (int j0 = 0; j0 < SB; j0 += 64) {
@@ -116,7 +116,7 @@
       const int pos = __popcll(mask & ((1ull << threadIdx.x) - 1ull));
       idx[out + pos] = i;
       const double w = fmax(a[i], 1.0 / c);
-      scale[out + pos] = sqrt(w * inv_wmax);
+      scale[out + pos] = inverse_prob ? fmax(1.0, 1.0 / (c * a[i])) : sqrt(w * inv_wmax);
     }
     out += __popcll(mask);
   }
@@ -140,7 +140,7 @@
 }
 
 int rebuild_select_rows(mln_ctx* ctx, const double* f_dev, const double* V_dev, int64_t n, int64_t row0,
-                        double target_rows_global, uint64_t seed, RebuildSelection* out, double cap) {
+                        double target_rows_global, uint64_t seed, RebuildSelection* out, double cap, bool inverse_prob) {
   *out = RebuildSelection();
   const int nb = 256;
   DevBuf<double> a, part, part2, scal;
@@ -209,7 +209,7 @@
         rc = MLN_ERR_HIP;
       if (rc == MLN_OK) {
         hipLaunchKernelGGL(k_select_write, dim3((unsigned)n_blk), dim3(64), 0, ctx->stream, a.get(), n, c, row0, seed, offsets.get(),
-                           1.0 / w_max, out->idx.get(), out->scale.get());
+                           1.0 / w_max, out->idx.get(), out->scale.get(), inverse_prob ? 1 : 0);
         if (hipStreamSynchronize(ctx->stream) != hipSuccess) rc = MLN_ERR_HIP;
       }
     }
diff --git a/mellon_amd/csrc/solver.h b/mellon_amd/csrc/solver.h
--- a/mellon_amd/csrc/solver.h
+++ b/mellon_amd/csrc/solver.h
@@ -47,6 +47,15 @@
   int revert_after;
   int it_at_resume;
   int pause_reason;
+  int tail_on;
+  int tail_sync;
+  int tail_max_evals;
+  int n_eval_anchor;
+  int tail_conv;
+  int n_tail_guard;
+  int tail_over_a;
+  double tail_ftol;
+  double tail_fa;
 };
 
 struct SolverBuffers {
@@ -55,6 +64,7 @@
   double *S, *Y;
   double *rho, *yy;
   double* c;
+  double *ua, *ga;
   const double* z;
   const double* z2;
   const double* lik;
diff --git a/mellon_amd/csrc/solver.hip b/mellon_amd/csrc/solver.hip
--- a/mellon_amd/csrc/solver.hip
+++ b/mellon_amd/csrc/solver.hip
@@ -79,8 +79,11 @@
   const bool resume = st->mode == MLN_SOLVE_RESUME;
   const bool phaseA = st->gate == MLN_GATE_F32, phaseC = st->gate == MLN_GATE_F32C, phaseS = st->gate == MLN_GATE_SUB;
   const bool phase32 = phaseA || phaseC;
-  const bool approx = phase32 || phaseS;
-  if (phaseC) {
+  const bool phaseT = st->gate == MLN_GATE_TAIL;
+  const bool tail_sync = phaseT && !resume && st->tail_sync != 0;
+  const bool phaseCT = phaseC || phaseT;
+  const bool approx = phase32 || phaseS || phaseT;
+  if (phaseC || (phaseT && !resume && !tail_sync)) {
     double cu = 0.0;
 #pragma unroll
     for (int e = 0; e < EPT; ++e) {
@@ -98,7 +101,12 @@
   double dec_prev = st->dec_prev, dec_prev2 = st->dec_prev2;
   const bool after_switch = mode == MLN_SOLVE_REEVAL && !phaseS && !phaseC && st->n_eval_sub > 0 && st->it_full == 0;
   bool recap = false;
-  if (mode != MLN_SOLVE_LS && !resume) t0 = 1.0;
+  if (mode != MLN_SOLVE_LS && !resume && !tail_sync) t0 = 1.0;
+  int tail_on = st->tail_on, n_eval_anchor = st->n_eval_anchor + ((phaseT && !resume && !tail_sync) ? 1 : 0);
+  bool tail_cut = false;
+  int n_tail_guard = st->n_tail_guard, tail_over_a = st->tail_over_a;
+  double tail_fa = st->tail_fa;
+  bool tail_req = false, tail_back = false, new_anchor = false;
   int f_slot = st->f_slot, f_valid = st->f_valid, corr = st->corr, n_anchor = st->n_anchor;
   int over_acc = st->over_acc;
   double over_cnt_acc = st->over_cnt_acc;
@@ -111,15 +119,39 @@
   bool to_head = false, reeval = false, done = false, verify = false, pause = false, shrink = false;
   int pause_reason = 1;
   if (resume) {
-    to_head = true;
     if (!st->resume_keep_pairs) { k = 0; head = 0; }
     dec_prev = 0.0; dec_prev2 = 0.0;
+    if (phaseT) tail_req = true; else to_head = true;
   } else if (mode == MLN_SOLVE_FIRST && (!isfinite(fn) || fn > st->start_cap) && st->n_shrink < 64) {
 #pragma unroll
     for (int e = 0; e < EPT; ++e) { u[e] *= 0.5; un[e] = u[e]; }
     shrink = true;
+  } else if (tail_sync) {
+    double cu = 0.0;
+#pragma unroll
+    for (int e = 0; e < EPT; ++e) {
+      const double cv = g[e] - gn[e];
+      if (on[e]) b.c[idx[e]] = cv;
+      cu = fma(cv, u[e], cu);
+    }
+    cu = block_sum(cu, red);
+    corr_k = (fx - fn) - cu;
+    corr = 1; n_anchor = 1; n_eval_anchor = 0;
+    to_head = true;
+  } else if (mode == MLN_SOLVE_REEVAL && !approx && tail_on && !(fn <= tail_fa)) {
+#pragma unroll
+    for (int e = 0; e < EPT; ++e) { u[e] = on[e] ? b.ua[idx[e]] : 0.0; g[e] = on[e] ? b.ga[idx[e]] : 0.0; }
+    fx = tail_fa; over_acc = tail_over_a; over_cnt_acc = 0.0;
+    tail_on = 0; corr = 0; ++n_tail_guard;
+    k = 0; head = 0; dec_prev = 0.0; dec_prev2 = 0.0;
+    f_valid = 1;
+    gate = MLN_GATE_F64;
+    tail_back = true;
+    to_head = true;
   } else if (mode != MLN_SOLVE_LS) {
-    if (mode == MLN_SOLVE_REEVAL && !phase32 && st->use_corr) {
+    const bool tail_verify = mode == MLN_SOLVE_REEVAL && !approx && tail_on;
+    if (tail_verify && st->tail_conv && (tail_fa - fn) <= st->ftol * fmax(fmax(fabs(tail_fa), fabs(fn)), 1.0)) { status = 0; done = true; }
+    if ((mode == MLN_SOLVE_REEVAL && !phase32 && st->use_corr) || tail_verify) {
       verify = corr != 0;
       if (n_anchor < 4) {
         double dcu = 0.0;
@@ -133,18 +165,28 @@
         dcu = block_sum(dcu, red);
         corr_k = (corr ? corr_k : 0.0) + (fn - fx) - dcu;
         corr = 1; ++n_anchor;
-        gate = MLN_GATE_F32C;
+        gate = tail_verify ? MLN_GATE_TAIL : MLN_GATE_F32C;
+        new_anchor = tail_verify;
       } else {
         corr = 0;
+        tail_on = 0;
       }
     }
     fx = fn;
+    if (tail_verify) { dec_prev = 0.0; dec_prev2 = 0.0; }
     over_acc = over_now; over_cnt_acc = over_cnt_now;
-    f_slot ^= 1; f_valid = approx ? 0 : 1;
+    if (!phaseT) f_slot ^= 1;
+    f_valid = approx ? 0 : 1;
 #pragma unroll
     for (int e = 0; e < EPT; ++e) g[e] = gn[e];
+    if (new_anchor) {
+#pragma unroll
+      for (int e = 0; e < EPT; ++e)
+        if (on[e]) { b.ua[idx[e]] = u[e]; b.ga[idx[e]] = g[e]; }
+      tail_fa = fx; tail_over_a = over_acc; n_eval_anchor = 0;
+    }
     if (mode == MLN_SOLVE_REEVAL && !approx && st->rebuild_armed && corr && n_anchor == 1 && st->use_corr) pause = true;
-    else to_head = true;
+    else if (!done) to_head = true;
   } else {
     ++ls;
     const bool ok = isfinite(fn) && fn <= fx + 1e-4 * t * gd;
@@ -170,7 +212,8 @@
       for (int e = 0; e < EPT; ++e) { u[e] = un[e]; g[e] = gn[e]; }
       fx = fn;
       over_acc = over_now; over_cnt_acc = over_cnt_now;
-      f_slot ^= 1; f_valid = approx ? 0 : 1;
+      if (!phaseT) f_slot ^= 1;
+      f_valid = approx ? 0 : 1;
       if (!phaseS) ++it_full;
       if (sy > 1e-10 * sqrt(ss * yy)) {
         int slot;
@@ -192,6 +235,13 @@
                           (f_old - fx) > st->ftol * fscale;
       if (revert) {
         pause = true; pause_reason = 2;
+        if (phaseT) {
+#pragma unroll
+          for (int e = 0; e < EPT; ++e) { u[e] = on[e] ? b.ua[idx[e]] : 0.0; g[e] = on[e] ? b.ga[idx[e]] : 0.0; }
+          fx = tail_fa; over_acc = tail_over_a; over_cnt_acc = 0.0;
+          tail_on = 0; corr = 0; f_valid = 1;
+          gate = MLN_GATE_F64;
+        }
       } else if (phaseS) {
         if (it >= 4 && ((f_old - fx) <= st->sub_tol * fscale || n_eval_sub >= st->sub_max_evals)) { reeval = true; next_level = true; } else to_head = true;
       } else if (st->rebuild_armed > 0 && st->it_resume < 0 && !phase32 && !recap && it_full >= 2 && (slow || (it_full >= 4 && st->over_many > 0.0 && over_cnt_acc >= st->over_many && isfinite(fx)))) {
@@ -203,8 +253,8 @@
         reeval = true;
       } else if (phaseA) {
         if ((f_old - fx) <= st->ftol32 * fscale) reeval = true; else to_head = true;
-      } else if ((f_old - fx) <= st->ftol * fscale) {
-        if (phaseC) reeval = true; else { status = 0; done = true; }
+      } else if ((f_old - fx) <= (phaseT ? st->tail_ftol : st->ftol) * fscale) {
+        if (phaseCT) reeval = true; else { status = 0; done = true; }
       } else {
         const double dec = f_old - fx;
         bool small_gap = false;
@@ -213,15 +263,28 @@
           const double r = dec / dec_prev;
           small_gap = dec * r / (1.0 - r) <= st->gap_tol * fscale;
         }
-        if (small_gap) { if (phaseC) reeval = true; else { status = 0; done = true; } }
+        if (small_gap) { if (phaseCT) reeval = true; else { status = 0; done = true; } }
+        else if (phaseT && n_eval_anchor >= st->tail_max_evals) { reeval = true; tail_cut = true; }
         else to_head = true;
       }
       if (!phaseS) { dec_prev2 = dec_prev; dec_prev = f_old - fx; }
-    } else if (isfinite(fn) && fabs(fn - fx) <= st->ftol * fmax(fmax(fabs(fx), fabs(fn)), 1.0)) {
-      if (approx && !(phaseC && f_valid)) { reeval = true; next_level = phaseS; } else { status = 0; done = true; }
+    } else if (phaseT && f_valid && isfinite(fn) && fabs(fn - fx) <= st->tail_ftol * fmax(fmax(fabs(fx), fabs(fn)), 1.0)) {
+      tail_on = 0; corr = 0; gate = MLN_GATE_F64;
+      t = 1.0; ls = 0;
+#pragma unroll
+      for (int e = 0; e < EPT; ++e) un[e] = u[e] + d[e];
+    } else if (isfinite(fn) && fabs(fn - fx) <= (phaseT ? st->tail_ftol : st->ftol) * fmax(fmax(fabs(fx), fabs(fn)), 1.0)) {
+      if (approx && !(phaseCT && f_valid)) { reeval = true; next_level = phaseS; } else { status = 0; done = true; }
+    } else if (phaseT && ls >= 3) {
+      if (f_valid) {
+        tail_on = 0; corr = 0; gate = MLN_GATE_F64;
+        t = 1.0; ls = 0;
+#pragma unroll
+        for (int e = 0; e < EPT; ++e) un[e] = u[e] + d[e];
+      } else { reeval = true; tail_cut = true; }
     } else if (ls >= st->maxls) {
-      if (approx && !(phaseC && f_valid)) { reeval = true; next_level = phaseS; }
-      else { status = phaseC ? 0 : 2; done = true; }
+      if (approx && !(phaseCT && f_valid)) { reeval = true; next_level = phaseS; tail_cut = phaseT; }
+      else { status = phaseCT ? 0 : 2; done = true; }
     } else {
       if (isfinite(fn)) {
         const double tq = -gd * t * t / (2.0 * (fn - fx - gd * t));
@@ -239,7 +302,7 @@
     for (int e = 0; e < EPT; ++e) gm = fmax(gm, fabs(g[e]));
     gm = block_max(gm, red);
     if (!(gm > st->gtol)) {
-      if (approx) { reeval = true; next_level = phaseS; } else { status = 0; done = true; }
+      if (approx && !(phaseT && f_valid)) { reeval = true; next_level = phaseS; } else { status = 0; done = true; }
     } else if (it >= st->maxiter) {
       status = 1; done = true;
     } else {
@@ -297,9 +360,10 @@
         gd = -block_sum(acc, red);
       }
       if (verify && -0.5 * gd <= st->ftol * fmax(fabs(fx), 1.0)) { status = 0; done = true; }
+      else if (new_anchor && -0.5 * gd <= st->tail_ftol * fmax(fabs(fx), 1.0)) { tail_on = 0; corr = 0; gate = MLN_GATE_F64; }
       t = t0;
       if (after_switch && st->switch_t0 > 0.0) t = st->switch_t0;
-      if (k == 0 && !resume) {
+      if (k == 0 && !resume && !tail_sync && !tail_back) {
         double g1 = 0.0;
 #pragma unroll
         for (int e = 0; e < EPT; ++e) g1 += fabs(g[e]);
@@ -325,6 +389,17 @@
     mode = MLN_SOLVE_REEVAL;
 #pragma unroll
     for (int e = 0; e < EPT; ++e) un[e] = u[e];
+  }
+  if (tail_req) {
+    mode = MLN_SOLVE_REEVAL;
+    sub_level = MLN_TAIL_LEVEL;
+    tail_on = 1; corr = 0; n_anchor = 0; n_eval_anchor = 0;
+    tail_fa = fx; tail_over_a = over_acc;
+#pragma unroll
+    for (int e = 0; e < EPT; ++e) {
+      un[e] = u[e];
+      if (on[e]) { b.ua[idx[e]] = u[e]; b.ga[idx[e]] = g[e]; }
+    }
   }
   if (pause) { if (tid == 0) st->gate_after_pause = gate; gate = MLN_GATE_PAUSE; }
   if (done) gate = MLN_GATE_DONE;
@@ -339,6 +414,9 @@
     st->n_eval_sub = n_eval_sub; st->it_full = it_full; st->sub_level = sub_level;
     st->dec_prev = dec_prev; st->dec_prev2 = dec_prev2;
     st->over_acc = over_acc; st->over_cnt_acc = over_cnt_acc;
+    st->tail_on = tail_on; st->tail_sync = tail_req ? 1 : 0; st->n_eval_anchor = n_eval_anchor;
+    if (reeval && phaseT) st->tail_conv = tail_cut ? 0 : 1;
+    st->n_tail_guard = n_tail_guard; st->tail_fa = tail_fa; st->tail_over_a = tail_over_a;
     if (shrink) st->n_shrink += 1;
     if (pause) { st->rebuild_armed = (pause_reason == 1 && st->rebuild_armed > 0) ? st->rebuild_armed - 1 : 0; st->pause_reason = pause_reason; st->it_at_resume = -1; }
   }
```

Result: faster. 8.412 million, median of 6 (+12.5%).
